# url-kaist/Quatro

Hardware: NVIDIA H100
Metric: registrations/sec (64-ring pair) (higher is better)
Workload: dtype f32 (front end, match, graph filter) / f64 (graph boundary, GNC, COTE)

## Files before the change

include/quatro_b200.h:

```cpp
#ifndef QUATRO_B200_H_
#define QUATRO_B200_H_

#include <stdint.h>

#ifdef __cplusplus
extern "C" {
#endif

#define QB200_VERSION 100

typedef enum qb200_status {
  QB200_OK = 0,
  QB200_DEGENERATE_CLIQUE = 1,
  QB200_DEGENERATE_INPUT = 2,
  QB200_CAPACITY_EXCEEDED = 3,
  QB200_ERR_BAD_ARG = -1,
  QB200_ERR_NO_DEVICE = -2,
  QB200_ERR_CUDA = -3,
  QB200_ERR_UNSUPPORTED = -4,
  QB200_ERR_VOXEL_OVERFLOW = -5
} qb200_status;

enum { QB200_FLAG_CLIQUE_TRUNCATED = 1  };
#define QB200_DEFAULT_CLIQUE_NODE_LIMIT 262144

enum { QB200_PMC_EXACT = 0, QB200_PMC_HEU = 1, QB200_KCORE_HEU = 2, QB200_INLIER_NONE = 3 };
enum { QB200_COTE_MEDIAN = 0, QB200_COTE_WEIGHTED_MEAN = 1 };
typedef enum qb200_mem_kind { QB200_MEM_HOST = 0, QB200_MEM_DEVICE = 1 } qb200_mem_kind;

typedef struct qb200_params {
  float voxel_size;
  float normal_radius;
  float fpfh_radius;
  float grid_cell;
  float tuple_scale;
  int32_t use_crosscheck;
  int32_t use_tuple_test;
  int32_t tuple_trials_per_corr;
  int32_t skip_flagged;
  int32_t reserved0;
  uint64_t seed;
  double noise_bound;
  double cbar2;
  double rot_noise_bound;
  double cote_noise_bound;
  double rotation_gnc_factor;
  double rotation_cost_threshold;
  double kcore_heuristic_threshold;
  int32_t rotation_max_iterations;
  int32_t inlier_selection_mode;
  int32_t cote_mode;
  int32_t using_rot_inliers_when_estimating_cote;
  int32_t use_pre_estimated_RyRx;
  int32_t max_clique_node_limit;
  double RyRx[9];
} qb200_params;

#define QB200_MAX_VOXEL_POINTS 262144

typedef struct qb200_config {
  int32_t device;
  int32_t max_batch_slots;
  int32_t max_raw_points;
  int32_t max_voxel_points;
  int32_t max_corr;
  int32_t reserved[3];
} qb200_config;

typedef struct qb200_result {
  int32_t valid;
  int32_t status;
  int32_t n_src_vox, n_tgt_vox;
  int32_t n_mutual;
  int32_t n_corr;
  int32_t max_core;
  int32_t clique_size;
  int32_t gnc_iters;
  int32_t n_rot_inliers;
  int32_t n_final_inliers;
  int32_t flags;
  int64_t n_edges;
  double cost;
  double T[16];
} qb200_result;

typedef struct qb200_pair {
  const float* src;
  const float* tgt;
  int32_t n_src, n_tgt;
} qb200_pair;

typedef struct qb200_handle qb200_handle;

void qb200_default_params(qb200_params* p);
void qb200_default_config(qb200_config* c);
int qb200_version(void);

int qb200_create(const qb200_config* cfg, qb200_handle** out);
void qb200_destroy(qb200_handle* h);
int qb200_set_stream(qb200_handle* h, void* cuda_stream);
const char* qb200_last_error(const qb200_handle* h);
int64_t qb200_launch_count(const qb200_handle* h);


int qb200_voxelize(qb200_handle* h, const float* pts4, int32_t n, float leaf, int32_t skip_flagged,
                   float* out4, int32_t cap, int32_t* n_out);

#define QB200_PW_MAX_ZONES 4
#define QB200_PW_MAX_THRESHOLDS 8
typedef struct qb200_patchwork_params {
  double sensor_height;
  double th_seeds;
  double th_dist;
  double max_range;
  double min_range;
  double uprightness_thr;
  double adaptive_seed_selection_margin;
  double global_elevation_threshold;
  double min_ranges_each_zone[QB200_PW_MAX_ZONES];
  double elevation_thresholds[QB200_PW_MAX_THRESHOLDS];
  double flatness_thresholds[QB200_PW_MAX_THRESHOLDS];
  int32_t num_iter;
  int32_t num_lpr;
  int32_t num_min_pts;
  int32_t using_global_elevation;
  int32_t num_zones;
  int32_t num_thresholds;
  int32_t num_sectors_each_zone[QB200_PW_MAX_ZONES];
  int32_t num_rings_each_zone[QB200_PW_MAX_ZONES];
} qb200_patchwork_params;
void qb200_default_patchwork_params(qb200_patchwork_params* p);

int qb200_patchwork(qb200_handle* h, const float* pts4, int32_t n, const qb200_patchwork_params* p,
                    float* ground4, int32_t* n_ground, float* nonground4, int32_t* n_nonground);

enum { QB200_NEIGHBORS_4 = 0, QB200_NEIGHBORS_8 = 1, QB200_NEIGHBORS_4_CROSS = 2 };
typedef struct qb200_segment_params {
  int32_t n_scan;
  int32_t horizon_scan;
  float ang_res_x;
  float ang_res_y;
  float ang_bottom;
  float segment_theta;
  int32_t neighbor_mode;
  int32_t min_pts_for_subclustering;
  int32_t segment_valid_point_num;
  int32_t segment_valid_line_num;
} qb200_segment_params;
void qb200_default_segment_params(qb200_segment_params* p);

int qb200_segment_cloud(qb200_handle* h, const float* pts4, int32_t n, const qb200_segment_params* p,
                        float* valid4, int32_t* n_valid, float* outlier4, int32_t* n_outlier);

int qb200_compute_fpfh(qb200_handle* h, const float* pts4, int32_t n, float normal_radius,
                       float fpfh_radius, float grid_cell, float* normals4, float* desc33);

int qb200_match(qb200_handle* h, const float* src4, int32_t n_src, const float* src_desc33,
                const float* tgt4, int32_t n_tgt, const float* tgt_desc33, const qb200_params* p,
                int32_t* corr, int32_t cap, int32_t* n_corr, int32_t* n_mutual);

int qb200_build_graph(qb200_handle* h, const float* a4, const float* b4, int32_t L,
                      double noise_bound, double cbar2, uint32_t* adj, int32_t words_per_row,
                      int32_t* degree, int64_t* n_edges);

int qb200_max_clique(qb200_handle* h, const uint32_t* adj, int32_t L, int32_t words_per_row,
                     int32_t mode, double kcore_heuristic_threshold, int32_t* clique, int32_t* n_clique,
                     int32_t* kcore, int32_t* kcore_order, int32_t* max_core);
int qb200_max_clique_ex(qb200_handle* h, const uint32_t* adj, int32_t L, int32_t words_per_row,
                        int32_t mode, double kcore_heuristic_threshold, int64_t node_limit, int32_t* clique, int32_t* n_clique,
                        int32_t* kcore, int32_t* kcore_order, int32_t* max_core, int32_t* flags);

int qb200_solve_pose(qb200_handle* h, const float* a4, const float* b4, int32_t L,
                     const int32_t* clique, int32_t n_clique, const qb200_params* p,
                     qb200_result* res, uint8_t* rot_inlier_mask, uint8_t* trans_inlier_mask);

int qb200_solve_correspondences(qb200_handle* h, const float* a4, const float* b4, int32_t L,
                                const qb200_params* p, qb200_result* res);

int qb200_match_and_pack(qb200_handle* h, const float* src4, int32_t n_src, const float* tgt4,
                         int32_t n_tgt, const qb200_params* p, int32_t* corr, float* src_matched4,
                         float* tgt_matched4, int32_t cap, int32_t* n_corr);

typedef struct qb200_corr_set {
  const float* a;
  const float* b;
  int32_t L;
  int32_t reserved;
} qb200_corr_set;
int qb200_solve_batch(qb200_handle* h, const qb200_corr_set* sets, int32_t n_sets, const qb200_params* p,
                      qb200_mem_kind kind, qb200_result* results);

int qb200_register_batch_enqueue(qb200_handle* h, const qb200_pair* pairs, int32_t n_pairs, const qb200_params* p, qb200_mem_kind kind,
                                 qb200_result* results);
int qb200_register_batch_flush(qb200_handle* h);

int qb200_register_pair(qb200_handle* h, const float* src4, int32_t n_src, const float* tgt4,
                        int32_t n_tgt, const qb200_params* p, qb200_result* res);

int qb200_register_batch(qb200_handle* h, const qb200_pair* pairs, int32_t n_pairs,
                         const qb200_params* p, qb200_mem_kind kind, qb200_result* results);

typedef struct qb200_slot_pair { int32_t src_slot, tgt_slot; } qb200_slot_pair;
int qb200_cache_reserve(qb200_handle* h, int32_t n_slots);
int qb200_cache_scans(qb200_handle* h, const float* const* scans4, const int32_t* n_points, const int32_t* slot_ids, int32_t n_scans,
                      const qb200_params* p, qb200_mem_kind kind);
int qb200_register_cached(qb200_handle* h, const qb200_slot_pair* pairs, int32_t n_pairs, const qb200_params* p, qb200_result* results);
int qb200_cache_copy(qb200_handle* h, int32_t from_slot, int32_t to_slot);
int qb200_cache_read(qb200_handle* h, int32_t slot, float* vox4, float* normals4, float* desc33, int32_t cap, int32_t* n);

#define QB200_UNIQUE_ID_BYTES 128
int qb200_comm_init_all(qb200_handle** handles, int32_t n_dev);
int qb200_register_batch_sharded(qb200_handle** handles, int32_t n_dev, const qb200_pair* pairs, int32_t n_pairs,
                                 const qb200_params* p, qb200_mem_kind kind, qb200_result* results);
int qb200_comm_unique_id(void* id128);
int qb200_comm_init_rank(qb200_handle* h, int32_t world, int32_t rank, const void* id128);
int qb200_register_batch_rank(qb200_handle* h, const qb200_pair* local_pairs, int32_t n_local, const qb200_params* p,
                              qb200_mem_kind kind, qb200_result* all_results, int32_t defer);
int qb200_comm_wait(qb200_handle* h);
int qb200_bind_numa(qb200_handle* h);

int qb200_get_last_clique(qb200_handle* h, int32_t* idx, int32_t cap, int32_t* n);
int qb200_get_last_final_inliers(qb200_handle* h, int32_t* idx, int32_t cap, int32_t* n);
int qb200_get_last_correspondences(qb200_handle* h, int32_t* corr, float* src_matched4,
                                   float* tgt_matched4, int32_t cap, int32_t* n);

int qb200_get_last_features(qb200_handle* h, int32_t which, float* normals4, float* desc33, int32_t cap, int32_t* n);

int qb200_get_stage_ms(qb200_handle* h, float* ms, int32_t n);

int qb200_get_kernel_ms(qb200_handle* h, float* ms, int32_t* launches, int32_t n);

int qb200_debug_tc_distances(qb200_handle* h, const float* a33, int32_t na, const float* b33, int32_t nb, float* out);


int qb200_debug_match_stats(qb200_handle* h, uint64_t* out4, int32_t reset);
int qb200_debug_tc_profile(qb200_handle* h, uint64_t* out24, int32_t reset);

int qb200_debug_match_verify(qb200_handle* h, uint64_t* out2, int32_t reset);

#ifdef __cplusplus
}
#endif
#endif
```

quatro_b200/capi.py:

```python
from __future__ import annotations

import ctypes as C
from typing import Optional, Sequence

import numpy as np

from . import _build

PMC_EXACT, PMC_HEU, KCORE_HEU, INLIER_NONE = 0, 1, 2, 3
FLAG_CLIQUE_TRUNCATED = 1
COTE_MEDIAN, COTE_WEIGHTED_MEAN = 0, 1
MEM_HOST, MEM_DEVICE = 0, 1

STATUS_NAMES = {0: "OK", 1: "DEGENERATE_CLIQUE", 2: "DEGENERATE_INPUT", 3: "CAPACITY_EXCEEDED", -1: "ERR_BAD_ARG",
                -2: "ERR_NO_DEVICE", -3: "ERR_CUDA", -4: "ERR_UNSUPPORTED", -5: "ERR_VOXEL_OVERFLOW"}


class Params(C.Structure):
    _fields_ = [
        ("voxel_size", C.c_float), ("normal_radius", C.c_float), ("fpfh_radius", C.c_float), ("grid_cell", C.c_float),
        ("tuple_scale", C.c_float), ("use_crosscheck", C.c_int32), ("use_tuple_test", C.c_int32),
        ("tuple_trials_per_corr", C.c_int32), ("skip_flagged", C.c_int32), ("reserved0", C.c_int32),
        ("seed", C.c_uint64),
        ("noise_bound", C.c_double), ("cbar2", C.c_double), ("rot_noise_bound", C.c_double),
        ("cote_noise_bound", C.c_double), ("rotation_gnc_factor", C.c_double),
        ("rotation_cost_threshold", C.c_double), ("kcore_heuristic_threshold", C.c_double),
        ("rotation_max_iterations", C.c_int32), ("inlier_selection_mode", C.c_int32), ("cote_mode", C.c_int32),
        ("using_rot_inliers_when_estimating_cote", C.c_int32), ("use_pre_estimated_RyRx", C.c_int32),
        ("max_clique_node_limit", C.c_int32), ("RyRx", C.c_double * 9),
    ]


class Config(C.Structure):
    _fields_ = [("device", C.c_int32), ("max_batch_slots", C.c_int32), ("max_raw_points", C.c_int32),
                ("max_voxel_points", C.c_int32), ("max_corr", C.c_int32), ("reserved", C.c_int32 * 3)]


class Result(C.Structure):
    _fields_ = [
        ("valid", C.c_int32), ("status", C.c_int32), ("n_src_vox", C.c_int32), ("n_tgt_vox", C.c_int32),
        ("n_mutual", C.c_int32), ("n_corr", C.c_int32), ("max_core", C.c_int32), ("clique_size", C.c_int32),
        ("gnc_iters", C.c_int32), ("n_rot_inliers", C.c_int32), ("n_final_inliers", C.c_int32),
        ("flags", C.c_int32), ("n_edges", C.c_int64), ("cost", C.c_double), ("T", C.c_double * 16),
    ]

    def matrix(self) -> np.ndarray:
        return np.array(self.T[:], dtype=np.float64).reshape(4, 4).T.copy()

    def as_dict(self) -> dict:
        d = {k: getattr(self, k) for k, _ in self._fields_ if k != "T"}
        d["T"] = self.matrix()
        return d


class PatchworkParams(C.Structure):
    _fields_ = [
        ("sensor_height", C.c_double), ("th_seeds", C.c_double), ("th_dist", C.c_double), ("max_range", C.c_double),
        ("min_range", C.c_double), ("uprightness_thr", C.c_double), ("adaptive_seed_selection_margin", C.c_double),
        ("global_elevation_threshold", C.c_double), ("min_ranges_each_zone", C.c_double * 4),
        ("elevation_thresholds", C.c_double * 8), ("flatness_thresholds", C.c_double * 8),
        ("num_iter", C.c_int32), ("num_lpr", C.c_int32), ("num_min_pts", C.c_int32), ("using_global_elevation", C.c_int32),
        ("num_zones", C.c_int32), ("num_thresholds", C.c_int32), ("num_sectors_each_zone", C.c_int32 * 4),
        ("num_rings_each_zone", C.c_int32 * 4),
    ]


class SegmentParams(C.Structure):
    _fields_ = [("n_scan", C.c_int32), ("horizon_scan", C.c_int32), ("ang_res_x", C.c_float), ("ang_res_y", C.c_float),
                ("ang_bottom", C.c_float), ("segment_theta", C.c_float), ("neighbor_mode", C.c_int32),
                ("min_pts_for_subclustering", C.c_int32), ("segment_valid_point_num", C.c_int32), ("segment_valid_line_num", C.c_int32)]


class Pair(C.Structure):
    _fields_ = [("src", C.c_void_p), ("tgt", C.c_void_p), ("n_src", C.c_int32), ("n_tgt", C.c_int32)]


class CorrSet(C.Structure):
    _fields_ = [("a", C.c_void_p), ("b", C.c_void_p), ("L", C.c_int32), ("reserved", C.c_int32)]


RESULT_DTYPE = np.dtype([
    ("valid", "<i4"), ("status", "<i4"), ("n_src_vox", "<i4"), ("n_tgt_vox", "<i4"), ("n_mutual", "<i4"),
    ("n_corr", "<i4"), ("max_core", "<i4"), ("clique_size", "<i4"), ("gnc_iters", "<i4"), ("n_rot_inliers", "<i4"),
    ("n_final_inliers", "<i4"), ("flags", "<i4"), ("n_edges", "<i8"), ("cost", "<f8"), ("T", "<f8", (16,)),
])
assert RESULT_DTYPE.itemsize == C.sizeof(Result)


class QuatroB200Error(RuntimeError):
    def __init__(self, code: int, where: str, detail: str = ""):
        self.code = code
        super().__init__(f"{where}: {STATUS_NAMES.get(code, code)} {detail}")


_LIB: Optional[C.CDLL] = None


def _f32(a, cols=None) -> np.ndarray:
    a = np.ascontiguousarray(a, dtype=np.float32)
    if cols is not None:
        assert a.ndim == 2 and a.shape[1] == cols, (a.shape, cols)
    return a


def _ptr(a: Optional[np.ndarray]):
    return None if a is None else a.ctypes.data_as(C.c_void_p)


def load_library(build: bool = True) -> C.CDLL:
    global _LIB
    if _LIB is not None:
        return _LIB
    path = _build.build_cuda() if build else _build.CUDA_LIB
    lib = C.CDLL(str(path))
    vp, i32, i64, f32, f64 = C.c_void_p, C.c_int32, C.c_int64, C.c_float, C.c_double
    P = C.POINTER
    sig = {
        "qb200_default_params": (None, [P(Params)]),
        "qb200_default_config": (None, [P(Config)]),
        "qb200_version": (i32, []),
        "qb200_create": (i32, [P(Config), P(vp)]),
        "qb200_destroy": (None, [vp]),
        "qb200_set_stream": (i32, [vp, vp]),
        "qb200_last_error": (C.c_char_p, [vp]),
        "qb200_launch_count": (i64, [vp]),
        "qb200_voxelize": (i32, [vp, vp, i32, f32, i32, vp, i32, P(i32)]),
        "qb200_default_patchwork_params": (None, [P(PatchworkParams)]),
        "qb200_default_segment_params": (None, [P(SegmentParams)]),
        "qb200_segment_cloud": (i32, [vp, vp, i32, P(SegmentParams), vp, P(i32), vp, P(i32)]),
        "qb200_patchwork": (i32, [vp, vp, i32, P(PatchworkParams), vp, P(i32), vp, P(i32)]),
        "qb200_compute_fpfh": (i32, [vp, vp, i32, f32, f32, f32, vp, vp]),
        "qb200_match": (i32, [vp, vp, i32, vp, vp, i32, vp, P(Params), vp, i32, P(i32), P(i32)]),
        "qb200_build_graph": (i32, [vp, vp, vp, i32, f64, f64, vp, i32, vp, P(i64)]),
        "qb200_max_clique": (i32, [vp, vp, i32, i32, i32, f64, vp, P(i32), vp, vp, P(i32)]),
        "qb200_max_clique_ex": (i32, [vp, vp, i32, i32, i32, f64, i64, vp, P(i32), vp, vp, P(i32), P(i32)]),
        "qb200_solve_pose": (i32, [vp, vp, vp, i32, vp, i32, P(Params), P(Result), vp, vp]),
        "qb200_solve_correspondences": (i32, [vp, vp, vp, i32, P(Params), P(Result)]),
        "qb200_match_and_pack": (i32, [vp, vp, i32, vp, i32, P(Params), vp, vp, vp, i32, P(i32)]),
        "qb200_register_pair": (i32, [vp, vp, i32, vp, i32, P(Params), P(Result)]),
        "qb200_register_batch": (i32, [vp, P(Pair), i32, P(Params), i32, vp]),
        "qb200_get_last_clique": (i32, [vp, vp, i32, P(i32)]),
        "qb200_get_last_final_inliers": (i32, [vp, vp, i32, P(i32)]),
        "qb200_get_last_correspondences": (i32, [vp, vp, vp, vp, i32, P(i32)]),
        "qb200_get_stage_ms": (i32, [vp, vp, i32]),
        "qb200_get_kernel_ms": (i32, [vp, vp, vp, i32]),
        "qb200_debug_tc_distances": (i32, [vp, vp, i32, vp, i32, vp]),
        "qb200_debug_match_stats": (i32, [vp, vp, i32]),
        "qb200_register_batch_enqueue": (i32, [vp, vp, i32, vp, i32, vp]),
        "qb200_register_batch_flush": (i32, [vp]),
        "qb200_debug_tc_profile": (i32, [vp, vp, i32]),
        "qb200_solve_batch": (i32, [vp, vp, i32, vp, i32, vp]),
        "qb200_comm_init_all": (i32, [P(vp), i32]),
        "qb200_register_batch_sharded": (i32, [P(vp), i32, P(Pair), i32, P(Params), i32, vp]),
        "qb200_comm_unique_id": (i32, [vp]),
        "qb200_comm_init_rank": (i32, [vp, i32, i32, vp]),
        "qb200_register_batch_rank": (i32, [vp, P(Pair), i32, P(Params), i32, vp, i32]),
        "qb200_comm_wait": (i32, [vp]),
        "qb200_bind_numa": (i32, [vp]),
        "qb200_debug_match_verify": (i32, [vp, vp, i32]),
        "qb200_get_last_features": (i32, [vp, i32, vp, vp, i32, P(i32)]),
        "qb200_cache_reserve": (i32, [vp, i32]),
        "qb200_cache_scans": (i32, [vp, P(vp), P(i32), P(i32), i32, P(Params), i32]),
        "qb200_register_cached": (i32, [vp, vp, i32, P(Params), vp]),
        "qb200_cache_copy": (i32, [vp, i32, i32]),
        "qb200_cache_read": (i32, [vp, i32, vp, vp, vp, i32, P(i32)]),
    }
    for name, (res, args) in sig.items():
        fn = getattr(lib, name)
        fn.restype = res
        fn.argtypes = args
    _LIB = lib
    return lib


EXPORTED_SYMBOLS = [
    "qb200_default_params", "qb200_default_config", "qb200_version", "qb200_create", "qb200_destroy",
    "qb200_set_stream", "qb200_last_error", "qb200_launch_count", "qb200_voxelize", "qb200_compute_fpfh",
    "qb200_default_patchwork_params", "qb200_patchwork", "qb200_default_segment_params", "qb200_segment_cloud", "qb200_match", "qb200_build_graph", "qb200_max_clique", "qb200_max_clique_ex", "qb200_solve_pose", "qb200_solve_correspondences",
    "qb200_match_and_pack", "qb200_register_pair", "qb200_register_batch", "qb200_get_last_clique",
    "qb200_get_last_final_inliers", "qb200_get_last_correspondences", "qb200_get_stage_ms", "qb200_get_kernel_ms",
    "qb200_debug_tc_distances",
    "qb200_debug_match_stats",
    "qb200_register_batch_enqueue",
    "qb200_register_batch_flush",
    "qb200_debug_tc_profile",
    "qb200_solve_batch",
    "qb200_comm_init_all", "qb200_register_batch_sharded", "qb200_comm_unique_id", "qb200_comm_init_rank",
    "qb200_register_batch_rank", "qb200_comm_wait", "qb200_bind_numa",
    "qb200_debug_match_verify", "qb200_get_last_features", "qb200_cache_reserve", "qb200_cache_scans", "qb200_register_cached", "qb200_cache_copy", "qb200_cache_read",
]


def default_params() -> Params:
    p = Params()
    p.voxel_size, p.normal_radius, p.fpfh_radius, p.grid_cell = 0.3, 0.5, 0.75, 0.0
    p.tuple_scale, p.use_crosscheck, p.use_tuple_test, p.tuple_trials_per_corr = 0.95, 1, 1, 100
    p.skip_flagged, p.seed = 1, 0x5EED
    p.noise_bound, p.cbar2, p.rot_noise_bound, p.cote_noise_bound = 0.3, 1.0, 0.0, 0.3
    p.rotation_gnc_factor, p.rotation_cost_threshold, p.kcore_heuristic_threshold = 1.4, 0.00011, 0.5
    p.rotation_max_iterations, p.inlier_selection_mode, p.cote_mode = 50, PMC_HEU, COTE_MEDIAN
    p.using_rot_inliers_when_estimating_cote, p.use_pre_estimated_RyRx = 0, 0
    for i in range(9):
        p.RyRx[i] = 1.0 if i in (0, 4, 8) else 0.0
    return p


def comm_init_all(handles: Sequence["Handle"]):
    arr = (C.c_void_p * len(handles))(*[h.h for h in handles])
    st = load_library().qb200_comm_init_all(arr, len(handles))
    if st != 0:
        raise QuatroB200Error(st, "qb200_comm_init_all")


def register_batch_sharded(handles: Sequence["Handle"], pairs: Sequence, params: "Params", kind: int = 0) -> np.ndarray:
    n = len(pairs)
    arr = (Pair * n)()
    keep = []
    for i, pr in enumerate(pairs):
        if kind == MEM_HOST:
            s, t = _f32(pr[0], 4), _f32(pr[1], 4)
            keep.append((s, t))
            arr[i].src, arr[i].n_src, arr[i].tgt, arr[i].n_tgt = s.ctypes.data, len(s), t.ctypes.data, len(t)
        else:
            arr[i].src, arr[i].n_src, arr[i].tgt, arr[i].n_tgt = pr[0], pr[1], pr[2], pr[3]
    out = np.zeros(n, RESULT_DTYPE)
    hs = (C.c_void_p * len(handles))(*[h.h for h in handles])
    st = load_library().qb200_register_batch_sharded(hs, len(handles), arr, n, C.byref(params), kind, _ptr(out))
    if st != 0:
        raise QuatroB200Error(st, "qb200_register_batch_sharded " + handles[0].last_error())
    return out


def default_patchwork_params() -> PatchworkParams:
    p = PatchworkParams()
    load_library().qb200_default_patchwork_params(C.byref(p))
    return p


def default_segment_params() -> SegmentParams:
    p = SegmentParams()
    load_library().qb200_default_segment_params(C.byref(p))
    return p


def default_config() -> Config:
    c = Config()
    c.device, c.max_batch_slots, c.max_raw_points, c.max_voxel_points, c.max_corr = 0, 64, 131072, 16384, 4096
    return c


class Handle:

    def __init__(self, config: Optional[Config] = None, **kw):
        self.lib = load_library()
        cfg = config or default_config()
        for k, v in kw.items():
            setattr(cfg, k, v)
        self.cfg = cfg
        h = C.c_void_p()
        st = self.lib.qb200_create(C.byref(cfg), C.byref(h))
        if st != 0:
            raise QuatroB200Error(st, "qb200_create")
        self.h = h

    def close(self):
        if getattr(self, "h", None):
            self.lib.qb200_destroy(self.h)
            self.h = None

    def __del__(self):
        try:
            self.close()
        except Exception:
            pass

    def __enter__(self):
        return self

    def __exit__(self, *a):
        self.close()

    def _check(self, st: int, where: str):
        if st < 0:
            msg = self.lib.qb200_last_error(self.h)
            raise QuatroB200Error(st, where, (msg or b"").decode())
        return st

    def set_stream(self, stream_ptr: int):
        self._check(self.lib.qb200_set_stream(self.h, C.c_void_p(stream_ptr)), "qb200_set_stream")

    def launch_count(self) -> int:
        return int(self.lib.qb200_launch_count(self.h))

    def voxelize(self, pts4, leaf: float, skip_flagged: int = 1, cap: Optional[int] = None):
        pts4 = _f32(pts4, 4)
        cap = cap or max(1, len(pts4))
        out = np.zeros((cap, 4), np.float32)
        n = C.c_int32(0)
        st = self.lib.qb200_voxelize(self.h, _ptr(pts4), len(pts4), leaf, skip_flagged, _ptr(out), cap, C.byref(n))
        if st != -5:
            self._check(st, "qb200_voxelize")
        return out[: min(n.value, cap)].copy(), st

    def compute_fpfh(self, pts4, normal_radius: float, fpfh_radius: float, grid_cell: float):
        pts4 = _f32(pts4, 4)
        n = len(pts4)
        normals = np.zeros((n, 4), np.float32)
        desc = np.zeros((n, 33), np.float32)
        self._check(self.lib.qb200_compute_fpfh(self.h, _ptr(pts4), n, normal_radius, fpfh_radius, grid_cell, _ptr(normals), _ptr(desc)),
                    "qb200_compute_fpfh")
        return normals, desc

    def match(self, src4, sdesc, tgt4, tdesc, params: Params, cap: Optional[int] = None):
        src4, tgt4, sdesc, tdesc = _f32(src4, 4), _f32(tgt4, 4), _f32(sdesc, 33), _f32(tdesc, 33)
        cap = cap or max(1, min(len(src4), len(tgt4)))
        corr = np.zeros((cap, 2), np.int32)
        n, nm = C.c_int32(0), C.c_int32(0)
        st = self._check(self.lib.qb200_match(self.h, _ptr(src4), len(src4), _ptr(sdesc), _ptr(tgt4), len(tgt4), _ptr(tdesc),
                                              C.byref(params), _ptr(corr), cap, C.byref(n), C.byref(nm)), "qb200_match")
        return corr[: min(n.value, cap)].copy(), nm.value, st

    def build_graph(self, a4, b4, noise_bound: float, cbar2: float, words_per_row: Optional[int] = None):
        a4, b4 = _f32(a4, 4), _f32(b4, 4)
        L = len(a4)
        wpr = words_per_row or (L + 31) // 32
        adj = np.zeros((L, wpr), np.uint32)
        deg = np.zeros(L, np.int32)
        ne = C.c_int64(0)
        self._check(self.lib.qb200_build_graph(self.h, _ptr(a4), _ptr(b4), L, noise_bound, cbar2, _ptr(adj), wpr, _ptr(deg), C.byref(ne)),
                    "qb200_build_graph")
        return adj, deg, ne.value

    def patchwork(self, pts, pp: "PatchworkParams"):
        pts = _f32(pts, 4)
        n = len(pts)
        g, ng = np.zeros((max(n, 1), 4), np.float32), np.zeros((max(n, 1), 4), np.float32)
        a, b = C.c_int32(0), C.c_int32(0)
        st = self._check(self.lib.qb200_patchwork(self.h, _ptr(pts), n, C.byref(pp), _ptr(g), C.byref(a), _ptr(ng), C.byref(b)), "qb200_patchwork")
        return g[: a.value].copy(), ng[: b.value].copy(), st

    def segment_cloud(self, pts, sp: "SegmentParams"):
        pts = _f32(pts, 4)
        npix = sp.n_scan * sp.horizon_scan
        v, o = np.zeros((npix, 4), np.float32), np.zeros((npix, 4), np.float32)
        a, b = C.c_int32(0), C.c_int32(0)
        self._check(self.lib.qb200_segment_cloud(self.h, _ptr(pts), len(pts), C.byref(sp), _ptr(v), C.byref(a), _ptr(o), C.byref(b)),
                    "qb200_segment_cloud")
        return v[: a.value].copy(), o[: b.value].copy()

    def max_clique(self, adj, mode: int = PMC_HEU, kcore_thr: float = 0.5):
        adj = np.ascontiguousarray(adj, np.uint32)
        L, wpr = adj.shape
        clique = np.zeros(max(L, 1), np.int32)
        kcore = np.zeros(max(L, 1), np.int32)
        order = np.zeros(max(L, 1), np.int32)
        n, mc = C.c_int32(0), C.c_int32(0)
        self._check(self.lib.qb200_max_clique(self.h, _ptr(adj), L, wpr, mode, kcore_thr, _ptr(clique), C.byref(n), _ptr(kcore),
                                              _ptr(order), C.byref(mc)), "qb200_max_clique")
        return clique[: n.value].copy(), kcore[:L].copy(), order[:L].copy(), mc.value

    def max_clique_ex(self, adj, mode: int = PMC_EXACT, kcore_thr: float = 0.5, node_limit: int = 0):
        adj = np.ascontiguousarray(adj, np.uint32)
        L, wpr = adj.shape
        clique, kcore, order = (np.zeros(max(L, 1), np.int32) for _ in range(3))
        n, mc, fl = C.c_int32(0), C.c_int32(0), C.c_int32(0)
        self._check(self.lib.qb200_max_clique_ex(self.h, _ptr(adj), L, wpr, mode, kcore_thr, node_limit, _ptr(clique), C.byref(n),
                                                 _ptr(kcore), _ptr(order), C.byref(mc), C.byref(fl)), "qb200_max_clique_ex")
        return clique[: n.value].copy(), kcore[:L].copy(), order[:L].copy(), mc.value, fl.value

    def solve_pose(self, a4, b4, clique, params: Params):
        a4, b4 = _f32(a4, 4), _f32(b4, 4)
        clique = np.ascontiguousarray(clique, np.int32)
        res = Result()
        rm = np.zeros(max(len(clique), 1), np.uint8)
        tm = np.zeros(max(len(clique), 1), np.uint8)
        st = self._check(self.lib.qb200_solve_pose(self.h, _ptr(a4), _ptr(b4), len(a4), _ptr(clique), len(clique), C.byref(params),
                                                   C.byref(res), _ptr(rm), _ptr(tm)), "qb200_solve_pose")
        return res, rm[: len(clique)], tm[: len(clique)], st

    def solve_correspondences(self, a4, b4, params: Params):
        a4, b4 = _f32(a4, 4), _f32(b4, 4)
        res = Result()
        st = self._check(self.lib.qb200_solve_correspondences(self.h, _ptr(a4), _ptr(b4), len(a4), C.byref(params), C.byref(res)),
                         "qb200_solve_correspondences")
        return res, st

    def match_and_pack(self, src4, tgt4, params: Params, cap: Optional[int] = None):
        src4, tgt4 = _f32(src4, 4), _f32(tgt4, 4)
        cap = cap or max(1, min(len(src4), len(tgt4)))
        corr = np.zeros((cap, 2), np.int32)
        sm = np.zeros((cap, 4), np.float32)
        tm = np.zeros((cap, 4), np.float32)
        n = C.c_int32(0)
        st = self._check(self.lib.qb200_match_and_pack(self.h, _ptr(src4), len(src4), _ptr(tgt4), len(tgt4), C.byref(params), _ptr(corr),
                                                       _ptr(sm), _ptr(tm), cap, C.byref(n)), "qb200_match_and_pack")
        m = min(n.value, cap)
        return corr[:m].copy(), sm[:m].copy(), tm[:m].copy(), st

    def register_pair(self, src4, tgt4, params: Params):
        src4, tgt4 = _f32(src4, 4), _f32(tgt4, 4)
        res = Result()
        st = self._check(self.lib.qb200_register_pair(self.h, _ptr(src4), len(src4), _ptr(tgt4), len(tgt4), C.byref(params), C.byref(res)),
                         "qb200_register_pair")
        return res, st

    def register_batch(self, pairs: Sequence, params: Params, kind: int = MEM_HOST) -> np.ndarray:
        n = len(pairs)
        arr = (Pair * n)()
        keep = []
        for i, pr in enumerate(pairs):
            if kind == MEM_HOST:
                s, t = _f32(pr[0], 4), _f32(pr[1], 4)
                keep.append((s, t))
                arr[i].src, arr[i].n_src, arr[i].tgt, arr[i].n_tgt = s.ctypes.data, len(s), t.ctypes.data, len(t)
            else:
                arr[i].src, arr[i].n_src, arr[i].tgt, arr[i].n_tgt = pr[0], pr[1], pr[2], pr[3]
        out = np.zeros(n, RESULT_DTYPE)
        self._check(self.lib.qb200_register_batch(self.h, arr, n, C.byref(params), kind, _ptr(out)), "qb200_register_batch")
        return out

    def solve_batch(self, sets: Sequence, params: Params, kind: int = MEM_HOST) -> np.ndarray:
        n = len(sets)
        arr = (CorrSet * n)()
        keep = []
        for i, st in enumerate(sets):
            if kind == MEM_HOST:
                a, b = _f32(st[0], 4), _f32(st[1], 4)
                assert len(a) == len(b)
                keep.append((a, b))
                arr[i].a, arr[i].b, arr[i].L = a.ctypes.data, b.ctypes.data, len(a)
            else:
                arr[i].a, arr[i].b, arr[i].L = st[0], st[1], st[2]
        out = np.zeros(n, RESULT_DTYPE)
        self._check(self.lib.qb200_solve_batch(self.h, arr, n, C.byref(params), kind, _ptr(out)), "qb200_solve_batch")
        return out

    def last_features(self, which: int, cap: Optional[int] = None):
        cap = cap or self.cfg.max_voxel_points
        nrm, desc = np.zeros((cap, 4), np.float32), np.zeros((cap, 33), np.float32)
        n = C.c_int32(0)
        self._check(self.lib.qb200_get_last_features(self.h, which, _ptr(nrm), _ptr(desc), cap, C.byref(n)), "qb200_get_last_features")
        m = min(n.value, cap)
        return nrm[:m].copy(), desc[:m].copy()

    def cache_reserve(self, n_slots: int):
        self._check(self.lib.qb200_cache_reserve(self.h, n_slots), "qb200_cache_reserve")

    def cache_scans(self, scans: Sequence, slot_ids: Sequence[int], params: Params, kind: int = MEM_HOST):
        n = len(scans)
        keep = [_f32(sc, 4) for sc in scans] if kind == MEM_HOST else None
        ptrs = (C.c_void_p * n)(*([a.ctypes.data for a in keep] if kind == MEM_HOST else [sc[0] for sc in scans]))
        cnts = (C.c_int32 * n)(*([len(a) for a in keep] if kind == MEM_HOST else [sc[1] for sc in scans]))
        ids = (C.c_int32 * n)(*[int(x) for x in slot_ids])
        self._check(self.lib.qb200_cache_scans(self.h, ptrs, cnts, ids, n, C.byref(params), kind), "qb200_cache_scans")

    def register_cached(self, slot_pairs, params: Params) -> np.ndarray:
        sp = np.ascontiguousarray(np.asarray(slot_pairs, np.int32).reshape(-1, 2))
        out = np.zeros(len(sp), RESULT_DTYPE)
        self._check(self.lib.qb200_register_cached(self.h, _ptr(sp), len(sp), C.byref(params), _ptr(out)), "qb200_register_cached")
        return out

    def cache_copy(self, from_slot: int, to_slot: int):
        self._check(self.lib.qb200_cache_copy(self.h, from_slot, to_slot), "qb200_cache_copy")

    def cache_read(self, slot: int, cap: Optional[int] = None):
        cap = cap or self.cfg.max_voxel_points
        vox, nrm, desc = np.zeros((cap, 4), np.float32), np.zeros((cap, 4), np.float32), np.zeros((cap, 33), np.float32)
        n = C.c_int32(0)
        self._check(self.lib.qb200_cache_read(self.h, slot, _ptr(vox), _ptr(nrm), _ptr(desc), cap, C.byref(n)), "qb200_cache_read")
        m = min(n.value, cap)
        return vox[:m].copy(), nrm[:m].copy(), desc[:m].copy()

    @staticmethod
    def comm_unique_id() -> bytes:
        buf = C.create_string_buffer(128)
        st = load_library().qb200_comm_unique_id(buf)
        if st != 0:
            raise QuatroB200Error(st, "qb200_comm_unique_id")
        return buf.raw

    def comm_init_rank(self, world: int, rank: int, unique_id: bytes):
        buf = C.create_string_buffer(unique_id, 128)
        self._check(self.lib.qb200_comm_init_rank(self.h, world, rank, buf), "qb200_comm_init_rank")
        self.world, self.rank = world, rank

    def register_batch_rank_raw(self, pair_array, n_local: int, params: Params, kind: int, out_all: np.ndarray, defer: bool = False):
        return self._check(self.lib.qb200_register_batch_rank(self.h, pair_array, n_local, C.byref(params), kind, _ptr(out_all), int(defer)),
                           "qb200_register_batch_rank")

    def bind_numa(self) -> int:
        return int(self.lib.qb200_bind_numa(self.h))

    def comm_wait(self):
        return self._check(self.lib.qb200_comm_wait(self.h), "qb200_comm_wait")

    def register_batch_raw(self, pair_array, n: int, params: Params, kind: int, out: np.ndarray):
        return self._check(self.lib.qb200_register_batch(self.h, pair_array, n, C.byref(params), kind, _ptr(out)), "qb200_register_batch")

    def register_batch_enqueue_raw(self, pair_array, n: int, params: Params, kind: int, out: np.ndarray):
        return self._check(self.lib.qb200_register_batch_enqueue(self.h, pair_array, n, C.byref(params), kind, _ptr(out)), "qb200_register_batch_enqueue")

    def register_batch_flush(self):
        return self._check(self.lib.qb200_register_batch_flush(self.h), "qb200_register_batch_flush")

    def last_clique(self, cap: int = 1 << 16):
        idx = np.zeros(cap, np.int32)
        n = C.c_int32(0)
        self._check(self.lib.qb200_get_last_clique(self.h, _ptr(idx), cap, C.byref(n)), "qb200_get_last_clique")
        return idx[: n.value].copy()

    def last_final_inliers(self, cap: int = 1 << 16):
        idx = np.zeros(cap, np.int32)
        n = C.c_int32(0)
        self._check(self.lib.qb200_get_last_final_inliers(self.h, _ptr(idx), cap, C.byref(n)), "qb200_get_last_final_inliers")
        return idx[: n.value].copy()

    def last_correspondences(self, cap: int = 1 << 16):
        corr = np.zeros((cap, 2), np.int32)
        sm = np.zeros((cap, 4), np.float32)
        tm = np.zeros((cap, 4), np.float32)
        n = C.c_int32(0)
        self._check(self.lib.qb200_get_last_correspondences(self.h, _ptr(corr), _ptr(sm), _ptr(tm), cap, C.byref(n)),
                    "qb200_get_last_correspondences")
        return corr[: n.value].copy(), sm[: n.value].copy(), tm[: n.value].copy()

    def debug_match_stats(self, reset: bool = True) -> dict:
        out = np.zeros(4, np.uint64)
        self._check(self.lib.qb200_debug_match_stats(self.h, _ptr(out), int(reset)), "qb200_debug_match_stats")
        return {"exact_evals": int(out[0]), "tiles": int(out[1]), "warmups": int(out[2]), "aborted_stripes": int(out[3])}

    def debug_tc_profile(self, reset: bool = True) -> np.ndarray:
        out = np.zeros(24, np.uint64)
        self._check(self.lib.qb200_debug_tc_profile(self.h, _ptr(out), int(reset)), "qb200_debug_tc_profile")
        return out

    def debug_match_verify(self, reset: bool = True) -> dict:
        out = np.zeros(2, np.uint64)
        self._check(self.lib.qb200_debug_match_verify(self.h, _ptr(out), int(reset)), "qb200_debug_match_verify")
        return {"compared": int(out[0]), "mismatches": int(out[1])}

    def debug_tc_distances(self, a33, b33) -> np.ndarray:
        a33, b33 = _f32(a33, 33), _f32(b33, 33)
        out = np.zeros((128, 128), np.float32)
        self._check(self.lib.qb200_debug_tc_distances(self.h, _ptr(a33), len(a33), _ptr(b33), len(b33), _ptr(out)), "qb200_debug_tc_distances")
        return out[: len(a33), : len(b33)].copy()

    def kernel_ms(self):
        ms = np.zeros(2, np.float32)
        calls = np.zeros(2, np.int32)
        self.lib.qb200_get_kernel_ms(self.h, _ptr(ms), _ptr(calls), 2)
        return ms, calls

    def stage_ms(self) -> np.ndarray:
        ms = np.zeros(8, np.float32)
        self.lib.qb200_get_stage_ms(self.h, _ptr(ms), 8)
        return ms
```

quatro_b200/csrc/api.cu:

```cuda
#include <math.h>
#include <new>
#include <stdio.h>
#include <stdlib.h>
#include <string.h>
#include <map>
#include <mutex>
#include <utility>
#include <vector>

#include "handle.cuh"

using namespace qb;

namespace qb {
int launch_degree(qb200_handle* h, int n_pairs);

int ensure_dyn_smem(qb200_handle* h, const void* kernel, size_t bytes) {
  static std::mutex mu;
  static std::map<std::pair<const void*, int>, size_t> current;
  std::lock_guard<std::mutex> lock(mu);
  size_t& cur = current[std::make_pair(kernel, h->device)];
  if (bytes > cur) {
    QB_CUDA_TRY(h, cudaFuncSetAttribute(kernel, cudaFuncAttributeMaxDynamicSharedMemorySize, (int)bytes));
    cur = bytes;
  }
  return QB200_OK;
}
}

namespace {

__global__ void wave_init_kernel(int* ctr_block, int n_ints, int* bbox, int n_clouds) {
  const int i = blockIdx.x * blockDim.x + threadIdx.x;
  if (i < n_ints) ctr_block[i] = 0;
  if (i < n_clouds * 6) bbox[i] = (i % 6) < 3 ? INT_MAX : INT_MIN;
}

__global__ void cache_copy_kernel(int to_cache, const int* __restrict__ slot_of_cloud, int V, float4* __restrict__ w_vox, float4* __restrict__ w_nrm,
                                  float* __restrict__ w_desc, int* __restrict__ w_n, int* __restrict__ w_status, float4* __restrict__ c_vox,
                                  float4* __restrict__ c_nrm, float* __restrict__ c_desc, int* __restrict__ c_n, int* __restrict__ c_status) {
  const int cloud = blockIdx.z, slot = slot_of_cloud[cloud], row = blockIdx.y;
  const int q = blockIdx.x * blockDim.x + threadIdx.x;
  if (slot < 0) return;
  const int n = to_cache ? w_n[cloud] : c_n[slot];
  if (row == 42) {
    if (q == 0) {
      if (to_cache) { c_n[slot] = w_n[cloud]; c_status[slot] = w_status[cloud]; }
      else { w_n[cloud] = c_n[slot]; w_status[cloud] = c_status[slot]; }
    }
    return;
  }
  if (q >= n || q >= V) return;
  if (row < kDescK) {
    float* w = w_desc + ((size_t)cloud * kDescK + row) * V + q;
    float* c = c_desc + ((size_t)slot * kDescK + row) * V + q;
    if (to_cache) *c = *w; else *w = *c;
  } else if (row == 40) {
    if (to_cache) c_vox[(size_t)slot * V + q] = w_vox[(size_t)cloud * V + q]; else w_vox[(size_t)cloud * V + q] = c_vox[(size_t)slot * V + q];
  } else {
    if (to_cache) c_nrm[(size_t)slot * V + q] = w_nrm[(size_t)cloud * V + q]; else w_nrm[(size_t)cloud * V + q] = c_nrm[(size_t)slot * V + q];
  }
}

template <class T>
cudaError_t dalloc(T** p, size_t count) {
  return cudaMalloc(reinterpret_cast<void**>(p), count * sizeof(T));
}

#define QB_ALLOC(h, ptr, count)                                                    \
  do {                                                                             \
    cudaError_t _e = dalloc(&(ptr), (size_t)(count));                              \
    if (_e != cudaSuccess) {                                                       \
      (h)->fail(__FILE__, __LINE__, cudaGetErrorString(_e));                       \
      return QB200_ERR_CUDA;                                                       \
    }                                                                              \
  } while (0)

int alloc_all(qb200_handle* h) {
  const size_t S = h->S, R = h->R, V = h->V, Lc = h->Lc, W = h->W, C = 2 * S;
  QB_CUDA_TRY(h, cudaMalloc((void**)&h->d_cloud_ptr, C * sizeof(float4*)));
  QB_ALLOC(h, h->d_cloud_n, C);
  QB_ALLOC(h, h->d_raw_off, C + 1);
  QB_CUDA_TRY(h, cudaMallocHost((void**)&h->h_cloud_ptr, C * sizeof(float4*)));
  QB_CUDA_TRY(h, cudaMallocHost((void**)&h->h_cloud_n, C * sizeof(int)));
  QB_CUDA_TRY(h, cudaMallocHost((void**)&h->h_raw_off, (C + 1) * sizeof(int)));
  QB_ALLOC(h, h->raw_stage, C * R);
  QB_CUDA_TRY(h, cudaEventCreate(&h->ev_fork));
  QB_CUDA_TRY(h, cudaStreamCreateWithFlags(&h->copy_stream, cudaStreamNonBlocking));
  QB_CUDA_TRY(h, cudaEventCreateWithFlags(&h->ev_copied, cudaEventDisableTiming));
  const size_t n_sort = C * (R > V ? R : V) + 64;
  const size_t n_hist = C * 256 * ((R + kVsTile - 1) / kVsTile);
  QB_ALLOC(h, h->key_a, n_sort);
  QB_ALLOC(h, h->key_b, n_sort);
  QB_ALLOC(h, h->val_a, n_sort > n_hist ? n_sort : n_hist);
  QB_ALLOC(h, h->val_b, n_sort);
  QB_ALLOC(h, h->aos_scratch, 2 * V * kDescDim);
  h->cub_bytes = sort_temp_bytes((int)(C * V));
  QB_CUDA_TRY(h, cudaMalloc(&h->cub_temp, h->cub_bytes));
  QB_ALLOC(h, h->vox_start, C * (V + 1));
  QB_ALLOC(h, h->vox_pts, C * V);
  QB_ALLOC(h, h->cell_key, C * V);
  QB_ALLOC(h, h->cell_start, C * (V + 1));
  QB_ALLOC(h, h->normals, C * V);
  QB_ALLOC(h, h->spfh, C * V * kDescPad);
  QB_ALLOC(h, h->nbr_list, C * kNbrGlobalCap * V);
  QB_ALLOC(h, h->nbr_cnt, C * V);
  QB_ALLOC(h, h->desc_t, C * kDescK * V);
  QB_CUDA_TRY(h, cudaMemset(h->desc_t, 0, C * kDescK * V * sizeof(float)));
  QB_ALLOC(h, h->desc_tiles, C * kDescK * V * 3);
  QB_CUDA_TRY(h, cudaMemset(h->desc_tiles, 0, C * kDescK * V * 3 * sizeof(float)));
  QB_ALLOC(h, h->desc_norm, C * V);
  QB_ALLOC(h, h->tc_fallback, S);
  QB_ALLOC(h, h->tc_stats, 32);
  QB_CUDA_TRY(h, cudaMemset(h->tc_stats, 0, 32 * sizeof(unsigned long long)));
  QB_ALLOC(h, h->rowbest, S * V);
  QB_ALLOC(h, h->colpart, 2 * S * V + S * (V >> 7) * 2 + 2);
  QB_ALLOC(h, h->colbest, S * V);
  QB_ALLOC(h, h->mut_i, S * V);
  QB_ALLOC(h, h->mut_j, S * V);
  QB_ALLOC(h, h->mark, S * V);
  QB_ALLOC(h, h->partner, S * V);
  QB_ALLOC(h, h->mean, C * 4);
  QB_ALLOC(h, h->corr_src, S * Lc);
  QB_ALLOC(h, h->corr_tgt, S * Lc);
  QB_ALLOC(h, h->ma, S * Lc);
  QB_ALLOC(h, h->mb, S * Lc);
  QB_ALLOC(h, h->adj, S * Lc * W);
  QB_ALLOC(h, h->adjp, S * Lc * W);
  QB_ALLOC(h, h->deg, S * Lc);
  QB_ALLOC(h, h->kcore, S * (Lc + 2));
  QB_ALLOC(h, h->korder, S * (Lc + 2));
  QB_ALLOC(h, h->rank_of, S * (Lc + 2));
  QB_ALLOC(h, h->by_rank, S * (Lc + 2));
  QB_ALLOC(h, h->kbin, S * (Lc + 2));
  QB_ALLOC(h, h->clique, S * Lc);
  QB_ALLOC(h, h->final_inl, S * Lc);
  QB_ALLOC(h, h->rot_mask, S * Lc);
  QB_ALLOC(h, h->trans_mask, S * Lc);
  QB_ALLOC(h, h->d_results, S);
  QB_CUDA_TRY(h, cudaMemset(h->d_results, 0, S * sizeof(qb200_result)));
  QB_CUDA_TRY(h, cudaMallocHost((void**)&h->h_results, S * sizeof(qb200_result)));
  const size_t n_ints = C * 5 + C * 6 + S * 7 + 2 * S + 2;
  QB_ALLOC(h, h->ctr_block, n_ints);
  h->ctr_ints = n_ints;
  int* p = h->ctr_block;
  h->ctr.n_edges = reinterpret_cast<long long*>(p); p += 2 * S;
  h->ctr.n_valid = p; p += C;
  h->ctr.n_vox = p; p += C;
  h->ctr.n_lat = p; p += C;
  h->ctr.n_cells = p; p += C;
  h->ctr.cloud_status = p; p += C;
  h->ctr.bbox = p; p += C * 6;
  h->ctr.n_mutual = p; p += S;
  h->ctr.n_corr = p; p += S;
  h->ctr.swapped = p; p += S;
  h->ctr.n_clique = p; p += S;
  h->ctr.max_core = p; p += S;
  h->ctr.n_final = p; p += S;
  h->ctr.flags = p; p += S;
  for (int i = 0; i < 9; ++i) QB_CUDA_TRY(h, cudaEventCreate(&h->ev[i]));
  for (int i = 0; i < 4; ++i) QB_CUDA_TRY(h, cudaEventCreate(&h->kev[i]));
  return QB200_OK;
}

int wave_reset(qb200_handle* h, int n_clouds) {
  const int n = (int)h->ctr_ints;
  wave_init_kernel<<<(n + 255) / 256, 256, 0, h->stream>>>(h->ctr_block, n, h->ctr.bbox, n_clouds);
  h->launches++;
  QB_CUDA_TRY(h, cudaGetLastError());
  return QB200_OK;
}

int set_counter(qb200_handle* h, int* dptr, int value) {
  QB_CUDA_TRY(h, cudaMemcpyAsync(dptr, &value, sizeof(int), cudaMemcpyHostToDevice, h->stream));
  QB_CUDA_TRY(h, cudaStreamSynchronize(h->stream));
  return QB200_OK;
}

int get_counter(qb200_handle* h, const int* dptr, int* value) {
  QB_CUDA_TRY(h, cudaMemcpyAsync(value, dptr, sizeof(int), cudaMemcpyDeviceToHost, h->stream));
  QB_CUDA_TRY(h, cudaStreamSynchronize(h->stream));
  return QB200_OK;
}

bool params_ok(const qb200_params* p) {
  if (!p) return false;
  if (!(p->voxel_size > 0) || !(p->normal_radius > 0) || !(p->fpfh_radius > 0)) return false;
  if (p->normal_radius > p->fpfh_radius) return false;
  if (!(p->noise_bound > 0) || !(p->cbar2 > 0) || !(p->cote_noise_bound > 0)) return false;
  if (p->cote_mode != QB200_COTE_MEDIAN && p->cote_mode != QB200_COTE_WEIGHTED_MEAN) return false;
  if (p->inlier_selection_mode < 0 || p->inlier_selection_mode > 3 || p->max_clique_node_limit < 0) return false;
  if (p->rotation_max_iterations < 0 || p->tuple_trials_per_corr < 0) return false;
  return true;
}

float lattice_cell(const qb200_params& p) { return p.grid_cell > 0 ? p.grid_cell : p.fpfh_radius * 1.001953125f; }

int run_solver(qb200_handle* h, int n_pairs, const qb200_params& p, int have_frontend) {
  int rc;
  if (p.inlier_selection_mode == QB200_INLIER_NONE) {
    if ((rc = launch_iota_clique(h, n_pairs))) return rc;
  } else {
    if ((rc = launch_graph(h, n_pairs, p.noise_bound, p.cbar2))) return rc;
    if (h->ev[5]) cudaEventRecord(h->ev[5], h->stream);
    if ((rc = launch_clique(h, n_pairs, p.inlier_selection_mode, p.kcore_heuristic_threshold, p.max_clique_node_limit))) return rc;
  }
  if (h->ev[6]) cudaEventRecord(h->ev[6], h->stream);
  if ((rc = launch_fill_counters(h, n_pairs, have_frontend))) return rc;
  if ((rc = launch_pose(h, n_pairs, p))) return rc;
  if ((rc = launch_finalize_status(h, n_pairs))) return rc;
  return QB200_OK;
}

int upload_matched(qb200_handle* h, const float* a4, const float* b4, int L) {
  if (L > h->Lc) {
    h->fail(__FILE__, __LINE__, "L exceeds max_corr");
    return QB200_ERR_BAD_ARG;
  }
  int rc = wave_reset(h, 2);
  if (rc) return rc;
  if (L > 0) {
    QB_CUDA_TRY(h, cudaMemcpyAsync(h->ma, a4, (size_t)L * sizeof(float4), cudaMemcpyHostToDevice, h->stream));
    QB_CUDA_TRY(h, cudaMemcpyAsync(h->mb, b4, (size_t)L * sizeof(float4), cudaMemcpyHostToDevice, h->stream));
  }
  return set_counter(h, h->ctr.n_corr, L);
}

int upload_cloud_as_voxels(qb200_handle* h, int cloud, const float* pts4, int n) {
  if (n > h->V) {
    h->fail(__FILE__, __LINE__, "cloud exceeds max_voxel_points");
    return QB200_ERR_BAD_ARG;
  }
  if (n > 0) QB_CUDA_TRY(h, cudaMemcpyAsync(h->vox_pts + (size_t)cloud * h->V, pts4, (size_t)n * sizeof(float4), cudaMemcpyHostToDevice, h->stream));
  return set_counter(h, h->ctr.n_vox + cloud, n);
}

int fetch_result(qb200_handle* h, qb200_result* res) {
  QB_CUDA_TRY(h, cudaMemcpyAsync(h->h_results, h->d_results, sizeof(qb200_result), cudaMemcpyDeviceToHost, h->stream));
  QB_CUDA_TRY(h, cudaStreamSynchronize(h->stream));
  *res = h->h_results[0];
  h->last_n_corr = res->n_corr;
  h->last_n_clique = res->clique_size;
  h->last_n_final = res->n_final_inliers;
  return res->status;
}

}

#define QB_IDLE(h)                                        \
  do {                                                    \
    if ((h) && (h)->lanes_active) {                       \
      const int rc_idle_ = batch_flush(h);                \
      if (rc_idle_) return rc_idle_;                      \
    }                                                     \
  } while (0)

extern "C" {
static int batch_flush(qb200_handle* h);
static void cache_free(qb200_handle* h);
}
static void cache_free_public(qb200_handle* h) { cache_free(h); }

extern "C" {

int qb200_version(void) { return QB200_VERSION; }

void qb200_default_params(qb200_params* p) {
  memset(p, 0, sizeof(*p));
  p->voxel_size = 0.3f; p->normal_radius = 0.5f; p->fpfh_radius = 0.75f; p->grid_cell = 0.0f;
  p->tuple_scale = 0.95f; p->use_crosscheck = 1; p->use_tuple_test = 1; p->tuple_trials_per_corr = 100;
  p->skip_flagged = 1; p->seed = 0x5EED;
  p->noise_bound = 0.3; p->cbar2 = 1.0; p->rot_noise_bound = 0.0; p->cote_noise_bound = 0.3;
  p->rotation_gnc_factor = 1.4; p->rotation_cost_threshold = 0.00011; p->kcore_heuristic_threshold = 0.5;
  p->rotation_max_iterations = 50; p->inlier_selection_mode = QB200_PMC_HEU; p->cote_mode = QB200_COTE_MEDIAN;
  p->using_rot_inliers_when_estimating_cote = 0; p->use_pre_estimated_RyRx = 0;
  p->RyRx[0] = p->RyRx[4] = p->RyRx[8] = 1.0;
}

void qb200_default_config(qb200_config* c) {
  memset(c, 0, sizeof(*c));
  c->device = 0; c->max_batch_slots = 64; c->max_raw_points = 131072; c->max_voxel_points = 16384; c->max_corr = 4096;
}

int qb200_create(const qb200_config* cfg_in, qb200_handle** out) {
  if (!out) return QB200_ERR_BAD_ARG;
  *out = nullptr;
  qb200_config cfg;
  if (cfg_in) cfg = *cfg_in; else qb200_default_config(&cfg);
  if (cfg.max_batch_slots < 1 || cfg.max_batch_slots > 2048 || cfg.max_raw_points < 1 || cfg.max_voxel_points < kMatchTile ||
      cfg.max_voxel_points % kMatchTile != 0 || cfg.max_voxel_points > QB200_MAX_VOXEL_POINTS || cfg.max_corr < 32 || cfg.max_corr % 32 != 0 ||
      cfg.max_corr > 8192 || (long long)cfg.max_batch_slots * 2 * cfg.max_raw_points > 2000000000LL ||
      (long long)cfg.max_batch_slots * 2 * cfg.max_voxel_points > 2000000000LL)
    return QB200_ERR_BAD_ARG;
  int ndev = 0;
  if (cudaGetDeviceCount(&ndev) != cudaSuccess || ndev <= 0 || cfg.device < 0 || cfg.device >= ndev) return QB200_ERR_NO_DEVICE;
  if (cudaSetDevice(cfg.device) != cudaSuccess) return QB200_ERR_NO_DEVICE;
  qb200_handle* h = new (std::nothrow) qb200_handle();
  if (!h) return QB200_ERR_CUDA;
  memset(h, 0, sizeof(*h));
  h->cfg = cfg; h->device = cfg.device;
  h->S = cfg.max_batch_slots; h->R = cfg.max_raw_points; h->V = cfg.max_voxel_points; h->Lc = cfg.max_corr;
  h->W = h->Lc / 32; h->NS = h->V / kMatchTile;
  if (cudaDeviceGetAttribute(&h->n_sm, cudaDevAttrMultiProcessorCount, cfg.device) != cudaSuccess || h->n_sm <= 0) { delete h; return QB200_ERR_NO_DEVICE; }
  const char* fe = getenv("QB200_MATCH_EXACT");
  h->force_exact_match = (fe && fe[0] == '1') ? 1 : 0;
  const char* ln = getenv("QB200_LANES");
  h->max_lanes = (ln && ln[0] >= '1' && ln[0] <= '8') ? ln[0] - '0' : 4;
  if (cudaStreamCreateWithFlags(&h->own_stream, cudaStreamNonBlocking) != cudaSuccess) { delete h; return QB200_ERR_CUDA; }
  h->stream = h->own_stream;
  const int rc = alloc_all(h);
  if (rc != QB200_OK) {
    fprintf(stderr, "qb200_create: %s\n", h->err);
    qb200_destroy(h);
    return rc;
  }
  cudaStreamSynchronize(h->stream);
  *out = h;
  return QB200_OK;
}

void qb200_destroy(qb200_handle* h) {
  if (!h) return;
  cudaSetDevice(h->device);
  cudaDeviceSynchronize();
  comm_release(h);
  cache_free_public(h);
  void* dev_ptrs[] = {(void*)h->d_cloud_ptr, h->d_cloud_n, h->d_raw_off, h->raw_stage, h->key_a, h->key_b, h->val_a, h->val_b, h->cub_temp,
                      h->vox_start, h->vox_pts, h->cell_key, h->cell_start, h->normals, h->spfh, h->nbr_list, h->nbr_cnt, h->desc_t, h->rowbest, h->colpart, h->colbest,
                      h->desc_tiles, h->desc_norm, h->tc_fallback, h->tc_stats, h->aos_scratch,
                      h->mut_i, h->mut_j, h->mark, h->partner, h->mean, h->corr_src, h->corr_tgt, h->ma, h->mb, h->adj, h->adjp, h->deg,
                      h->kcore, h->korder, h->rank_of, h->by_rank, h->kbin, h->clique, h->ex_stack, h->ex_pool, h->ex_lvl, h->ex_cur, h->pw_ints, h->pw_out, h->ip_buf, h->final_inl, h->rot_mask, h->trans_mask, h->d_results,
                      h->ctr_block};
  for (void* p : dev_ptrs)
    if (p) cudaFree(p);
  if (h->h_cloud_ptr) cudaFreeHost((void*)h->h_cloud_ptr);
  if (h->h_cloud_n) cudaFreeHost(h->h_cloud_n);
  if (h->h_raw_off) cudaFreeHost(h->h_raw_off);
  if (h->h_results) cudaFreeHost(h->h_results);
  for (int i = 0; i < 9; ++i)
    if (h->ev[i]) cudaEventDestroy(h->ev[i]);
  for (int i = 0; i < 4; ++i)
    if (h->kev[i]) cudaEventDestroy(h->kev[i]);
  if (h->ev_fork) cudaEventDestroy(h->ev_fork);
  if (h->ev_copied) cudaEventDestroy(h->ev_copied);
  if (h->copy_stream) cudaStreamDestroy(h->copy_stream);
  for (int i = 0; i < 7; ++i)
    if (h->lane[i]) qb200_destroy(h->lane[i]);
  if (h->own_stream) cudaStreamDestroy(h->own_stream);
  delete h;
}

int qb200_set_stream(qb200_handle* h, void* cuda_stream) {
  if (!h) return QB200_ERR_BAD_ARG;
  h->stream = cuda_stream ? (cudaStream_t)cuda_stream : h->own_stream;
  return QB200_OK;
}

const char* qb200_last_error(const qb200_handle* h) { return h ? h->err : "null handle"; }
int64_t qb200_launch_count(const qb200_handle* h) {
  if (!h) return 0;
  int64_t n = h->launches;
  for (int i = 0; i < 7; ++i)
    if (h->lane[i]) n += h->lane[i]->launches;
  return n;
}

int qb200_voxelize(qb200_handle* h, const float* pts4, int32_t n, float leaf, int32_t skip_flagged, float* out4, int32_t cap,
                   int32_t* n_out) {
  QB_IDLE(h);
  if (!h || !n_out || n < 0 || (n > 0 && !pts4) || !(leaf > 0) || cap < 0 || (cap > 0 && !out4)) return QB200_ERR_BAD_ARG;
  *n_out = 0;
  if (n > h->R) { h->fail(__FILE__, __LINE__, "n exceeds max_raw_points"); return QB200_ERR_BAD_ARG; }
  cudaSetDevice(h->device);
  if (n == 0) return QB200_OK;
  int rc = wave_reset(h, 1);
  if (rc) return rc;
  QB_CUDA_TRY(h, cudaMemcpyAsync(h->raw_stage, pts4, (size_t)n * sizeof(float4), cudaMemcpyHostToDevice, h->stream));
  h->h_cloud_ptr[0] = h->raw_stage; h->h_cloud_n[0] = n; h->h_raw_off[0] = 0; h->h_raw_off[1] = n;
  QB_CUDA_TRY(h, cudaMemcpyAsync(h->d_cloud_ptr, h->h_cloud_ptr, sizeof(float4*), cudaMemcpyHostToDevice, h->stream));
  QB_CUDA_TRY(h, cudaMemcpyAsync(h->d_cloud_n, h->h_cloud_n, sizeof(int), cudaMemcpyHostToDevice, h->stream));
  QB_CUDA_TRY(h, cudaMemcpyAsync(h->d_raw_off, h->h_raw_off, 2 * sizeof(int), cudaMemcpyHostToDevice, h->stream));
  if ((rc = launch_voxel(h, 1, leaf, skip_flagged))) return rc;
  int nv = 0, st = 0;
  if ((rc = get_counter(h, h->ctr.n_vox, &nv))) return rc;
  if ((rc = get_counter(h, h->ctr.cloud_status, &st))) return rc;
  if (st == QB200_ERR_VOXEL_OVERFLOW) {
    int m = 0;
    for (int i = 0; i < n; ++i) {
      const float* p = pts4 + 4 * (size_t)i;
      if (!(isfinite(p[0]) && isfinite(p[1]) && isfinite(p[2])) || (skip_flagged && p[3] < 0.0f)) continue;
      if (m < cap) memcpy(out4 + 4 * (size_t)m, p, 4 * sizeof(float));
      ++m;
    }
    *n_out = m;
    return m > cap ? QB200_CAPACITY_EXCEEDED : QB200_ERR_VOXEL_OVERFLOW;
  }
  *n_out = nv;
  const int m = nv < cap ? nv : cap;
  if (m > 0) {
    QB_CUDA_TRY(h, cudaMemcpyAsync(out4, h->vox_pts, (size_t)m * sizeof(float4), cudaMemcpyDeviceToHost, h->stream));
    QB_CUDA_TRY(h, cudaStreamSynchronize(h->stream));
  }
  if (st == QB200_CAPACITY_EXCEEDED || nv > cap) return QB200_CAPACITY_EXCEEDED;
  return QB200_OK;
}

int qb200_patchwork(qb200_handle* h, const float* pts4, int32_t n, const qb200_patchwork_params* p, float* ground4, int32_t* n_ground,
                    float* nonground4, int32_t* n_nonground) {
  QB_IDLE(h);
  if (!h || !p || !n_ground || !n_nonground || n < 0 || (n > 0 && !pts4)) return QB200_ERR_BAD_ARG;
  *n_ground = *n_nonground = 0;
  if (n > h->R) { h->fail(__FILE__, __LINE__, "n exceeds max_raw_points"); return QB200_ERR_BAD_ARG; }
  cudaSetDevice(h->device);
  if (n > 0) QB_CUDA_TRY(h, cudaMemcpyAsync(h->raw_stage, pts4, (size_t)n * sizeof(float4), cudaMemcpyHostToDevice, h->stream));
  int ng = 0, nn = 0, st = 0;
  const int rc = launch_patchwork(h, h->raw_stage, n, *p, &ng, &nn, &st);
  if (rc) return rc;
  *n_ground = ng;
  *n_nonground = nn;
  if (ground4 && ng > 0) QB_CUDA_TRY(h, cudaMemcpyAsync(ground4, h->pw_out, (size_t)ng * sizeof(float4), cudaMemcpyDeviceToHost, h->stream));
  if (nonground4 && nn > 0)
    QB_CUDA_TRY(h, cudaMemcpyAsync(nonground4, h->pw_out + h->R, (size_t)nn * sizeof(float4), cudaMemcpyDeviceToHost, h->stream));
  QB_CUDA_TRY(h, cudaStreamSynchronize(h->stream));
  return st;
}

int qb200_segment_cloud(qb200_handle* h, const float* pts4, int32_t n, const qb200_segment_params* p, float* valid4, int32_t* n_valid,
                        float* outlier4, int32_t* n_outlier) {
  QB_IDLE(h);
  if (!h || !p || !n_valid || !n_outlier || n < 0 || (n > 0 && !pts4)) return QB200_ERR_BAD_ARG;
  *n_valid = *n_outlier = 0;
  if (n > h->R) { h->fail(__FILE__, __LINE__, "n exceeds max_raw_points"); return QB200_ERR_BAD_ARG; }
  cudaSetDevice(h->device);
  if (n > 0) QB_CUDA_TRY(h, cudaMemcpyAsync(h->raw_stage, pts4, (size_t)n * sizeof(float4), cudaMemcpyHostToDevice, h->stream));
  int nv = 0, no = 0;
  const float4 *dv = nullptr, *dout = nullptr;
  const int rc = launch_segment_cloud(h, h->raw_stage, n, *p, &nv, &no, &dv, &dout);
  if (rc) return rc;
  *n_valid = nv;
  *n_outlier = no;
  if (valid4 && nv > 0) QB_CUDA_TRY(h, cudaMemcpyAsync(valid4, dv, (size_t)nv * sizeof(float4), cudaMemcpyDeviceToHost, h->stream));
  if (outlier4 && no > 0) QB_CUDA_TRY(h, cudaMemcpyAsync(outlier4, dout, (size_t)no * sizeof(float4), cudaMemcpyDeviceToHost, h->stream));
  QB_CUDA_TRY(h, cudaStreamSynchronize(h->stream));
  return QB200_OK;
}

int qb200_compute_fpfh(qb200_handle* h, const float* pts4, int32_t n, float normal_radius, float fpfh_radius, float grid_cell,
                       float* normals4, float* desc33) {
  QB_IDLE(h);
  if (!h || n < 0 || (n > 0 && !pts4) || !(normal_radius > 0) || !(fpfh_radius > 0) || !(grid_cell > 0)) return QB200_ERR_BAD_ARG;
  if (normal_radius > fpfh_radius) return QB200_ERR_BAD_ARG;
  cudaSetDevice(h->device);
  if (n == 0) return QB200_OK;
  int rc = wave_reset(h, 1);
  if (rc) return rc;
  if ((rc = upload_cloud_as_voxels(h, 0, pts4, n))) return rc;
  if ((rc = launch_fpfh(h, 1, normal_radius, fpfh_radius, grid_cell))) return rc;
  if (normals4) QB_CUDA_TRY(h, cudaMemcpyAsync(normals4, h->normals, (size_t)n * sizeof(float4), cudaMemcpyDeviceToHost, h->stream));
  if (desc33) {
    float* scratch = h->aos_scratch;
    if ((rc = launch_desc_to_aos(h, 0, n, scratch))) return rc;
    QB_CUDA_TRY(h, cudaMemcpyAsync(desc33, scratch, (size_t)n * kDescDim * sizeof(float), cudaMemcpyDeviceToHost, h->stream));
  }
  QB_CUDA_TRY(h, cudaStreamSynchronize(h->stream));
  return QB200_OK;
}

static int download_corr(qb200_handle* h, int32_t* corr, float* sm4, float* tm4, int cap, int32_t* n_corr, int32_t* n_mutual) {
  int nc = 0, nm = 0, st = 0, rc;
  if ((rc = get_counter(h, h->ctr.n_corr, &nc))) return rc;
  if ((rc = get_counter(h, h->ctr.n_mutual, &nm))) return rc;
  if ((rc = get_counter(h, h->ctr.cloud_status, &st))) return rc;
  *n_corr = nc;
  if (n_mutual) *n_mutual = nm;
  h->last_n_corr = nc;
  const int m = nc < cap ? nc : cap;
  if (m > 0) {
    std::vector<int> s(m), t(m);
    QB_CUDA_TRY(h, cudaMemcpyAsync(s.data(), h->corr_src, (size_t)m * sizeof(int), cudaMemcpyDeviceToHost, h->stream));
    QB_CUDA_TRY(h, cudaMemcpyAsync(t.data(), h->corr_tgt, (size_t)m * sizeof(int), cudaMemcpyDeviceToHost, h->stream));
    if (sm4) QB_CUDA_TRY(h, cudaMemcpyAsync(sm4, h->ma, (size_t)m * sizeof(float4), cudaMemcpyDeviceToHost, h->stream));
    if (tm4) QB_CUDA_TRY(h, cudaMemcpyAsync(tm4, h->mb, (size_t)m * sizeof(float4), cudaMemcpyDeviceToHost, h->stream));
    QB_CUDA_TRY(h, cudaStreamSynchronize(h->stream));
    if (corr)
      for (int i = 0; i < m; ++i) { corr[2 * i] = s[i]; corr[2 * i + 1] = t[i]; }
  }
  if (st == QB200_CAPACITY_EXCEEDED || nc > cap) return QB200_CAPACITY_EXCEEDED;
  return QB200_OK;
}

int qb200_match(qb200_handle* h, const float* src4, int32_t n_src, const float* src_desc33, const float* tgt4, int32_t n_tgt,
                const float* tgt_desc33, const qb200_params* p, int32_t* corr, int32_t cap, int32_t* n_corr, int32_t* n_mutual) {
  QB_IDLE(h);
  if (!h || !p || !n_corr || n_src < 0 || n_tgt < 0 || cap < 0) return QB200_ERR_BAD_ARG;
  if ((n_src > 0 && (!src4 || !src_desc33)) || (n_tgt > 0 && (!tgt4 || !tgt_desc33))) return QB200_ERR_BAD_ARG;
  if (!p->use_crosscheck) return QB200_ERR_UNSUPPORTED;
  *n_corr = 0;
  if (n_mutual) *n_mutual = 0;
  if (n_src > h->V || n_tgt > h->V) { h->fail(__FILE__, __LINE__, "cloud exceeds max_voxel_points"); return QB200_ERR_BAD_ARG; }
  cudaSetDevice(h->device);
  if (n_src == 0 || n_tgt == 0) return QB200_OK;
  int rc = wave_reset(h, 2);
  if (rc) return rc;
  if ((rc = upload_cloud_as_voxels(h, 0, src4, n_src))) return rc;
  if ((rc = upload_cloud_as_voxels(h, 1, tgt4, n_tgt))) return rc;
  float* scratch = h->aos_scratch;
  QB_CUDA_TRY(h, cudaMemcpyAsync(scratch, src_desc33, (size_t)n_src * kDescDim * sizeof(float), cudaMemcpyHostToDevice, h->stream));
  if ((rc = launch_desc_from_aos(h, 0, n_src, scratch))) return rc;
  float* scratch2 = scratch + (size_t)h->V * kDescDim;
  QB_CUDA_TRY(h, cudaMemcpyAsync(scratch2, tgt_desc33, (size_t)n_tgt * kDescDim * sizeof(float), cudaMemcpyHostToDevice, h->stream));
  if ((rc = launch_desc_from_aos(h, 1, n_tgt, scratch2))) return rc;
  if ((rc = launch_match(h, 1, *p))) return rc;
  return download_corr(h, corr, nullptr, nullptr, cap, n_corr, n_mutual);
}

int qb200_match_and_pack(qb200_handle* h, const float* src4, int32_t n_src, const float* tgt4, int32_t n_tgt, const qb200_params* p,
                         int32_t* corr, float* src_matched4, float* tgt_matched4, int32_t cap, int32_t* n_corr) {
  QB_IDLE(h);
  if (!h || !n_corr || !params_ok(p) || n_src < 0 || n_tgt < 0 || cap < 0) return QB200_ERR_BAD_ARG;
  if (!p->use_crosscheck) return QB200_ERR_UNSUPPORTED;
  *n_corr = 0;
  if (n_src > h->V || n_tgt > h->V) { h->fail(__FILE__, __LINE__, "cloud exceeds max_voxel_points"); return QB200_ERR_BAD_ARG; }
  cudaSetDevice(h->device);
  if (n_src == 0 || n_tgt == 0) return QB200_OK;
  int rc = wave_reset(h, 2);
  if (rc) return rc;
  if ((rc = upload_cloud_as_voxels(h, 0, src4, n_src))) return rc;
  if ((rc = upload_cloud_as_voxels(h, 1, tgt4, n_tgt))) return rc;
  if ((rc = launch_fpfh(h, 2, p->normal_radius, p->fpfh_radius, lattice_cell(*p)))) return rc;
  if ((rc = launch_match(h, 1, *p))) return rc;
  return download_corr(h, corr, src_matched4, tgt_matched4, cap, n_corr, nullptr);
}

int qb200_build_graph(qb200_handle* h, const float* a4, const float* b4, int32_t L, double noise_bound, double cbar2, uint32_t* adj,
                      int32_t words_per_row, int32_t* degree, int64_t* n_edges) {
  QB_IDLE(h);
  if (!h || L < 0 || (L > 0 && (!a4 || !b4 || !adj)) || words_per_row < (L + 31) / 32 || !(noise_bound > 0) || !(cbar2 > 0))
    return QB200_ERR_BAD_ARG;
  cudaSetDevice(h->device);
  if (n_edges) *n_edges = 0;
  if (L == 0) return QB200_OK;
  int rc = upload_matched(h, a4, b4, L);
  if (rc) return rc;
  if ((rc = launch_graph(h, 1, noise_bound, cbar2))) return rc;
  const int nb = (L + 31) / 32;
  memset(adj, 0, (size_t)L * words_per_row * sizeof(uint32_t));
  QB_CUDA_TRY(h, cudaMemcpy2DAsync(adj, (size_t)words_per_row * 4, h->adj, (size_t)h->W * 4, (size_t)nb * 4, L, cudaMemcpyDeviceToHost, h->stream));
  if (degree) QB_CUDA_TRY(h, cudaMemcpyAsync(degree, h->deg, (size_t)L * sizeof(int), cudaMemcpyDeviceToHost, h->stream));
  long long e2 = 0;
  QB_CUDA_TRY(h, cudaMemcpyAsync(&e2, h->ctr.n_edges, sizeof(long long), cudaMemcpyDeviceToHost, h->stream));
  QB_CUDA_TRY(h, cudaStreamSynchronize(h->stream));
  if (n_edges) *n_edges = e2 / 2;
  return QB200_OK;
}

int qb200_max_clique_ex(qb200_handle* h, const uint32_t* adj, int32_t L, int32_t words_per_row, int32_t mode, double kcore_thr,
                        int64_t node_limit, int32_t* clique, int32_t* n_clique, int32_t* kcore, int32_t* kcore_order, int32_t* max_core,
                        int32_t* flags) {
  QB_IDLE(h);
  if (!h || !n_clique || L < 0 || (L > 0 && (!adj || !clique)) || words_per_row < (L + 31) / 32) return QB200_ERR_BAD_ARG;
  if (mode != QB200_PMC_EXACT && mode != QB200_PMC_HEU && mode != QB200_KCORE_HEU) return QB200_ERR_BAD_ARG;
  if (node_limit < 0) return QB200_ERR_BAD_ARG;
  if (flags) *flags = 0;
  *n_clique = 0;
  if (max_core) *max_core = 0;
  if (L > h->Lc) { h->fail(__FILE__, __LINE__, "L exceeds max_corr"); return QB200_ERR_BAD_ARG; }
  cudaSetDevice(h->device);
  if (L == 0) return QB200_OK;
  int rc = wave_reset(h, 2);
  if (rc) return rc;
  const int nb = (L + 31) / 32;
  QB_CUDA_TRY(h, cudaMemsetAsync(h->adj, 0, (size_t)L * h->W * 4, h->stream));
  QB_CUDA_TRY(h, cudaMemcpy2DAsync(h->adj, (size_t)h->W * 4, adj, (size_t)words_per_row * 4, (size_t)nb * 4, L, cudaMemcpyHostToDevice, h->stream));
  if ((rc = set_counter(h, h->ctr.n_corr, L))) return rc;
  if ((rc = launch_degree(h, 1))) return rc;
  if ((rc = launch_clique(h, 1, mode, kcore_thr, node_limit))) return rc;
  int nc = 0, mc = 0, fl = 0;
  if ((rc = get_counter(h, h->ctr.n_clique, &nc))) return rc;
  if ((rc = get_counter(h, h->ctr.max_core, &mc))) return rc;
  if ((rc = get_counter(h, h->ctr.flags, &fl))) return rc;
  if (flags) *flags = fl;
  *n_clique = nc;
  if (max_core) *max_core = mc;
  if (nc > 0) QB_CUDA_TRY(h, cudaMemcpyAsync(clique, h->clique, (size_t)nc * sizeof(int), cudaMemcpyDeviceToHost, h->stream));
  if (kcore) QB_CUDA_TRY(h, cudaMemcpyAsync(kcore, h->kcore, (size_t)L * sizeof(int), cudaMemcpyDeviceToHost, h->stream));
  if (kcore_order) QB_CUDA_TRY(h, cudaMemcpyAsync(kcore_order, h->korder, (size_t)L * sizeof(int), cudaMemcpyDeviceToHost, h->stream));
  QB_CUDA_TRY(h, cudaStreamSynchronize(h->stream));
  h->last_n_clique = nc;
  return QB200_OK;
}

int qb200_max_clique(qb200_handle* h, const uint32_t* adj, int32_t L, int32_t words_per_row, int32_t mode, double kcore_thr,
                     int32_t* clique, int32_t* n_clique, int32_t* kcore, int32_t* kcore_order, int32_t* max_core) {
  return qb200_max_clique_ex(h, adj, L, words_per_row, mode, kcore_thr, 0, clique, n_clique, kcore, kcore_order, max_core, nullptr);
}

int qb200_solve_pose(qb200_handle* h, const float* a4, const float* b4, int32_t L, const int32_t* clique, int32_t n_clique,
                     const qb200_params* p, qb200_result* res, uint8_t* rot_inlier_mask, uint8_t* trans_inlier_mask) {
  QB_IDLE(h);
  if (!h || !res || !params_ok(p) || L < 0 || (L > 0 && (!a4 || !b4)) || n_clique < 0 || n_clique > L || (n_clique > 0 && !clique))
    return QB200_ERR_BAD_ARG;
  cudaSetDevice(h->device);
  int rc = upload_matched(h, a4, b4, L);
  if (rc) return rc;
  if (n_clique > 0) QB_CUDA_TRY(h, cudaMemcpyAsync(h->clique, clique, (size_t)n_clique * sizeof(int), cudaMemcpyHostToDevice, h->stream));
  if ((rc = set_counter(h, h->ctr.n_clique, n_clique))) return rc;
  if ((rc = launch_fill_counters(h, 1, 0))) return rc;
  if ((rc = launch_pose(h, 1, *p))) return rc;
  rc = fetch_result(h, res);
  if (rc < 0) return rc;
  if (res->valid) {
    const int nc = res->clique_size;
    if (rot_inlier_mask) QB_CUDA_TRY(h, cudaMemcpyAsync(rot_inlier_mask, h->rot_mask, (size_t)nc, cudaMemcpyDeviceToHost, h->stream));
    if (trans_inlier_mask) QB_CUDA_TRY(h, cudaMemcpyAsync(trans_inlier_mask, h->trans_mask, (size_t)nc, cudaMemcpyDeviceToHost, h->stream));
    QB_CUDA_TRY(h, cudaStreamSynchronize(h->stream));
  }
  return rc;
}

int qb200_solve_correspondences(qb200_handle* h, const float* a4, const float* b4, int32_t L, const qb200_params* p, qb200_result* res) {
  if (!h || !res || !params_ok(p) || L < 0 || (L > 0 && (!a4 || !b4))) return QB200_ERR_BAD_ARG;
  cudaSetDevice(h->device);
  int rc = upload_matched(h, a4, b4, L);
  if (rc) return rc;
  if ((rc = run_solver(h, 1, *p, 0))) return rc;
  return fetch_result(h, res);
}

int qb200_solve_batch(qb200_handle* h, const qb200_corr_set* sets, int32_t n_sets, const qb200_params* p, qb200_mem_kind kind,
                      qb200_result* results) {
  QB_IDLE(h);
  if (!h || n_sets < 0 || (n_sets > 0 && (!sets || !results)) || !params_ok(p)) return QB200_ERR_BAD_ARG;
  for (int i = 0; i < n_sets; ++i)
    if (sets[i].L < 0 || sets[i].L > h->Lc || (sets[i].L > 0 && (!sets[i].a || !sets[i].b))) {
      h->fail(__FILE__, __LINE__, "correspondence set is null or exceeds max_corr");
      return QB200_ERR_BAD_ARG;
    }
  cudaSetDevice(h->device);
  for (int i = 0; i < 8; ++i) h->stage_ms[i] = 0.f;
  for (int i = 0; i < 2; ++i) { h->kernel_ms[i] = 0.f; h->kernel_calls[i] = 0; h->kev_armed[i] = 0; }
  const cudaMemcpyKind ck = kind == QB200_MEM_HOST ? cudaMemcpyHostToDevice : cudaMemcpyDeviceToDevice;
  for (int w0 = 0; w0 < n_sets; w0 += h->S) {
    const int np = n_sets - w0 < h->S ? n_sets - w0 : h->S;
    int rc = wave_reset(h, 2 * np);
    if (rc) return rc;
    for (int s = 0; s < np; ++s) {
      const qb200_corr_set& cs = sets[w0 + s];
      h->h_cloud_n[s] = cs.L;
      if (cs.L > 0) {
        QB_CUDA_TRY(h, cudaMemcpyAsync(h->ma + (size_t)s * h->Lc, cs.a, (size_t)cs.L * sizeof(float4), ck, h->stream));
        QB_CUDA_TRY(h, cudaMemcpyAsync(h->mb + (size_t)s * h->Lc, cs.b, (size_t)cs.L * sizeof(float4), ck, h->stream));
      }
    }
    QB_CUDA_TRY(h, cudaMemcpyAsync(h->ctr.n_corr, h->h_cloud_n, (size_t)np * sizeof(int), cudaMemcpyHostToDevice, h->stream));
    cudaEventRecord(h->ev[4], h->stream);
    cudaEventRecord(h->ev[5], h->stream);
    if ((rc = run_solver(h, np, *p, 0))) return rc;
    cudaEventRecord(h->ev[7], h->stream);
    QB_CUDA_TRY(h, cudaMemcpyAsync(h->h_results, h->d_results, (size_t)np * sizeof(qb200_result), cudaMemcpyDeviceToHost, h->stream));
    QB_CUDA_TRY(h, cudaStreamSynchronize(h->stream));
    memcpy(results + w0, h->h_results, (size_t)np * sizeof(qb200_result));
    for (int i = 4; i < 7; ++i) {
      float ms = 0.f;
      if (cudaEventElapsedTime(&ms, h->ev[i], h->ev[i + 1]) == cudaSuccess) h->stage_ms[i] += ms;
    }
    if (h->kev_armed[1]) {
      float ms = 0.f;
      if (cudaEventElapsedTime(&ms, h->kev[2], h->kev[3]) == cudaSuccess) { h->kernel_ms[1] += ms; h->kernel_calls[1] += 1; }
      h->kev_armed[1] = 0;
    }
  }
  if (n_sets == 1) {
    h->last_n_corr = results[0].n_corr;
    h->last_n_clique = results[0].clique_size;
    h->last_n_final = results[0].n_final_inliers;
  }
  return QB200_OK;
}

static int wave_submit(qb200_handle* L, const qb200_pair* pairs, int w0, int np, qb200_mem_kind kind, const qb200_params* p, float cell,
                       cudaStream_t cs) {
  const int ncl = 2 * np;
  int rc;
  cudaEventRecord(L->ev[0], L->stream);
  const cudaStream_t cps = cs ? cs : L->stream;
  int total = 0;
  const float* run_src = nullptr;
  int run_dst = 0, run_n = 0;
  auto flush_run = [&]() -> int {
    if (run_n > 0)
      QB_CUDA_TRY(L, cudaMemcpyAsync(L->raw_stage + run_dst, run_src, (size_t)run_n * sizeof(float4), cudaMemcpyHostToDevice, cps));
    run_n = 0;
    return QB200_OK;
  };
  for (int s = 0; s < np; ++s) {
    const qb200_pair& pr = pairs[w0 + s];
    const float* ptr[2] = {pr.src, pr.tgt};
    const int cnt[2] = {pr.n_src, pr.n_tgt};
    for (int k = 0; k < 2; ++k) {
      const int cloud = 2 * s + k;
      L->h_raw_off[cloud] = total;
      L->h_cloud_n[cloud] = cnt[k];
      if (kind == QB200_MEM_HOST) {
        L->h_cloud_ptr[cloud] = L->raw_stage + total;
        if (cnt[k] > 0) {
          if (run_n > 0 && ptr[k] == run_src + (size_t)run_n * 4 && run_n < (1 << 26)) {
            run_n += cnt[k];
          } else {
            if ((rc = flush_run())) return rc;
            run_src = ptr[k]; run_dst = total; run_n = cnt[k];
          }
        }
      } else {
        L->h_cloud_ptr[cloud] = reinterpret_cast<const float4*>(ptr[k]);
      }
      total += cnt[k];
    }
  }
  if ((rc = flush_run())) return rc;
  L->h_raw_off[ncl] = total;
  QB_CUDA_TRY(L, cudaMemcpyAsync(L->d_cloud_ptr, L->h_cloud_ptr, (size_t)ncl * sizeof(float4*), cudaMemcpyHostToDevice, cps));
  QB_CUDA_TRY(L, cudaMemcpyAsync(L->d_cloud_n, L->h_cloud_n, (size_t)ncl * sizeof(int), cudaMemcpyHostToDevice, cps));
  QB_CUDA_TRY(L, cudaMemcpyAsync(L->d_raw_off, L->h_raw_off, (size_t)(ncl + 1) * sizeof(int), cudaMemcpyHostToDevice, cps));
  if ((rc = wave_reset(L, ncl))) return rc;
  if (cs) {
    QB_CUDA_TRY(L, cudaEventRecord(L->ev_copied, cs));
    QB_CUDA_TRY(L, cudaStreamWaitEvent(L->stream, L->ev_copied, 0));
  }
  cudaEventRecord(L->ev[1], L->stream);
  if ((rc = launch_voxel(L, ncl, p->voxel_size, p->skip_flagged))) return rc;
  cudaEventRecord(L->ev[2], L->stream);
  if ((rc = launch_fpfh(L, ncl, p->normal_radius, p->fpfh_radius, cell))) return rc;
  cudaEventRecord(L->ev[3], L->stream);
  if ((rc = launch_match(L, np, *p))) return rc;
  cudaEventRecord(L->ev[4], L->stream);
  cudaEventRecord(L->ev[5], L->stream);
  if ((rc = run_solver(L, np, *p, 1))) return rc;
  cudaEventRecord(L->ev[7], L->stream);
  QB_CUDA_TRY(L, cudaMemcpyAsync(L->h_results, L->d_results, (size_t)np * sizeof(qb200_result), cudaMemcpyDeviceToHost, L->stream));
  cudaEventRecord(L->ev[8], L->stream);
  L->pend_w0 = w0;
  L->pend_np = np;
  return QB200_OK;
}

static int wave_collect(qb200_handle* h, qb200_handle* L) {
  if (L->pend_np == 0) return QB200_OK;
  const int np = L->pend_np;
  L->pend_np = 0;
  if (cudaStreamSynchronize(L->stream) != cudaSuccess) {
    h->fail(__FILE__, __LINE__, cudaGetErrorString(cudaGetLastError()));
    return QB200_ERR_CUDA;
  }
  memcpy(L->pend_dst + L->pend_w0, L->h_results, (size_t)np * sizeof(qb200_result));
  static const int timeline = (getenv("QB200_TIMELINE") && getenv("QB200_TIMELINE")[0] == '1') ? 1 : 0;
  if (timeline) {
    fprintf(stderr, "[qb200 timeline] wave w0=%d np=%d:", L->pend_w0, np);
    for (int i = 0; i < 9; ++i) {
      float ms = -1.f;
      cudaEventElapsedTime(&ms, h->ev_fork, L->ev[i]);
      fprintf(stderr, " %.2f", ms);
    }
    fprintf(stderr, "\n");
  }
  for (int i = 0; i < 8; ++i) {
    float ms = 0.f;
    if (cudaEventElapsedTime(&ms, L->ev[i], L->ev[i + 1]) == cudaSuccess) h->stage_ms[i] += ms;
  }
  for (int k = 0; k < 2; ++k) {
    float ms = 0.f;
    if (L->kev_armed[k] && cudaEventElapsedTime(&ms, L->kev[2 * k], L->kev[2 * k + 1]) == cudaSuccess) {
      h->kernel_ms[k] += ms;
      h->kernel_calls[k] += 1;
    }
    L->kev_armed[k] = 0;
  }
  return QB200_OK;
}

static int batch_flush(qb200_handle* h) {
  int rc = QB200_OK;
  const int n = h->lanes_active > 0 ? h->lanes_active : 1;
  for (int i = 0; i < n; ++i) {
    const int l = (h->lane_cursor + i) % n;
    qb200_handle* L = l == 0 ? h : h->lane[l - 1];
    if (!L) continue;
    const int rc2 = wave_collect(h, L);
    if (rc == QB200_OK) rc = rc2;
  }
  h->lanes_active = 0;
  h->lane_cursor = 0;
  return rc;
}

static int collect_batch_impl(qb200_handle* h, const qb200_result* dst) {
  int rc = QB200_OK;
  const int n = h->lanes_active > 0 ? h->lanes_active : 1;
  for (int i = 0; i < n; ++i) {
    const int l = (h->lane_cursor + i) % n;
    qb200_handle* L = l == 0 ? h : h->lane[l - 1];
    if (!L || L->pend_np == 0 || L->pend_dst != dst) continue;
    const int rc2 = wave_collect(h, L);
    if (rc == QB200_OK) rc = rc2;
  }
  return rc;
}

int qb200_register_batch_flush(qb200_handle* h) {
  if (!h) return QB200_ERR_BAD_ARG;
  cudaSetDevice(h->device);
  return batch_flush(h);
}

int qb200_register_batch(qb200_handle* h, const qb200_pair* pairs, int32_t n_pairs, const qb200_params* p, qb200_mem_kind kind,
                         qb200_result* results) {
  int rc = qb200_register_batch_enqueue(h, pairs, n_pairs, p, kind, results);
  const int rc2 = h ? batch_flush(h) : QB200_OK;
  if (rc == QB200_OK) rc = rc2;
  if (rc != QB200_OK) return rc;
  if (n_pairs == 1) {
    h->last_n_corr = results[0].n_corr;
    h->last_n_clique = results[0].clique_size;
    h->last_n_final = results[0].n_final_inliers;
  }
  return QB200_OK;
}

int qb200_register_batch_enqueue(qb200_handle* h, const qb200_pair* pairs, int32_t n_pairs, const qb200_params* p, qb200_mem_kind kind,
                                 qb200_result* results) {
  if (!h || n_pairs < 0 || (n_pairs > 0 && (!pairs || !results)) || !params_ok(p)) return QB200_ERR_BAD_ARG;
  if (!p->use_crosscheck) return QB200_ERR_UNSUPPORTED;
  for (int i = 0; i < n_pairs; ++i) {
    if (pairs[i].n_src < 0 || pairs[i].n_tgt < 0 || pairs[i].n_src > h->R || pairs[i].n_tgt > h->R ||
        (pairs[i].n_src > 0 && !pairs[i].src) || (pairs[i].n_tgt > 0 && !pairs[i].tgt)) {
      h->fail(__FILE__, __LINE__, "pair has a null cloud or exceeds max_raw_points");
      return QB200_ERR_BAD_ARG;
    }
  }
  cudaSetDevice(h->device);
  const bool pipelined = h->lanes_active > 0;
  if (!pipelined) {
    for (int i = 0; i < 8; ++i) h->stage_ms[i] = 0.f;
    for (int i = 0; i < 2; ++i) { h->kernel_ms[i] = 0.f; h->kernel_calls[i] = 0; h->kev_armed[i] = 0; }
  }
  qb200_params p_resolved = *p;
  if (!(p_resolved.rot_noise_bound > 0)) {
    if (h->rot_noise_bound_latched <= 0) h->rot_noise_bound_latched = 2.0 * p->noise_bound;
    p_resolved.rot_noise_bound = h->rot_noise_bound_latched;
  }
  p = &p_resolved;
  const float cell = lattice_cell(*p);
  int wave_n[64], n_waves = 0;
  {
    int left = n_pairs;
    if (kind == QB200_MEM_HOST && n_pairs > h->S && h->S >= 8 && h->max_lanes > 1) {
      wave_n[n_waves++] = h->S / 4;
      wave_n[n_waves++] = h->S - h->S / 4;
      left -= h->S;
    }
    while (left > 0 && n_waves < 63) {
      wave_n[n_waves] = left < h->S ? left : h->S;
      left -= wave_n[n_waves++];
    }
    if (left > 0) n_waves = 0;
  }
  const bool planned = n_waves > 0;
  if (!planned) n_waves = (n_pairs + h->S - 1) / h->S;
  int n_lanes = n_waves < h->max_lanes ? (n_waves < 1 ? 1 : n_waves) : h->max_lanes;
  if (pipelined && h->lanes_active != n_lanes) {
    const int rc0 = batch_flush(h);
    if (rc0) return rc0;
  }
  const bool fresh = h->lanes_active == 0;
  qb200_handle* lanes[8] = {h, h, h, h, h, h, h, h};
  for (int l = 1; l < n_lanes; ++l) {
    if (!h->lane[l - 1]) {
      const int rc = qb200_create(&h->cfg, &h->lane[l - 1]);
      if (rc != QB200_OK) {
        h->fail(__FILE__, __LINE__, "cannot allocate another lane");
        return rc;
      }
      h->lane[l - 1]->max_lanes = 1;
    }
    lanes[l] = h->lane[l - 1];
    if (fresh) {
      if (l == 1) QB_CUDA_TRY(h, cudaEventRecord(h->ev_fork, h->stream));
      QB_CUDA_TRY(h, cudaStreamWaitEvent(lanes[l]->stream, h->ev_fork, 0));
    }
  }
  cudaStream_t copy_stream = nullptr;
  if (kind == QB200_MEM_HOST && n_lanes > 1) {
    copy_stream = h->copy_stream;
    if (fresh) QB_CUDA_TRY(h, cudaStreamWaitEvent(copy_stream, h->ev_fork, 0));
  }
  h->lanes_active = n_lanes;
  int rc = QB200_OK, wave = 0;
  for (int w0 = 0; w0 < n_pairs && rc == QB200_OK; ++wave) {
    qb200_handle* L = lanes[h->lane_cursor];
    int np = planned ? wave_n[wave] : h->S;
    if (np > n_pairs - w0) np = n_pairs - w0;
    if ((rc = wave_collect(h, L))) break;
    L->pend_dst = results;
    rc = wave_submit(L, pairs, w0, np, kind, p, cell, copy_stream);
    if (rc != QB200_OK && L != h) h->fail(__FILE__, __LINE__, L->err);
    h->lane_cursor = (h->lane_cursor + 1) % n_lanes;
    w0 += np;
  }
  return rc;
}

int qb200_register_pair(qb200_handle* h, const float* src4, int32_t n_src, const float* tgt4, int32_t n_tgt, const qb200_params* p,
                        qb200_result* res) {
  if (!res) return QB200_ERR_BAD_ARG;
  qb200_pair pr;
  pr.src = src4; pr.tgt = tgt4; pr.n_src = n_src; pr.n_tgt = n_tgt;
  const int rc = qb200_register_batch(h, &pr, 1, p, QB200_MEM_HOST, res);
  if (rc != QB200_OK) return rc;
  return res->status;
}

static int copy_ints(qb200_handle* h, const int* dsrc, int n_have, int32_t* dst, int32_t cap, int32_t* n) {
  if (!h || !n || cap < 0) return QB200_ERR_BAD_ARG;
  *n = n_have;
  const int m = n_have < cap ? n_have : cap;
  cudaSetDevice(h->device);
  if (m > 0 && dst) {
    QB_CUDA_TRY(h, cudaMemcpyAsync(dst, dsrc, (size_t)m * sizeof(int), cudaMemcpyDeviceToHost, h->stream));
    QB_CUDA_TRY(h, cudaStreamSynchronize(h->stream));
  }
  return n_have > cap ? QB200_CAPACITY_EXCEEDED : QB200_OK;
}
int qb200_get_last_clique(qb200_handle* h, int32_t* idx, int32_t cap, int32_t* n) {
  return h ? copy_ints(h, h->clique, h->last_n_clique, idx, cap, n) : QB200_ERR_BAD_ARG;
}
int qb200_get_last_final_inliers(qb200_handle* h, int32_t* idx, int32_t cap, int32_t* n) {
  return h ? copy_ints(h, h->final_inl, h->last_n_final, idx, cap, n) : QB200_ERR_BAD_ARG;
}
int qb200_get_last_correspondences(qb200_handle* h, int32_t* corr, float* src_matched4, float* tgt_matched4, int32_t cap, int32_t* n) {
  if (!h || !n || cap < 0) return QB200_ERR_BAD_ARG;
  cudaSetDevice(h->device);
  const int nc = h->last_n_corr;
  *n = nc;
  const int m = nc < cap ? nc : cap;
  if (m > 0) {
    std::vector<int> s(m), t(m);
    QB_CUDA_TRY(h, cudaMemcpyAsync(s.data(), h->corr_src, (size_t)m * sizeof(int), cudaMemcpyDeviceToHost, h->stream));
    QB_CUDA_TRY(h, cudaMemcpyAsync(t.data(), h->corr_tgt, (size_t)m * sizeof(int), cudaMemcpyDeviceToHost, h->stream));
    if (src_matched4) QB_CUDA_TRY(h, cudaMemcpyAsync(src_matched4, h->ma, (size_t)m * sizeof(float4), cudaMemcpyDeviceToHost, h->stream));
    if (tgt_matched4) QB_CUDA_TRY(h, cudaMemcpyAsync(tgt_matched4, h->mb, (size_t)m * sizeof(float4), cudaMemcpyDeviceToHost, h->stream));
    QB_CUDA_TRY(h, cudaStreamSynchronize(h->stream));
    if (corr)
      for (int i = 0; i < m; ++i) { corr[2 * i] = s[i]; corr[2 * i + 1] = t[i]; }
  }
  return nc > cap ? QB200_CAPACITY_EXCEEDED : QB200_OK;
}

int qb200_get_last_features(qb200_handle* h, int32_t which, float* normals4, float* desc33, int32_t cap, int32_t* n_out) {
  if (!h || !n_out || which < 0 || which > 1 || cap < 0) return QB200_ERR_BAD_ARG;
  cudaSetDevice(h->device);
  int n = 0, rc;
  if ((rc = get_counter(h, h->ctr.n_vox + which, &n))) return rc;
  *n_out = n;
  const int m = n < cap ? n : cap;
  if (m > 0) {
    if (normals4) QB_CUDA_TRY(h, cudaMemcpyAsync(normals4, h->normals + (size_t)which * h->V, (size_t)m * sizeof(float4), cudaMemcpyDeviceToHost, h->stream));
    if (desc33) {
      if ((rc = launch_desc_to_aos(h, which, m, h->aos_scratch))) return rc;
      QB_CUDA_TRY(h, cudaMemcpyAsync(desc33, h->aos_scratch, (size_t)m * kDescDim * sizeof(float), cudaMemcpyDeviceToHost, h->stream));
    }
    QB_CUDA_TRY(h, cudaStreamSynchronize(h->stream));
  }
  return n > cap ? QB200_CAPACITY_EXCEEDED : QB200_OK;
}

int qb200_get_stage_ms(qb200_handle* h, float* ms, int32_t n) {
  if (!h || !ms || n < 0) return QB200_ERR_BAD_ARG;
  for (int i = 0; i < n && i < 8; ++i) ms[i] = h->stage_ms[i];
  return QB200_OK;
}

int qb200_debug_match_verify(qb200_handle* h, uint64_t* out2, int32_t reset) {
  if (!h || !out2) return QB200_ERR_BAD_ARG;
  cudaSetDevice(h->device);
  QB_CUDA_TRY(h, cudaStreamSynchronize(h->stream));
  QB_CUDA_TRY(h, cudaMemcpy(out2, h->tc_stats + 4, 2 * sizeof(unsigned long long), cudaMemcpyDeviceToHost));
  if (reset) QB_CUDA_TRY(h, cudaMemset(h->tc_stats + 4, 0, 2 * sizeof(unsigned long long)));
  for (int l = 0; l < 7; ++l) {
    if (!h->lane[l]) continue;
    uint64_t o2[2];
    const int rc = qb200_debug_match_verify(h->lane[l], o2, reset);
    if (rc) return rc;
    out2[0] += o2[0]; out2[1] += o2[1];
  }
  return QB200_OK;
}

int qb200_debug_tc_profile(qb200_handle* h, uint64_t* out24, int32_t reset) {
  if (!h || !out24) return QB200_ERR_BAD_ARG;
  cudaSetDevice(h->device);
  QB_CUDA_TRY(h, cudaStreamSynchronize(h->stream));
  QB_CUDA_TRY(h, cudaMemcpy(out24, h->tc_stats + 8, 24 * sizeof(unsigned long long), cudaMemcpyDeviceToHost));
  if (reset) QB_CUDA_TRY(h, cudaMemset(h->tc_stats + 8, 0, 24 * sizeof(unsigned long long)));
  for (int l = 0; l < 7; ++l) {
    if (!h->lane[l]) continue;
    uint64_t o[24];
    const int rc = qb200_debug_tc_profile(h->lane[l], o, reset);
    if (rc) return rc;
    for (int i = 0; i < 24; ++i) out24[i] += o[i];
  }
  return QB200_OK;
}

int qb200_debug_match_stats(qb200_handle* h, uint64_t* out4, int32_t reset) {
  if (!h || !out4) return QB200_ERR_BAD_ARG;
  cudaSetDevice(h->device);
  QB_CUDA_TRY(h, cudaStreamSynchronize(h->stream));
  QB_CUDA_TRY(h, cudaMemcpy(out4, h->tc_stats, 4 * sizeof(unsigned long long), cudaMemcpyDeviceToHost));
  if (reset) QB_CUDA_TRY(h, cudaMemset(h->tc_stats, 0, 4 * sizeof(unsigned long long)));
  for (int l = 0; l < 7; ++l) {
    if (!h->lane[l]) continue;
    uint64_t o2[4];
    const int rc = qb200_debug_match_stats(h->lane[l], o2, reset);
    if (rc) return rc;
    for (int i = 0; i < 4; ++i) out4[i] += o2[i];
  }
  return QB200_OK;
}

int qb200_debug_tc_distances(qb200_handle* h, const float* a33, int32_t na, const float* b33, int32_t nb, float* out) {
  QB_IDLE(h);
  if (!h || !a33 || !b33 || !out || na < 1 || nb < 1 || na > 128 || nb > 128) return QB200_ERR_BAD_ARG;
  cudaSetDevice(h->device);
  int rc = wave_reset(h, 2);
  if (rc) return rc;
  if ((rc = set_counter(h, h->ctr.n_vox + 0, na))) return rc;
  if ((rc = set_counter(h, h->ctr.n_vox + 1, nb))) return rc;
  float* scratch = h->aos_scratch;
  QB_CUDA_TRY(h, cudaMemcpyAsync(scratch, a33, (size_t)na * kDescDim * sizeof(float), cudaMemcpyHostToDevice, h->stream));
  if ((rc = launch_desc_from_aos(h, 0, na, scratch))) return rc;
  float* scratch2 = scratch + (size_t)128 * kDescDim;
  QB_CUDA_TRY(h, cudaMemcpyAsync(scratch2, b33, (size_t)nb * kDescDim * sizeof(float), cudaMemcpyHostToDevice, h->stream));
  if ((rc = launch_desc_from_aos(h, 1, nb, scratch2))) return rc;
  float* d_out = h->spfh;
  QB_CUDA_TRY(h, cudaMemsetAsync(d_out, 0, 128 * 128 * sizeof(float), h->stream));
  if ((rc = launch_tc_debug_tile(h, d_out))) return rc;
  QB_CUDA_TRY(h, cudaMemcpyAsync(out, d_out, 128 * 128 * sizeof(float), cudaMemcpyDeviceToHost, h->stream));
  QB_CUDA_TRY(h, cudaStreamSynchronize(h->stream));
  return QB200_OK;
}

static void cache_free(qb200_handle* h) {
  if (h->c_vox) cudaFree(h->c_vox);
  if (h->c_nrm) cudaFree(h->c_nrm);
  if (h->c_desc) cudaFree(h->c_desc);
  if (h->c_n) cudaFree(h->c_n);
  if (h->c_status) cudaFree(h->c_status);
  if (h->d_slot_of_cloud) cudaFree(h->d_slot_of_cloud);
  if (h->h_slot_of_cloud) cudaFreeHost(h->h_slot_of_cloud);
  delete[] h->c_sig;
  h->c_vox = h->c_nrm = nullptr; h->c_desc = nullptr; h->c_n = h->c_status = h->d_slot_of_cloud = h->h_slot_of_cloud = nullptr;
  h->c_sig = nullptr;
  h->c_slots = 0;
}

int qb200_cache_reserve(qb200_handle* h, int32_t n_slots) {
  if (!h || n_slots < 0 || n_slots > (1 << 20)) return QB200_ERR_BAD_ARG;
  cudaSetDevice(h->device);
  QB_CUDA_TRY(h, cudaStreamSynchronize(h->stream));
  cache_free(h);
  if (n_slots == 0) return QB200_OK;
  const size_t V = h->V, N = (size_t)n_slots;
  QB_ALLOC(h, h->c_vox, N * V);
  QB_ALLOC(h, h->c_nrm, N * V);
  QB_ALLOC(h, h->c_desc, N * kDescK * V);
  QB_ALLOC(h, h->c_n, N);
  QB_ALLOC(h, h->c_status, N);
  QB_ALLOC(h, h->d_slot_of_cloud, 2 * (size_t)h->S);
  QB_CUDA_TRY(h, cudaMallocHost((void**)&h->h_slot_of_cloud, 2 * (size_t)h->S * sizeof(int)));
  QB_CUDA_TRY(h, cudaMemset(h->c_n, 0, N * sizeof(int)));
  QB_CUDA_TRY(h, cudaMemset(h->c_status, 0, N * sizeof(int)));
  QB_CUDA_TRY(h, cudaMemset(h->c_desc, 0, N * kDescK * V * sizeof(float)));
  h->c_sig = new (std::nothrow) float[4 * N]();
  if (!h->c_sig) return QB200_ERR_CUDA;
  h->c_slots = n_slots;
  return QB200_OK;
}

static int cache_copy(qb200_handle* h, int to_cache, int n_clouds) {
  QB_CUDA_TRY(h, cudaMemcpyAsync(h->d_slot_of_cloud, h->h_slot_of_cloud, (size_t)n_clouds * sizeof(int), cudaMemcpyHostToDevice, h->stream));
  const dim3 g((h->V + 255) / 256, 43, n_clouds);
  cache_copy_kernel<<<g, 256, 0, h->stream>>>(to_cache, h->d_slot_of_cloud, h->V, h->vox_pts, h->normals, h->desc_t, h->ctr.n_vox, h->ctr.cloud_status,
                                              h->c_vox, h->c_nrm, h->c_desc, h->c_n, h->c_status);
  h->launches++;
  QB_CUDA_TRY(h, cudaGetLastError());
  return QB200_OK;
}

int qb200_cache_scans(qb200_handle* h, const float* const* scans4, const int32_t* n_points, const int32_t* slot_ids, int32_t n_scans,
                      const qb200_params* p, qb200_mem_kind kind) {
  QB_IDLE(h);
  if (!h || n_scans < 0 || (n_scans > 0 && (!scans4 || !n_points || !slot_ids)) || !params_ok(p)) return QB200_ERR_BAD_ARG;
  for (int i = 0; i < n_scans; ++i)
    if (slot_ids[i] < 0 || slot_ids[i] >= h->c_slots || n_points[i] < 0 || n_points[i] > h->R || (n_points[i] > 0 && !scans4[i])) {
      h->fail(__FILE__, __LINE__, "scan is null, exceeds max_raw_points or names a slot outside qb200_cache_reserve()");
      return QB200_ERR_BAD_ARG;
    }
  cudaSetDevice(h->device);
  const float cell = lattice_cell(*p);
  const int C = 2 * h->S;
  for (int c0 = 0; c0 < n_scans; c0 += C) {
    const int nc = n_scans - c0 < C ? n_scans - c0 : C;
    int total = 0, rc;
    for (int c = 0; c < nc; ++c) {
      const int n = n_points[c0 + c];
      h->h_raw_off[c] = total;
      h->h_cloud_n[c] = n;
      h->h_slot_of_cloud[c] = slot_ids[c0 + c];
      if (kind == QB200_MEM_HOST) {
        h->h_cloud_ptr[c] = h->raw_stage + total;
        if (n > 0) QB_CUDA_TRY(h, cudaMemcpyAsync(h->raw_stage + total, scans4[c0 + c], (size_t)n * sizeof(float4), cudaMemcpyHostToDevice, h->stream));
      } else {
        h->h_cloud_ptr[c] = reinterpret_cast<const float4*>(scans4[c0 + c]);
      }
      total += n;
      float* sig = h->c_sig + 4 * (size_t)slot_ids[c0 + c];
      sig[0] = p->voxel_size; sig[1] = p->normal_radius; sig[2] = p->fpfh_radius; sig[3] = cell;
    }
    h->h_raw_off[nc] = total;
    QB_CUDA_TRY(h, cudaMemcpyAsync(h->d_cloud_ptr, h->h_cloud_ptr, (size_t)nc * sizeof(float4*), cudaMemcpyHostToDevice, h->stream));
    QB_CUDA_TRY(h, cudaMemcpyAsync(h->d_cloud_n, h->h_cloud_n, (size_t)nc * sizeof(int), cudaMemcpyHostToDevice, h->stream));
    QB_CUDA_TRY(h, cudaMemcpyAsync(h->d_raw_off, h->h_raw_off, (size_t)(nc + 1) * sizeof(int), cudaMemcpyHostToDevice, h->stream));
    if ((rc = wave_reset(h, nc))) return rc;
    if ((rc = launch_voxel(h, nc, p->voxel_size, p->skip_flagged))) return rc;
    if ((rc = launch_fpfh(h, nc, p->normal_radius, p->fpfh_radius, cell))) return rc;
    if ((rc = cache_copy(h, 1, nc))) return rc;
    QB_CUDA_TRY(h, cudaStreamSynchronize(h->stream));
  }
  return QB200_OK;
}

int qb200_register_cached(qb200_handle* h, const qb200_slot_pair* pairs, int32_t n_pairs, const qb200_params* p, qb200_result* results) {
  QB_IDLE(h);
  if (!h || n_pairs < 0 || (n_pairs > 0 && (!pairs || !results)) || !params_ok(p)) return QB200_ERR_BAD_ARG;
  if (!p->use_crosscheck) return QB200_ERR_UNSUPPORTED;
  const float cell = lattice_cell(*p);
  for (int i = 0; i < n_pairs; ++i) {
    const int sl[2] = {pairs[i].src_slot, pairs[i].tgt_slot};
    for (int k = 0; k < 2; ++k) {
      if (sl[k] < 0 || sl[k] >= h->c_slots) { h->fail(__FILE__, __LINE__, "slot outside qb200_cache_reserve()"); return QB200_ERR_BAD_ARG; }
      const float* sig = h->c_sig + 4 * (size_t)sl[k];
      if (sig[0] != p->voxel_size || sig[1] != p->normal_radius || sig[2] != p->fpfh_radius || sig[3] != cell) {
        h->fail(__FILE__, __LINE__, "cached scan was computed with other front-end parameters (or the slot is empty)");
        return QB200_ERR_BAD_ARG;
      }
    }
  }
  cudaSetDevice(h->device);
  qb200_params pr = *p;
  if (!(pr.rot_noise_bound > 0)) {
    if (h->rot_noise_bound_latched <= 0) h->rot_noise_bound_latched = 2.0 * p->noise_bound;
    pr.rot_noise_bound = h->rot_noise_bound_latched;
  }
  for (int i = 0; i < 8; ++i) h->stage_ms[i] = 0.f;
  for (int w0 = 0; w0 < n_pairs; w0 += h->S) {
    const int np = n_pairs - w0 < h->S ? n_pairs - w0 : h->S;
    int rc;
    for (int s = 0; s < np; ++s) {
      h->h_slot_of_cloud[2 * s] = pairs[w0 + s].src_slot;
      h->h_slot_of_cloud[2 * s + 1] = pairs[w0 + s].tgt_slot;
    }
    if ((rc = wave_reset(h, 2 * np))) return rc;
    cudaEventRecord(h->ev[2], h->stream);
    if ((rc = cache_copy(h, 0, 2 * np))) return rc;
    cudaEventRecord(h->ev[3], h->stream);
    if ((rc = launch_match(h, np, pr))) return rc;
    cudaEventRecord(h->ev[4], h->stream);
    cudaEventRecord(h->ev[5], h->stream);
    if ((rc = run_solver(h, np, pr, 1))) return rc;
    cudaEventRecord(h->ev[7], h->stream);
    QB_CUDA_TRY(h, cudaMemcpyAsync(h->h_results, h->d_results, (size_t)np * sizeof(qb200_result), cudaMemcpyDeviceToHost, h->stream));
    QB_CUDA_TRY(h, cudaStreamSynchronize(h->stream));
    memcpy(results + w0, h->h_results, (size_t)np * sizeof(qb200_result));
    for (int i = 2; i < 7; ++i) {
      float ms = 0.f;
      if (cudaEventElapsedTime(&ms, h->ev[i], h->ev[i + 1]) == cudaSuccess) h->stage_ms[i] += ms;
    }
  }
  if (n_pairs == 1) {
    h->last_n_corr = results[0].n_corr;
    h->last_n_clique = results[0].clique_size;
    h->last_n_final = results[0].n_final_inliers;
  }
  return QB200_OK;
}

int qb200_cache_copy(qb200_handle* h, int32_t from_slot, int32_t to_slot) {
  if (!h || from_slot < 0 || to_slot < 0 || from_slot >= h->c_slots || to_slot >= h->c_slots) return QB200_ERR_BAD_ARG;
  if (from_slot == to_slot) return QB200_OK;
  cudaSetDevice(h->device);
  const size_t V = h->V;
  QB_CUDA_TRY(h, cudaMemcpyAsync(h->c_vox + to_slot * V, h->c_vox + from_slot * V, V * sizeof(float4), cudaMemcpyDeviceToDevice, h->stream));
  QB_CUDA_TRY(h, cudaMemcpyAsync(h->c_nrm + to_slot * V, h->c_nrm + from_slot * V, V * sizeof(float4), cudaMemcpyDeviceToDevice, h->stream));
  QB_CUDA_TRY(h, cudaMemcpyAsync(h->c_desc + to_slot * kDescK * V, h->c_desc + from_slot * kDescK * V, kDescK * V * sizeof(float), cudaMemcpyDeviceToDevice, h->stream));
  QB_CUDA_TRY(h, cudaMemcpyAsync(h->c_n + to_slot, h->c_n + from_slot, sizeof(int), cudaMemcpyDeviceToDevice, h->stream));
  QB_CUDA_TRY(h, cudaMemcpyAsync(h->c_status + to_slot, h->c_status + from_slot, sizeof(int), cudaMemcpyDeviceToDevice, h->stream));
  memcpy(h->c_sig + 4 * (size_t)to_slot, h->c_sig + 4 * (size_t)from_slot, 4 * sizeof(float));
  QB_CUDA_TRY(h, cudaStreamSynchronize(h->stream));
  return QB200_OK;
}

int qb200_cache_read(qb200_handle* h, int32_t slot, float* vox4, float* normals4, float* desc33, int32_t cap, int32_t* n_out) {
  if (!h || !n_out || slot < 0 || slot >= h->c_slots || cap < 0) return QB200_ERR_BAD_ARG;
  cudaSetDevice(h->device);
  int n = 0, rc;
  if ((rc = get_counter(h, h->c_n + slot, &n))) return rc;
  *n_out = n;
  const int m = n < cap ? n : cap;
  const size_t V = h->V;
  if (m > 0) {
    if (vox4) QB_CUDA_TRY(h, cudaMemcpyAsync(vox4, h->c_vox + slot * V, (size_t)m * sizeof(float4), cudaMemcpyDeviceToHost, h->stream));
    if (normals4) QB_CUDA_TRY(h, cudaMemcpyAsync(normals4, h->c_nrm + slot * V, (size_t)m * sizeof(float4), cudaMemcpyDeviceToHost, h->stream));
    if (desc33) {
      desc_to_aos_rows(h, h->c_desc + slot * kDescK * V, m, h->aos_scratch);
      QB_CUDA_TRY(h, cudaMemcpyAsync(desc33, h->aos_scratch, (size_t)m * kDescDim * sizeof(float), cudaMemcpyDeviceToHost, h->stream));
    }
    QB_CUDA_TRY(h, cudaStreamSynchronize(h->stream));
  }
  return n > cap ? QB200_CAPACITY_EXCEEDED : QB200_OK;
}

int qb200_get_kernel_ms(qb200_handle* h, float* ms, int32_t* launches, int32_t n) {
  if (!h || !ms || n < 0) return QB200_ERR_BAD_ARG;
  for (int i = 0; i < n && i < 2; ++i) {
    ms[i] = h->kernel_ms[i];
    if (launches) launches[i] = h->kernel_calls[i];
  }
  return QB200_OK;
}

}

namespace qb {
int collect_batch(qb200_handle* h, const qb200_result* dst) {
  cudaSetDevice(h->device);
  return collect_batch_impl(h, dst);
}
}
```

quatro_b200/csrc/handle.cuh:

```cuda
#pragma once
#include <string.h>

#include "common.cuh"

struct qb200_handle {
  qb200_config cfg;
  int S, R, V, Lc, W;
  int NS;
  int device;
  int n_sm;
  cudaStream_t own_stream, stream;
  char err[512];
  int64_t launches;

  const float4** d_cloud_ptr;
  int* d_cloud_n;
  int* d_raw_off;
  const float4** h_cloud_ptr; int* h_cloud_n; int* h_raw_off;
  float4* raw_stage;
  qb200_handle* lane[7];
  int max_lanes;
  unsigned func_attr_set;
  int pend_w0, pend_np;
  qb200_result* pend_dst;
  int lanes_active, lane_cursor;
  cudaEvent_t ev_fork;
  cudaStream_t copy_stream;
  cudaEvent_t ev_copied;

  uint64_t *key_a, *key_b;
  uint32_t *val_a, *val_b;
  void* cub_temp; size_t cub_bytes;
  float* aos_scratch;

  int* vox_start;
  float4* vox_pts;
  uint64_t* cell_key;
  int* cell_start;
  float4* normals;
  float* spfh;
  uint32_t* nbr_list;
  int* nbr_cnt;
  float* desc_t;
  float* desc_tiles;
  float* desc_norm;
  int* tc_fallback;
  unsigned long long* tc_stats;
  int force_exact_match;
  unsigned long long* rowbest;
  unsigned long long* colpart;
  unsigned long long* colbest;
  int *mut_i, *mut_j;
  unsigned char* mark;
  int* partner;
  float* mean;
  int *corr_src, *corr_tgt;
  float4 *ma, *mb;
  uint32_t *adj, *adjp;
  int* deg;
  int *kcore, *korder, *rank_of, *by_rank, *kbin;
  int* clique;
  uint32_t *ex_stack, *ex_pool;
  int* ex_lvl;
  unsigned short* ex_cur;
  int* final_inl;
  unsigned char *rot_mask, *trans_mask;
  int* pw_ints;
  float4* pw_out;
  void* ip_buf; int ip_npix;
  qb200_result* d_results;
  qb200_result* h_results;
  qb::WaveCounters ctr;
  int* ctr_block; size_t ctr_ints;

  int c_slots;
  float4 *c_vox, *c_nrm;
  float* c_desc;
  int *c_n, *c_status;
  int *d_slot_of_cloud, *h_slot_of_cloud;
  float* c_sig;

  void* comm;
  int comm_world, comm_rank, comm_cap;
  cudaStream_t comm_stream;
  cudaEvent_t comm_done;
  qb200_result *d_send, *d_recv, *h_send, *h_recv;
  int pend_gather_n;
  qb200_result* pend_gather_dst;
  int pipe_n, pipe_buf;
  qb200_result* pipe_dst;

  double rot_noise_bound_latched;
  int last_n_corr, last_n_clique, last_n_final;

  cudaEvent_t ev[9];
  float stage_ms[8];
  cudaEvent_t kev[4];
  float kernel_ms[2];
  int kernel_calls[2];
  int kev_armed[2];

  void fail(const char* file, int line, const char* msg) {
    snprintf(err, sizeof(err), "%s:%d: %s", file, line, msg);
  }
};

namespace qb {

int launch_voxel(qb200_handle* h, int n_clouds, float leaf, int skip_flagged);
int launch_fpfh(qb200_handle* h, int n_clouds, float normal_radius, float fpfh_radius, float cell);
int launch_match(qb200_handle* h, int n_pairs, const qb200_params& p);
int launch_graph(qb200_handle* h, int n_pairs, double noise_bound, double cbar2);
int launch_clique(qb200_handle* h, int n_pairs, int mode, double kcore_thr, long long node_limit);
int launch_pose(qb200_handle* h, int n_pairs, const qb200_params& p);
int launch_fill_counters(qb200_handle* h, int n_pairs, int have_frontend);
int launch_finalize_status(qb200_handle* h, int n_pairs);
int launch_iota_clique(qb200_handle* h, int n_pairs);
int launch_segment_cloud(qb200_handle* h, const float4* pts, int n, const qb200_segment_params& sp, int* n_valid, int* n_outlier,
                         const float4** valid_dev, const float4** outlier_dev);
int launch_patchwork(qb200_handle* h, const float4* pts, int n, const qb200_patchwork_params& pp, int* n_ground, int* n_nonground, int* status);
int launch_match_nn(qb200_handle* h, int n_pairs);
int launch_match_exact(qb200_handle* h, int n_pairs, const int* only);
int launch_tc_debug_tile(qb200_handle* h, float* d_out);
int launch_desc_to_aos(qb200_handle* h, int cloud, int n, float* d_out33);
int launch_desc_from_aos(qb200_handle* h, int cloud, int n, const float* d_in33);
int desc_to_aos_rows(qb200_handle* h, const float* desc_rows, int n, float* d_out33);
size_t sort_temp_bytes(int max_items);
void comm_release(qb200_handle* h);
int collect_batch(qb200_handle* h, const qb200_result* dst);
int ensure_dyn_smem(qb200_handle* h, const void* kernel, size_t bytes);
int sort_pairs(qb200_handle* h, int n_items, int end_bit);
int launch_voxel_sort(qb200_handle* h, int n_clouds, float inv_leaf, int skip_flagged, int idx_bits);
int launch_cloud_sort(qb200_handle* h, int n_clouds, const int* n_items, int f1, int f2);

}
```

quatro_b200/csrc/tc_match.cu:

```cuda
#include "handle.cuh"
#include <cstdlib>

namespace qb {

constexpr int kTcM = 128, kTcN = 128;
constexpr int kTcKB = kDescK / 8;
constexpr int kTcTileBytes = kDescK * 128 * 4;
constexpr int kTileFloats = kDescK * 128;
constexpr int kTcImages = 3;
constexpr int kTcEpiWarps = 16;
constexpr int kTcThreads = (kTcEpiWarps + 2) * 32;
constexpr int kTcDone = 4;
constexpr int kTcStages = 4;
constexpr float kTcC = 1.2e-4f;
constexpr int kSpinLimit = 400000;

__device__ __forceinline__ uint32_t smem_u32(const void* p) { return (uint32_t)__cvta_generic_to_shared(p); }

__device__ __forceinline__ uint64_t tc_smem_desc(uint32_t addr) {
  return (uint64_t)((addr & 0x3FFFF) >> 4) | ((uint64_t)(2048 >> 4) << 16) | ((uint64_t)(128 >> 4) << 32);
}

__device__ __forceinline__ void wgmma_tf32_64x64x8(float (&d)[32], uint64_t adesc, uint64_t bdesc, int accumulate) {
  asm volatile(
      "{\n\t"
      ".reg .pred p;\n\t"
      "setp.ne.b32 p, %34, 0;\n\t"
      "wgmma.mma_async.sync.aligned.m64n64k8.f32.tf32.tf32 "
      "{%0, %1, %2, %3, %4, %5, %6, %7, %8, %9, %10, %11, %12, %13, %14, %15, "
      "%16, %17, %18, %19, %20, %21, %22, %23, %24, %25, %26, %27, %28, %29, %30, %31}, %32, %33, p, 1, 1;\n\t"
      "}\n"
      : "+f"(d[0]), "+f"(d[1]), "+f"(d[2]), "+f"(d[3]), "+f"(d[4]), "+f"(d[5]), "+f"(d[6]), "+f"(d[7]), "+f"(d[8]), "+f"(d[9]),
        "+f"(d[10]), "+f"(d[11]), "+f"(d[12]), "+f"(d[13]), "+f"(d[14]), "+f"(d[15]), "+f"(d[16]), "+f"(d[17]), "+f"(d[18]),
        "+f"(d[19]), "+f"(d[20]), "+f"(d[21]), "+f"(d[22]), "+f"(d[23]), "+f"(d[24]), "+f"(d[25]), "+f"(d[26]), "+f"(d[27]),
        "+f"(d[28]), "+f"(d[29]), "+f"(d[30]), "+f"(d[31])
      : "l"(adesc), "l"(bdesc), "r"(accumulate)
      : "memory");
}

__device__ __forceinline__ bool wg_all(bool v, int g) {
  uint32_t r;
  asm volatile(
      "{\n\t.reg .pred p, q;\n\t"
      "setp.ne.u32 p, %1, 0;\n\t"
      "bar.red.and.pred q, %2, 128, p;\n\t"
      "selp.u32 %0, 1, 0, q;\n\t}\n"
      : "=r"(r)
      : "r"((uint32_t)v), "r"(1 + g)
      : "memory");
  return r != 0;
}

__device__ __forceinline__ float tc_mu(int d) { return (d == 5 || d == 16 || d == 27) ? 100.0f : 0.0f; }

__global__ void __launch_bounds__(256) norm_key_kernel(const float* __restrict__ desc_t, const int* __restrict__ n_vox, int V,
                                                       uint64_t* __restrict__ keys, uint32_t* __restrict__ vals) {
  const int cloud = blockIdx.y;
  const int q = blockIdx.x * blockDim.x + threadIdx.x;
  if (q >= V) return;
  uint32_t bits = 0xFFFFFFFFu;
  if (q < n_vox[cloud]) {
    const size_t base = (size_t)cloud * kDescK * V + q;
    float acc = 0.0f;
#pragma unroll
    for (int d = 0; d < kDescDim; ++d) {
      const float xc = desc_t[base + (size_t)d * V] - tc_mu(d);
      acc = __fmaf_rn(xc, xc, acc);
    }
    bits = acc == acc ? __float_as_uint(acc) : 0xFFFFFFFEu;
  }
  keys[(size_t)cloud * V + q] = ((uint64_t)cloud << 32) | bits;
  vals[(size_t)cloud * V + q] = (uint32_t)q;
}

__global__ void __launch_bounds__(256) split_desc_kernel(const float* __restrict__ desc_t, const int* __restrict__ n_vox, int V,
                                                         const uint32_t* __restrict__ perm, float* __restrict__ tiles,
                                                         float* __restrict__ norm) {
  const int cloud = blockIdx.y;
  const int q = blockIdx.x * blockDim.x + threadIdx.x;
  const int n = n_vox[cloud];
  const int NB = V >> 7;
  if (q >= ((n + 127) & ~127)) return;
  const size_t base = (size_t)cloud * kDescK * V + (q < n ? perm[(size_t)cloud * V + q] : 0u);
  const int blk = q >> 7, p = q & 127;
  float4* __restrict__ img = reinterpret_cast<float4*>(tiles + (size_t)(cloud * NB + blk) * kTcImages * kTileFloats) + p;
  const bool is_col = (cloud & 1) != 0;
  const float kLow = 1.0f - 0.5f * kTcC;
  float acc = 0.0f;
#pragma unroll
  for (int kc = 0; kc < kDescK / 4; ++kc) {
    float xv[4], hv[4], lv[4];
#pragma unroll
    for (int e = 0; e < 4; ++e) {
      const int d = 4 * kc + e;
      const bool live = d < kDescDim && q < n;
      const float x = live ? desc_t[base + (size_t)d * V] : 0.0f;
      const float xc = live ? x - tc_mu(d) : 0.0f;
      xv[e] = x;
      acc = __fmaf_rn(xc, xc, acc);
      float xs = is_col ? -2.0f * xc : xc;
      if (q < n && d == kDescDim) xs = is_col ? 1.0f : kLow * acc;
      if (q < n && d == kDescDim + 1) xs = is_col ? kLow * acc : 1.0f;
      hv[e] = __uint_as_float(__float_as_uint(xs) & 0xFFFFE000u);
      lv[e] = __uint_as_float(__float_as_uint(xs - hv[e]) & 0xFFFFE000u);
    }
    img[0 * (kTileFloats / 4) + kc * 128] = make_float4(hv[0], hv[1], hv[2], hv[3]);
    img[1 * (kTileFloats / 4) + kc * 128] = make_float4(lv[0], lv[1], lv[2], lv[3]);
    if (kc < kDescK / 4 - 1) img[2 * (kTileFloats / 4) + kc * 128] = make_float4(xv[0], xv[1], xv[2], xv[3]);
  }
  img[2 * (kTileFloats / 4) + (kDescK / 4 - 1) * 128] = make_float4(q < n ? kLow * acc : INFINITY, 0.0f, 0.0f, 0.0f);
  if (q < n) norm[(size_t)cloud * V + q] = acc;
}

__global__ void __launch_bounds__(1024) dedup_kernel(const float* __restrict__ desc_t, const int* __restrict__ n_vox, int V,
                                                     const uint64_t* __restrict__ sorted_keys, const uint32_t* __restrict__ perm, int enable,
                                                     uint32_t* __restrict__ uperm, uint32_t* __restrict__ class_of, int* __restrict__ n_unique) {
  __shared__ int scan_smem[33];
  const int cloud = blockIdx.x;
  const int n = n_vox[cloud];
  const float* __restrict__ D = desc_t + (size_t)cloud * kDescK * V;
  const uint32_t* __restrict__ pm = perm + (size_t)cloud * V;
  const uint64_t* __restrict__ sk = sorted_keys + (size_t)cloud * V;
  int base = 0;
  for (int start = 0; start < n; start += blockDim.x) {
    const int r = start + threadIdx.x;
    int flag = 0;
    if (r < n) {
      flag = 1;
      if (enable && r > 0 && sk[r] == sk[r - 1]) {
        const uint32_t a = pm[r], b = pm[r - 1];
        bool same = true;
#pragma unroll
        for (int g = 0; g < 3; ++g) {
          if (!same) break;
          unsigned diff = 0;
#pragma unroll
          for (int j = 0; j < 11; ++j) {
            const int d = 11 * g + j;
            diff |= __float_as_uint(D[(size_t)d * V + a]) ^ __float_as_uint(D[(size_t)d * V + b]);
          }
          same = diff == 0;
        }
        flag = same ? 0 : 1;
      }
    }
    int total;
    const int ex = block_excl_scan(flag, scan_smem, &total);
    if (r < n) {
      const int u = base + ex + flag - 1;
      class_of[(size_t)cloud * V + r] = (uint32_t)u;
      if (flag) uperm[(size_t)cloud * V + u] = pm[r];
    }
    base += total;
  }
  if (threadIdx.x == 0) n_unique[cloud] = base;
}

__global__ void __launch_bounds__(256) broadcast_best_kernel(const unsigned long long* __restrict__ rowbest_u,
                                                             const unsigned long long* __restrict__ colbest_u, const int* __restrict__ n_vox,
                                                             int V, const uint32_t* __restrict__ perm, const uint32_t* __restrict__ class_of,
                                                             unsigned long long* __restrict__ rowbest, unsigned long long* __restrict__ colbest) {
  const int cloud = blockIdx.y, pair = cloud >> 1;
  const int r = blockIdx.x * blockDim.x + threadIdx.x;
  if (r >= n_vox[cloud]) return;
  const uint32_t u = class_of[(size_t)cloud * V + r], q = perm[(size_t)cloud * V + r];
  if (cloud & 1) colbest[(size_t)pair * V + q] = colbest_u[(size_t)pair * V + u];
  else rowbest[(size_t)pair * V + q] = rowbest_u[(size_t)pair * V + u];
}

__device__ __forceinline__ void mbar_init(uint32_t bar, int count) {
  asm volatile("mbarrier.init.shared::cta.b64 [%0], %1;\n" ::"r"(bar), "r"(count) : "memory");
}
__device__ __forceinline__ void mbar_expect_tx(uint32_t bar, uint32_t bytes) {
  asm volatile("mbarrier.arrive.expect_tx.shared::cta.b64 _, [%0], %1;\n" ::"r"(bar), "r"(bytes) : "memory");
}
__device__ __forceinline__ void bulk_g2s(uint32_t dst, const void* src, uint32_t bytes, uint32_t bar) {
  asm volatile("cp.async.bulk.shared::cluster.global.mbarrier::complete_tx::bytes [%0], [%1], %2, [%3];\n" ::"r"(dst), "l"(src), "r"(bytes),
               "r"(bar)
               : "memory");
}
__device__ __forceinline__ bool mbar_wait(uint32_t bar, uint32_t parity) {
  for (int spin = 0; spin < kSpinLimit; ++spin) {
    uint32_t ok;
    asm volatile(
        "{\n\t.reg .pred p;\n\t"
        "mbarrier.try_wait.parity.shared::cta.b64 p, [%1], %2;\n\t"
        "selp.u32 %0, 1, 0, p;\n\t}\n"
        : "=r"(ok)
        : "r"(bar), "r"(parity)
        : "memory");
    if (ok) return true;
  }
  return false;
}

__device__ __forceinline__ unsigned long long tc_pack(float d, int idx) {
  return ((unsigned long long)__float_as_uint(d) << 32) | (unsigned)idx;
}

__device__ __forceinline__ void mbar_arrive(uint32_t bar) {
  asm volatile("mbarrier.arrive.shared::cta.b64 _, [%0];\n" ::"r"(bar) : "memory");
}
__device__ __forceinline__ unsigned tc_fkey(float f) {
  unsigned key = __float_as_uint(f);
  key = (key & 0x80000000u) ? ~key : (key | 0x80000000u);
  return f == f ? key : 0xFFFFFFFFu;
}
__device__ __forceinline__ float tc_fkey_inv(unsigned key) { return __uint_as_float((key & 0x80000000u) ? (key & 0x7FFFFFFFu) : ~key); }

template <bool kDbg, bool kProf = false>
__global__ void __launch_bounds__(kTcThreads, 1)
tc_nn_kernel(const float* __restrict__ tiles, const float* __restrict__ norm, const int* __restrict__ n_vox, int V,
             const uint32_t* __restrict__ perm, unsigned long long* __restrict__ rowbest, unsigned long long* __restrict__ colbest_r,
             unsigned* __restrict__ tile_cmax, int* __restrict__ fallback, unsigned long long* __restrict__ stats,
             float* __restrict__ dbg_tile) {
  extern __shared__ __align__(128) unsigned char smem[];
  __shared__ uint64_t s_fullx[kTcStages], s_sfree[kTcStages], s_fullhl[2], s_mma[kTcDone], s_afull;
  __shared__ unsigned long long s_rbest[kTcM];
  __shared__ __align__(16) float s_wcj[kTcEpiWarps][64];
  __shared__ unsigned short s_queue[kTcEpiWarps][32];
  __shared__ int s_seq[8];
  __shared__ float s_tlb[128];
  __shared__ int s_dead, s_abort, s_evals, s_warm, s_npos;
  __shared__ int s_ndec;

  const int pair = blockIdx.y, stripe = blockIdx.x;
  const int cloudA = 2 * pair, cloudB = 2 * pair + 1;
  const int nA = n_vox[cloudA], nB = n_vox[cloudB];
  const int r0 = stripe * kTcM;
  if (r0 >= nA || nB <= 0) return;

  const int warp = threadIdx.x >> 5, lane = threadIdx.x & 31;
  const int NB = V >> 7;
  auto tick = [&]() -> long long { return kProf ? clock64() : 0ll; };
  auto prof = [&](int slot, long long cyc) { if (kProf && lane == 0) atomicAdd(stats + slot, (unsigned long long)cyc); };
  const long long t_begin = tick();
  constexpr uint32_t kABytes = kTcImages * kTcTileBytes;
  constexpr uint32_t kHLBytes = 2 * kTcTileBytes;
  constexpr uint32_t kXBytes = kTcTileBytes;
  const uint32_t sA = smem_u32(smem), sHL0 = sA + kABytes, sX0 = sHL0 + 2 * kHLBytes;
  const float* __restrict__ tA = tiles + (size_t)cloudA * NB * kTcImages * kTileFloats;
  const float* __restrict__ tB = tiles + (size_t)cloudB * NB * kTcImages * kTileFloats;
  const float* __restrict__ nrmA = norm + (size_t)cloudA * V;
  const float* __restrict__ nrmB = norm + (size_t)cloudB * V;
  const uint32_t* __restrict__ permA = perm + (size_t)cloudA * V;
  const uint32_t* __restrict__ permB = perm + (size_t)cloudB * V;
  unsigned long long* __restrict__ cbg = colbest_r + (size_t)pair * V;
  const uint32_t bar_fullx0 = smem_u32(&s_fullx[0]), bar_sfree0 = smem_u32(&s_sfree[0]), bar_fullhl0 = smem_u32(&s_fullhl[0]),
                 bar_mma0 = smem_u32(&s_mma[0]), bar_a = smem_u32(&s_afull);
  const int n_tiles = (nB + kTcN - 1) / kTcN;

  if (threadIdx.x == 0) {
    for (int i = 0; i < kTcStages; ++i) { mbar_init(bar_fullx0 + 8 * i, 1); mbar_init(bar_sfree0 + 8 * i, kTcEpiWarps); }
    for (int i = 0; i < 2; ++i) mbar_init(bar_fullhl0 + 8 * i, 1);
    for (int i = 0; i < kTcDone; ++i) mbar_init(bar_mma0 + 8 * i, kTcEpiWarps);
    mbar_init(bar_a, 1);
    s_dead = 0; s_abort = 0; s_evals = 0; s_warm = 0; s_npos = 0; s_ndec = 0;
    asm volatile("fence.mbarrier_init.release.cluster;\n" ::: "memory");
  }
  if (threadIdx.x < kTcM) s_rbest[threadIdx.x] = ~0ull;
  __syncthreads();
  const long long t_setup = tick();
  if (kProf && threadIdx.x == 0) { atomicAdd(stats + 8, 1ull); atomicAdd(stats + 10, (unsigned long long)(t_setup - t_begin)); }
  volatile int* v_dead = &s_dead;
  volatile int* v_abort = &s_abort;
  volatile int* v_seq = s_seq;
  volatile int* v_ndec = &s_ndec;
  auto wait_decided = [&](int n) -> bool {
    for (int spin = 0; spin < kSpinLimit; ++spin) {
      if (*v_ndec > n) { __threadfence_block(); return true; }
      __nanosleep(32);
    }
    return false;
  };
  volatile unsigned long long* v_rbest = s_rbest;

  if (warp == kTcEpiWarps) {
    auto issue_hl = [&](int n) {
      const int t = v_seq[n & 7];
      if (lane != 0) return;
      const uint32_t bar = bar_fullhl0 + 8 * (n & 1);
      if (t < 0) { mbar_arrive(bar); return; }
      mbar_expect_tx(bar, kHLBytes);
      bulk_g2s(sHL0 + (n & 1) * kHLBytes, tB + (size_t)t * kTcImages * kTileFloats, kHLBytes, bar);
    };
    if (lane == 0) {
      mbar_expect_tx(bar_a, kABytes);
      bulk_g2s(sA, tA + (size_t)stripe * kTcImages * kTileFloats, kABytes, bar_a);
    }
    bool ok = wait_decided(0);
    if (ok) { issue_hl(0); ok = wait_decided(1); }
    if (ok) issue_hl(1);
    long long p_wm = 0, p_wd = 0;
    bool ended = !ok || v_seq[0] < 0 || v_seq[1] < 0;
    for (int k = 0; ok && !ended; ++k) {
      const long long t0 = tick();
      ok = mbar_wait(bar_mma0 + 8 * (k & (kTcDone - 1)), (uint32_t)((k >> 2) & 1));
      const long long t1 = tick();
      p_wm += t1 - t0;
      if (ok) ok = wait_decided(k + 2);
      p_wd += tick() - t1;
      if (!ok) break;
      issue_hl(k + 2);
      ended = v_seq[(k + 2) & 7] < 0;
    }
    prof(12, p_wm); prof(28, p_wd);
    if (!ok) *v_dead = 1;
  } else if (warp == kTcEpiWarps + 1) {
    const float amin = sqrtf(nrmA[r0]), amax = sqrtf(nrmA[(r0 + kTcM < nA ? r0 + kTcM : nA) - 1]);
    auto tile_lb = [&](int t) -> float {
      const float bmin = sqrtf(nrmB[t * kTcN]), bmax = sqrtf(nrmB[(t * kTcN + kTcN < nB ? t * kTcN + kTcN : nB) - 1]);
      const float gap = fmaxf(amin - bmax, bmin - amax) - 2.0e-3f;
      if (!(amin <= amax && bmin <= bmax)) return 0.0f;
      return gap > 0.0f ? gap * gap * 0.9999f : 0.0f;
    };
    const uint4* __restrict__ tcm4 = reinterpret_cast<const uint4*>(tile_cmax) + (size_t)pair * (V >> 7);
    uint4 pq0, pq1, pq2, pq3;
    auto fetch_tcm = [&]() {
      pq0 = pq1 = pq2 = pq3 = make_uint4(0xFFFFFFFFu, 0xFFFFFFFFu, 0xFFFFFFFFu, 0xFFFFFFFFu);
      if (lane < n_tiles) pq0 = __ldcg(tcm4 + lane);
      if (lane + 32 < n_tiles) pq1 = __ldcg(tcm4 + lane + 32);
      if (lane + 64 < n_tiles) pq2 = __ldcg(tcm4 + lane + 64);
      if (lane + 96 < n_tiles) pq3 = __ldcg(tcm4 + lane + 96);
    };
    auto max4 = [](const uint4& q) -> unsigned { return max(max(q.x, q.y), max(q.z, q.w)); };
    fetch_tcm();
    int t0 = 0;
    {
      float best = INFINITY;
      for (int t = lane; t < n_tiles; t += 32) {
        const float g = tile_lb(t);
        if (t < 128) s_tlb[t] = g;
        if (g < best) { best = g; t0 = t; }
      }
      const unsigned key = __reduce_min_sync(0xffffffffu, tc_fkey(best));
      const unsigned who = __ballot_sync(0xffffffffu, tc_fkey(best) == key);
      t0 = __shfl_sync(0xffffffffu, t0, __ffs(who) - 1);
      __syncwarp();
    }
    auto tlb = [&](int t) -> float { return t < 128 ? s_tlb[t] : tile_lb(t); };
    int lo = t0 - 1, hi = t0 + 1;
    bool first = true, done = false;
    auto next_tile = [&]() -> int {
      if (first) { first = false; return t0; }
      unsigned rmax = 0;
#pragma unroll
      for (int i = 0; i < kTcM / 32; ++i) {
        const int row = lane + 32 * i;
        if (r0 + row < nA) {
          const unsigned long long rb = v_rbest[row];
          rmax = max(rmax, rb == ~0ull ? 0x7F800000u : (unsigned)(rb >> 32));
        }
      }
      const float rmaxf = __uint_as_float(__reduce_max_sync(0xffffffffu, rmax));
      const unsigned tc0 = max4(pq0), tc1 = max4(pq1), tc2 = max4(pq2), tc3 = max4(pq3);
      if (*v_abort || *v_dead) return -1;
      const bool is_left = lane < 16;
      while (true) {
        if (lo < 0 && hi >= n_tiles) return -1;
        const int t = is_left ? lo - lane : hi + (lane - 16);
        const bool valid = is_left ? t >= 0 : t < n_tiles;
        const float lb = valid ? tlb(t) : INFINITY;
        unsigned cm = 0xFFFFFFFFu;
        {
          const int src = t & 31, sl = (t >> 5) & 3;
          const unsigned a0 = __shfl_sync(0xffffffffu, tc0, src), a1 = __shfl_sync(0xffffffffu, tc1, src);
          const unsigned a2 = __shfl_sync(0xffffffffu, tc2, src), a3 = __shfl_sync(0xffffffffu, tc3, src);
          if (valid && t < 128) cm = sl == 0 ? a0 : sl == 1 ? a1 : sl == 2 ? a2 : a3;
          else if (valid) cm = max4(__ldcg(tcm4 + t));
        }
        const bool visit = valid && (lb <= 0.0f || !(lb > rmaxf) || !(lb > __uint_as_float(cm)));
        const unsigned vb = __ballot_sync(0xffffffffu, visit);
        const int fl = (vb & 0xFFFFu) ? __ffs(vb & 0xFFFFu) - 1 : 16;
        const int fr = (vb >> 16) ? __ffs(vb >> 16) - 1 : 16;
        if (fl == 16 && fr == 16) { lo -= 16; hi += 16; continue; }
        const float gl = __shfl_sync(0xffffffffu, lb, fl & 15), gh = __shfl_sync(0xffffffffu, lb, 16 + (fr & 15));
        const bool left = fr == 16 || (fl < 16 && gl <= gh);
        const int tv = left ? lo - fl : hi + fr;
        lo -= left ? fl + 1 : fl;
        hi += left ? fr : fr + 1;
        return tv;
      }
    };
    int n_issued = 0;
    auto decide = [&](int n) {
      int t = -1;
      if (!done) {
        t = next_tile();
        if (t < 0) done = true; else ++n_issued;
      }
      if (lane == 0) {
        v_seq[n & 7] = t;
        __threadfence_block();
        *v_ndec = n + 1;
      }
      __syncwarp();
      if (!done) fetch_tcm();
      return t;
    };
    auto issue_x = [&](int n) {
      const int t = v_seq[n & 7];
      if (lane != 0) return;
      const uint32_t bar = bar_fullx0 + 8 * (n & (kTcStages - 1));
      if (t < 0) { mbar_arrive(bar); return; }
      mbar_expect_tx(bar, kXBytes);
      bulk_g2s(sX0 + (n & (kTcStages - 1)) * kXBytes, tB + ((size_t)t * kTcImages + 2) * kTileFloats, kXBytes, bar);
    };
    for (int n = 0; n < 3; ++n) { decide(n); issue_x(n); }
    prof(11, tick() - t_setup);
    long long p_wm = 0, p_dec = 0, p_sf = 0;
    auto mbar_test = [&](uint32_t bar, uint32_t parity) -> bool {
      uint32_t ready;
      asm volatile(
          "{\n\t.reg .pred p;\n\t"
          "mbarrier.test_wait.parity.shared::cta.b64 p, [%1], %2;\n\t"
          "selp.u32 %0, 1, 0, p;\n\t}\n"
          : "=r"(ready)
          : "r"(bar), "r"(parity)
          : "memory");
      return __all_sync(0xffffffffu, ready != 0);
    };
    int nd = 3, nx = 3;
    bool ok = true, end_decided = v_seq[0] < 0 || v_seq[1] < 0 || v_seq[2] < 0;
    if (end_decided) nx = nd;
    int idle = 0;
    long long t_idle = 0;
    while (ok && !(end_decided && nx == nd)) {
      const uint32_t bar_s = bar_sfree0 + 8 * (nx & (kTcStages - 1)), par_s = (uint32_t)(((nx - 4) >> 2) & 1);
      const uint32_t bar_m = bar_mma0 + 8 * ((nd - 3) & (kTcDone - 1)), par_m = (uint32_t)(((nd - 3) >> 2) & 1);
      const bool can_x = nx < nd, can_d = !end_decided && nd < nx + 4;
      if (can_x && (nx < 4 || mbar_test(bar_s, par_s))) {
        if (kProf && idle) { (can_d ? p_wm : p_sf) += tick() - t_idle; }
        idle = 0;
        issue_x(nx);
        ++nx;
        continue;
      }
      if (can_d && mbar_test(bar_m, par_m)) {
        const long long t1 = tick();
        if (kProf && idle) { (can_x ? p_wm : p_sf) += t1 - t_idle; }
        idle = 0;
        if (decide(nd) < 0) end_decided = true;
        ++nd;
        p_dec += tick() - t1;
        continue;
      }
      if (idle == 0) t_idle = tick();
      if (++idle > kSpinLimit) { ok = false; break; }
      __nanosleep(32);
    }
    prof(29, p_wm); prof(13, p_dec); prof(14, p_sf);
    if (!ok) *v_dead = 1;
    if (lane == 0) s_npos = n_issued;
  } else {
    const int wg = warp >> 2;
    const int rbase = (wg & 1) * 64 + 16 * (warp & 3);
    const int cb = (wg >> 1) * 64;
    const int cl = 2 * (lane & 3);
    const float kLow = 1.0f - 0.5f * kTcC;
    const float kW = kTcC / kLow;
    bool row_ok[2];
    float nam[2], Ri_ub[2];
    unsigned oa[2];
#pragma unroll
    for (int h = 0; h < 2; ++h) {
      const int gi = r0 + rbase + (lane >> 2) + 8 * h;
      row_ok[h] = gi < nA;
      nam[h] = row_ok[h] ? kLow * nrmA[gi] : INFINITY;
      oa[h] = row_ok[h] ? permA[gi] : 0u;
      Ri_ub[h] = row_ok[h] ? INFINITY : -INFINITY;
    }
    const uint32_t row_bits = (row_ok[0] ? 0x33333333u : 0u) | (row_ok[1] ? 0xCCCCCCCCu : 0u);
    const float4* __restrict__ aex = reinterpret_cast<const float4*>(smem + 2 * kTcTileBytes);
    const uint32_t aH = sA + (uint32_t)((wg & 1) * 64 * 16), aL = aH + kTcTileBytes;
    float* wcj = s_wcj[warp];
    unsigned short* wq = s_queue[warp];
    int evals_w = 0;
    bool alive = mbar_wait(bar_a, 0);
    const long long t_loop = tick();
    prof(19, t_loop - t_setup);
    long long p_wx = 0, p_wmm = 0, p_ld = 0, p_prep = 0, p_fil = 0, p_ev = 0;
    int p_tiles = 0;
    int pf_tile = -1;
    unsigned long long pf_cb[2] = {~0ull, ~0ull};
    unsigned pf_ob[2] = {0u, 0u};
    unsigned* __restrict__ tcmw = tile_cmax + ((size_t)pair * (V >> 7)) * 4 + (cb >> 5);
    int rr_tile = -1;
    unsigned rr_val[2] = {0u, 0u};
    auto rr_flush = [&]() {
      if (rr_tile < 0) return;
#pragma unroll
      for (int s = 0; s < 2; ++s) {
        const unsigned m = __reduce_max_sync(0xffffffffu, rr_val[s]);
        if (lane == 0) atomicMin(tcmw + (size_t)rr_tile * 4 + s, m);
      }
      rr_tile = -1;
    };
    for (int k = 0;; ++k) {
      const int ts = k & (kTcDone - 1), st = k & (kTcStages - 1), hs = k & 1;
      const long long q0 = tick();
      if (alive) alive = mbar_wait(bar_fullx0 + 8 * st, (uint32_t)((k >> 2) & 1));
      const long long q1 = tick();
      p_wx += q1 - q0;
      alive = __all_sync(0xffffffffu, alive);
      const int jt = alive ? v_seq[k & 7] : -1;
      const int c0 = jt * kTcN;
      unsigned long long cb_cur[2] = {~0ull, ~0ull};
      unsigned ob[2] = {0u, 0u};
      if (jt >= 0) {
        if (pf_tile == jt) {
#pragma unroll
          for (int s = 0; s < 2; ++s) { cb_cur[s] = pf_cb[s]; ob[s] = pf_ob[s]; }
        } else {
#pragma unroll
          for (int s = 0; s < 2; ++s)
            if (c0 + cb + 32 * s + lane < nB) {
              cb_cur[s] = __ldcg(cbg + c0 + cb + 32 * s + lane);
              ob[s] = permB[c0 + cb + 32 * s + lane];
            }
        }
        pf_tile = -1;
        if (__all_sync(0xffffffffu, *v_ndec > k + 1)) {
          const int jn = v_seq[(k + 1) & 7];
          if (jn >= 0) {
            pf_tile = jn;
#pragma unroll
            for (int s = 0; s < 2; ++s) {
              pf_cb[s] = ~0ull; pf_ob[s] = 0u;
              if (jn * kTcN + cb + 32 * s + lane < nB) {
                pf_cb[s] = __ldcg(cbg + jn * kTcN + cb + 32 * s + lane);
                pf_ob[s] = permB[jn * kTcN + cb + 32 * s + lane];
              }
            }
          }
        }
      }
      const long long q2 = tick();
      if (alive && jt >= 0) alive = mbar_wait(bar_fullhl0 + 8 * hs, (uint32_t)((k >> 1) & 1));
      alive = __all_sync(0xffffffffu, alive);
      if (!wg_all(alive && jt >= 0, wg)) {
        if (!alive) *v_dead = 1;
        break;
      }
      float d[32];
#pragma unroll
      for (int i = 0; i < 32; ++i) d[i] = 0.0f;
      {
        const uint32_t bH = sHL0 + hs * kHLBytes + (uint32_t)(cb * 16), bL = bH + kTcTileBytes;
        asm volatile("wgmma.fence.sync.aligned;\n" ::: "memory");
#pragma unroll
        for (int kb = 0; kb < kTcKB; ++kb) {
          wgmma_tf32_64x64x8(d, tc_smem_desc(aH + kb * 4096), tc_smem_desc(bL + kb * 4096), kb > 0);
          wgmma_tf32_64x64x8(d, tc_smem_desc(aL + kb * 4096), tc_smem_desc(bH + kb * 4096), 1);
        }
#pragma unroll
        for (int kb = 0; kb < kTcKB; ++kb) wgmma_tf32_64x64x8(d, tc_smem_desc(aH + kb * 4096), tc_smem_desc(bH + kb * 4096), 1);
        asm volatile("wgmma.commit_group.sync.aligned;\n" ::: "memory");
        asm volatile("wgmma.wait_group.sync.aligned 0;\n" ::: "memory");
#pragma unroll
        for (int i = 0; i < 32; ++i) asm volatile("" : "+f"(d[i])::"memory");
      }
      __syncwarp();
      if (lane == 0) mbar_arrive(bar_mma0 + 8 * ts);
      const long long q3 = tick();
      p_wmm += q3 - q2;
      p_prep += q2 - q1;
      ++p_tiles;
      const bool skip = __any_sync(0xffffffffu, (*v_abort | *v_dead) != 0);
      const long long q4 = tick();
      p_ld += q4 - q3;
      if (!skip) {
        const float4* __restrict__ bex = reinterpret_cast<const float4*>(smem + kABytes + 2 * kHLBytes + st * kXBytes);
        float dbest[2];
        bool col_warm = false;
#pragma unroll
        for (int s = 0; s < 2; ++s) {
          const float nbm = bex[9 * 128 + cb + 32 * s + lane].x;
          dbest[s] = cb_cur[s] == ~0ull ? INFINITY : __uint_as_float((unsigned)(cb_cur[s] >> 32));
          wcj[32 * s + lane] = nbm == INFINITY ? -INFINITY : dbest[s];
          col_warm |= cb_cur[s] == ~0ull && nbm != INFINITY;
        }
        float Ri[2];
        bool row_warm = false;
#pragma unroll
        for (int h = 0; h < 2; ++h) {
          const unsigned long long rb = v_rbest[rbase + (lane >> 2) + 8 * h];
          Ri[h] = fminf(Ri_ub[h], rb == ~0ull ? INFINITY : __uint_as_float((unsigned)(rb >> 32)));
          row_warm |= row_ok[h] && Ri[h] == INFINITY;
        }
        __syncwarp();
        if (__any_sync(0xffffffffu, row_warm || col_warm)) {
          if (lane == 0) atomicAdd(&s_warm, 1);
          float rowub[2] = {INFINITY, INFINITY};
#pragma unroll
          for (int i = 0; i < 32; i += 4) {
#pragma unroll
            for (int e = 0; e < 2; ++e) {
              const int c = 2 * i + cl + e;
              const float nbc = bex[9 * 128 + cb + c].x;
              const float ub0 = fmaf(kW, nam[0] + nbc, d[i + e]), ub1 = fmaf(kW, nam[1] + nbc, d[i + 2 + e]);
              rowub[0] = fminf(rowub[0], ub0);
              rowub[1] = fminf(rowub[1], ub1);
              unsigned mn = min(ub0 >= 0.0f ? __float_as_uint(ub0) : 0xFFFFFFFFu, ub1 >= 0.0f ? __float_as_uint(ub1) : 0xFFFFFFFFu);
              mn = min(mn, __shfl_xor_sync(0xffffffffu, mn, 4));
              mn = min(mn, __shfl_xor_sync(0xffffffffu, mn, 8));
              mn = min(mn, __shfl_xor_sync(0xffffffffu, mn, 16));
              if (lane < 4 && mn != 0xFFFFFFFFu && nbc != INFINITY) wcj[c] = fminf(wcj[c], __uint_as_float(mn));
            }
          }
#pragma unroll
          for (int h = 0; h < 2; ++h) {
            rowub[h] = fminf(rowub[h], __shfl_xor_sync(0xffffffffu, rowub[h], 1));
            rowub[h] = fminf(rowub[h], __shfl_xor_sync(0xffffffffu, rowub[h], 2));
            if (row_ok[h]) { Ri_ub[h] = fminf(Ri_ub[h], rowub[h]); Ri[h] = fminf(Ri[h], Ri_ub[h]); }
          }
        }
        __syncwarp();
        const long long q5 = tick();
        p_prep += q5 - q4;
        const int ncol = nB - c0 - cb;
        uint32_t mask = 0, col_bits = 0;
#pragma unroll
        for (int i = 0; i < 32; i += 4) {
          const float2 x = *reinterpret_cast<const float2*>(wcj + 2 * i + cl);
#pragma unroll
          for (int e = 0; e < 4; ++e) {
            const float lbv = d[i + e];
            const float xc = (e & 1) ? x.y : x.x;
            asm("{\n\t.reg .pred p, q;\n\t"
                "setp.le.f32 p, %1, %2;\n\t"
                "setp.le.or.f32 q, %1, %3, p;\n\t"
                "@q or.b32 %0, %0, %4;\n\t}\n"
                : "+r"(mask)
                : "f"(lbv), "f"(xc), "f"(Ri[e >> 1]), "r"(1u << (i + e)));
            if (2 * i + cl + (e & 1) < ncol) col_bits |= 1u << (i + e);
            if (kDbg) {
              const int h = e >> 1, c = 2 * i + cl + (e & 1);
              if (stripe == 0 && k == 0 && row_ok[h] && c < ncol)
                dbg_tile[(size_t)oa[h] * kTcN + permB[c0 + cb + c]] = fmaf(0.5f * kW, nam[h] + bex[9 * 128 + cb + c].x, lbv);
            }
          }
        }
        mask &= col_bits & row_bits;
        int remaining = __reduce_add_sync(0xffffffffu, __popc(mask));
        const long long q6 = tick();
        p_fil += q6 - q5;
        evals_w += remaining;
        while (remaining > 0) {
          int tot;
          int p = warp_excl_scan(__popc(mask), &tot);
          while (mask && p < 32) {
            const int i = __ffs(mask) - 1;
            mask &= mask - 1;
            wq[p++] = (unsigned short)((lane << 5) | i);
          }
          __syncwarp();
          const int nb = tot < 32 ? tot : 32;
          const int q = lane < nb ? wq[lane] : 0;
          const int sl = q >> 5, i = q & 31, h = (i >> 1) & 1;
          const int rr = rbase + (sl >> 2) + 8 * h;
          const int c = 8 * (i >> 2) + 2 * (sl & 3) + (i & 1);
          const int pcol = cb + c;
          float acc = 0.0f;
#pragma unroll
          for (int kc = 0; kc < (kDescDim + 3) / 4; ++kc) {
            const float4 a = aex[kc * 128 + rr], b = bex[kc * 128 + pcol];
            float diff = a.x - b.x;
            acc = __fmaf_rn(diff, diff, acc);
            if (4 * kc + 1 < kDescDim) { diff = a.y - b.y; acc = __fmaf_rn(diff, diff, acc); }
            if (4 * kc + 2 < kDescDim) { diff = a.z - b.z; acc = __fmaf_rn(diff, diff, acc); }
            if (4 * kc + 3 < kDescDim) { diff = a.w - b.w; acc = __fmaf_rn(diff, diff, acc); }
          }
          const float db0 = __shfl_sync(0xffffffffu, dbest[0], c & 31), db1 = __shfl_sync(0xffffffffu, dbest[1], c & 31);
          const unsigned ob0 = __shfl_sync(0xffffffffu, ob[0], c & 31), ob1 = __shfl_sync(0xffffffffu, ob[1], c & 31);
          const unsigned oa0 = __shfl_sync(0xffffffffu, oa[0], sl & ~3), oa1 = __shfl_sync(0xffffffffu, oa[1], sl & ~3);
          const float dbc = c < 32 ? db0 : db1;
          const unsigned oc = c < 32 ? ob0 : ob1;
          const unsigned orow = h ? oa1 : oa0;
          if (lane < nb && acc == acc) {
            const unsigned long long pr = tc_pack(acc, (int)oc);
            if (pr < v_rbest[rr]) atomicMin(&s_rbest[rr], pr);
            if (acc <= dbc) atomicMin(cbg + c0 + pcol, tc_pack(acc, (int)orow));
          }
          __syncwarp();
          remaining = tot - nb;
        }
        if (lane == 0 && evals_w) {
          const int seen = atomicAdd(&s_evals, evals_w) + evals_w;
          if (k >= 7 && seen > (k + 1) * (kTcM * kTcN / 2)) *v_abort = 1;
        }
        evals_w = 0;
        p_ev += tick() - q6;
      }
      __syncwarp();
      if (lane == 0) mbar_arrive(bar_sfree0 + 8 * st);
      rr_flush();
      if (!skip) {
        rr_tile = jt;
#pragma unroll
        for (int s = 0; s < 2; ++s) {
          rr_val[s] = 0;
          if (c0 + cb + 32 * s + lane < nB) {
            const unsigned long long cbn = __ldcg(cbg + c0 + cb + 32 * s + lane);
            rr_val[s] = cbn == ~0ull ? 0x7F800000u : (unsigned)(cbn >> 32);
          }
        }
      }
    }
    rr_flush();
    prof(20, p_wx); prof(21, p_wmm); prof(22, p_ld); prof(23, p_prep); prof(24, p_fil); prof(25, p_ev);
    prof(26, tick() - t_loop); prof(27, p_tiles);
  }
  __syncthreads();
  const bool aborted = (s_abort | s_dead) != 0;
  if (kProf && threadIdx.x == 0) atomicAdd(stats + 9, (unsigned long long)(tick() - t_begin));
  if (threadIdx.x == 0) {
    atomicAdd(stats + 0, (unsigned long long)s_evals);
    atomicAdd(stats + 1, (unsigned long long)s_npos);
    atomicAdd(stats + 2, (unsigned long long)s_warm);
    if (aborted) {
      atomicAdd(stats + 3, 1ull);
      fallback[pair] = 1;
    }
  }
  if (!aborted && threadIdx.x < kTcM && r0 + (int)threadIdx.x < nA) rowbest[(size_t)pair * V + r0 + threadIdx.x] = s_rbest[threadIdx.x];
}

static size_t tc_smem_bytes() { return (size_t)kTcImages * kTcTileBytes + 2 * 2 * (size_t)kTcTileBytes + (size_t)kTcStages * kTcTileBytes; }

static int sort_and_dedup(qb200_handle* h, int n_clouds, int dedup) {
  const int V = h->V;
  const dim3 g((V + 255) / 256, n_clouds);
  norm_key_kernel<<<g, 256, 0, h->stream>>>(h->desc_t, h->ctr.n_vox, V, h->key_a, h->val_a);
  h->launches += 1;
  int bits = 0;
  while ((1 << bits) < n_clouds) ++bits;
  int rc = launch_cloud_sort(h, n_clouds, h->ctr.n_vox, 32, 32);
  if (rc == QB200_ERR_UNSUPPORTED) rc = sort_pairs(h, n_clouds * V, 32 + bits);
  if (rc) return rc;
  uint32_t* class_of = reinterpret_cast<uint32_t*>(h->key_a);
  int* n_unique = reinterpret_cast<int*>(class_of + (size_t)2 * h->S * V);
  dedup_kernel<<<n_clouds, 1024, 0, h->stream>>>(h->desc_t, h->ctr.n_vox, V, h->key_b, h->val_b, dedup, h->val_a, class_of, n_unique);
  h->launches += 1;
  QB_CUDA_TRY(h, cudaGetLastError());
  return QB200_OK;
}

int launch_match_nn(qb200_handle* h, int n_pairs) {
  const int V = h->V;
  const size_t smem = tc_smem_bytes();
  if (int rc = ensure_dyn_smem(h, (const void*)tc_nn_kernel<false>, smem)) return rc;
  int rc = sort_and_dedup(h, 2 * n_pairs, 1);
  if (rc) return rc;
  const uint32_t* uperm = h->val_a;
  const uint32_t* class_of = reinterpret_cast<const uint32_t*>(h->key_a);
  const int* n_unique = reinterpret_cast<const int*>(class_of + (size_t)2 * h->S * V);
  unsigned long long* colbest_u = h->colpart;
  unsigned long long* rowbest_u = h->colpart + (size_t)h->S * V;
  unsigned* tile_cmax = reinterpret_cast<unsigned*>(h->colpart + (size_t)2 * h->S * V);
  QB_CUDA_TRY(h, cudaMemsetAsync(h->rowbest, 0xFF, (size_t)n_pairs * V * 8, h->stream));
  QB_CUDA_TRY(h, cudaMemsetAsync(h->colbest, 0xFF, (size_t)n_pairs * V * 8, h->stream));
  QB_CUDA_TRY(h, cudaMemsetAsync(h->colpart, 0xFF, ((size_t)2 * h->S * V + (size_t)h->S * (V >> 7) * 2 + 2) * 8, h->stream));
  QB_CUDA_TRY(h, cudaMemsetAsync(h->tc_fallback, 0, (size_t)n_pairs * sizeof(int), h->stream));
  const dim3 gsplit((V + 255) / 256, 2 * n_pairs);
  split_desc_kernel<<<gsplit, 256, 0, h->stream>>>(h->desc_t, n_unique, V, uperm, h->desc_tiles, h->desc_norm);
  const dim3 g(h->NS, n_pairs);
  cudaEventRecord(h->kev[0], h->stream);
  static const int tc_prof = (getenv("QB200_TC_PROF") && getenv("QB200_TC_PROF")[0] == '1') ? 1 : 0;
  if (tc_prof) {
    if (int rc2 = ensure_dyn_smem(h, (const void*)tc_nn_kernel<false, true>, smem)) return rc2;
    tc_nn_kernel<false, true><<<g, kTcThreads, smem, h->stream>>>(h->desc_tiles, h->desc_norm, n_unique, V, uperm, rowbest_u, colbest_u,
                                                                  tile_cmax, h->tc_fallback, h->tc_stats, nullptr);
  } else {
    tc_nn_kernel<false><<<g, kTcThreads, smem, h->stream>>>(h->desc_tiles, h->desc_norm, n_unique, V, uperm, rowbest_u, colbest_u,
                                                            tile_cmax, h->tc_fallback, h->tc_stats, nullptr);
  }
  cudaEventRecord(h->kev[1], h->stream);
  h->kev_armed[0] = 1;
  broadcast_best_kernel<<<gsplit, 256, 0, h->stream>>>(rowbest_u, colbest_u, h->ctr.n_vox, V, h->val_b, class_of, h->rowbest, h->colbest);
  h->launches += 3;
  QB_CUDA_TRY(h, cudaGetLastError());
  return launch_match_exact(h, n_pairs, h->tc_fallback);
}

int launch_tc_debug_tile(qb200_handle* h, float* d_out) {
  const size_t smem = tc_smem_bytes();
  if (int rc0 = ensure_dyn_smem(h, (const void*)tc_nn_kernel<true>, smem)) return rc0;
  int rc = sort_and_dedup(h, 2, 0);
  if (rc) return rc;
  const uint32_t* uperm = h->val_a;
  const int* n_unique = reinterpret_cast<const int*>(reinterpret_cast<const uint32_t*>(h->key_a) + (size_t)2 * h->S * h->V);
  QB_CUDA_TRY(h, cudaMemsetAsync(h->colpart, 0xFF, ((size_t)2 * h->S * h->V + (size_t)h->S * (h->V >> 7) * 2 + 2) * 8, h->stream));
  QB_CUDA_TRY(h, cudaMemsetAsync(h->tc_fallback, 0, sizeof(int), h->stream));
  const dim3 gsplit((h->V + 255) / 256, 2);
  split_desc_kernel<<<gsplit, 256, 0, h->stream>>>(h->desc_t, n_unique, h->V, uperm, h->desc_tiles, h->desc_norm);
  const dim3 g(1, 1);
  tc_nn_kernel<true><<<g, kTcThreads, smem, h->stream>>>(h->desc_tiles, h->desc_norm, n_unique, h->V, uperm, h->colpart + (size_t)h->S * h->V,
                                                         h->colpart, reinterpret_cast<unsigned*>(h->colpart + (size_t)2 * h->S * h->V), h->tc_fallback, h->tc_stats, d_out);
  h->launches += 2;
  QB_CUDA_TRY(h, cudaGetLastError());
  return QB200_OK;
}

}
```

Before: 12120.

## Shrink TC NN tiles to 128x64 and fit two CTAs per SM

Narrows the column tile of the tensor-core nearest-neighbour kernel from 128 to 64, halves the epilogue warps, drops the H/L buffer from double to single, and cuts X stages from four to two. The shared-memory footprint shrinks so launch bounds can request two CTAs per SM, with the max-shared carveout set explicitly. The goal is to hide latency through more resident CTAs instead of deeper per-CTA pipelining. The cost is less prefetch depth per CTA and a single HL buffer that serialises loads against MMA. A footprint debug API is also added.

```diff
diff --git a/include/quatro_b200.h b/include/quatro_b200.h
--- a/include/quatro_b200.h
+++ b/include/quatro_b200.h
@@ -235,6 +235,7 @@
 
 int qb200_debug_match_stats(qb200_handle* h, uint64_t* out4, int32_t reset);
 int qb200_debug_tc_profile(qb200_handle* h, uint64_t* out24, int32_t reset);
+int qb200_debug_tc_footprint(qb200_handle* h, int32_t* out5);
 
 int qb200_debug_match_verify(qb200_handle* h, uint64_t* out2, int32_t reset);
 
diff --git a/quatro_b200/capi.py b/quatro_b200/capi.py
--- a/quatro_b200/capi.py
+++ b/quatro_b200/capi.py
@@ -149,6 +149,7 @@
         "qb200_register_batch_enqueue": (i32, [vp, vp, i32, vp, i32, vp]),
         "qb200_register_batch_flush": (i32, [vp]),
         "qb200_debug_tc_profile": (i32, [vp, vp, i32]),
+        "qb200_debug_tc_footprint": (i32, [vp, vp]),
         "qb200_solve_batch": (i32, [vp, vp, i32, vp, i32, vp]),
         "qb200_comm_init_all": (i32, [P(vp), i32]),
         "qb200_register_batch_sharded": (i32, [P(vp), i32, P(Pair), i32, P(Params), i32, vp]),
@@ -184,6 +185,7 @@
     "qb200_register_batch_enqueue",
     "qb200_register_batch_flush",
     "qb200_debug_tc_profile",
+    "qb200_debug_tc_footprint",
     "qb200_solve_batch",
     "qb200_comm_init_all", "qb200_register_batch_sharded", "qb200_comm_unique_id", "qb200_comm_init_rank",
     "qb200_register_batch_rank", "qb200_comm_wait", "qb200_bind_numa",
@@ -534,6 +536,12 @@
         self._check(self.lib.qb200_debug_tc_profile(self.h, _ptr(out), int(reset)), "qb200_debug_tc_profile")
         return out
 
+    def debug_tc_footprint(self) -> dict:
+        out = np.zeros(5, np.int32)
+        self._check(self.lib.qb200_debug_tc_footprint(self.h, _ptr(out)), "qb200_debug_tc_footprint")
+        return {"threads": int(out[0]), "dyn_smem": int(out[1]), "static_smem": int(out[2]), "regs": int(out[3]),
+                "ctas_per_sm": int(out[4])}
+
     def debug_match_verify(self, reset: bool = True) -> dict:
         out = np.zeros(2, np.uint64)
         self._check(self.lib.qb200_debug_match_verify(self.h, _ptr(out), int(reset)), "qb200_debug_match_verify")
diff --git a/quatro_b200/csrc/api.cu b/quatro_b200/csrc/api.cu
--- a/quatro_b200/csrc/api.cu
+++ b/quatro_b200/csrc/api.cu
@@ -1027,6 +1027,12 @@
   return QB200_OK;
 }
 
+int qb200_debug_tc_footprint(qb200_handle* h, int32_t* out5) {
+  if (!h || !out5) return QB200_ERR_BAD_ARG;
+  cudaSetDevice(h->device);
+  return tc_footprint(h, out5);
+}
+
 int qb200_debug_tc_distances(qb200_handle* h, const float* a33, int32_t na, const float* b33, int32_t nb, float* out) {
   QB_IDLE(h);
   if (!h || !a33 || !b33 || !out || na < 1 || nb < 1 || na > 128 || nb > 128) return QB200_ERR_BAD_ARG;
diff --git a/quatro_b200/csrc/handle.cuh b/quatro_b200/csrc/handle.cuh
--- a/quatro_b200/csrc/handle.cuh
+++ b/quatro_b200/csrc/handle.cuh
@@ -122,6 +122,7 @@
 int launch_match_nn(qb200_handle* h, int n_pairs);
 int launch_match_exact(qb200_handle* h, int n_pairs, const int* only);
 int launch_tc_debug_tile(qb200_handle* h, float* d_out);
+int tc_footprint(qb200_handle* h, int* out5);
 int launch_desc_to_aos(qb200_handle* h, int cloud, int n, float* d_out33);
 int launch_desc_from_aos(qb200_handle* h, int cloud, int n, const float* d_in33);
 int desc_to_aos_rows(qb200_handle* h, const float* desc_rows, int n, float* d_out33);
diff --git a/quatro_b200/csrc/tc_match.cu b/quatro_b200/csrc/tc_match.cu
--- a/quatro_b200/csrc/tc_match.cu
+++ b/quatro_b200/csrc/tc_match.cu
@@ -3,22 +3,24 @@
 
 namespace qb {
 
-constexpr int kTcM = 128, kTcN = 128;
+constexpr int kTcM = 128, kTcN = 64;
+constexpr int kTcBlk = 64;
 constexpr int kTcKB = kDescK / 8;
-constexpr int kTcTileBytes = kDescK * 128 * 4;
-constexpr int kTileFloats = kDescK * 128;
+constexpr int kTcTileBytes = kDescK * kTcBlk * 4;
+constexpr int kTileFloats = kDescK * kTcBlk;
 constexpr int kTcImages = 3;
-constexpr int kTcEpiWarps = 16;
+constexpr int kTcEpiWarps = 8;
 constexpr int kTcThreads = (kTcEpiWarps + 2) * 32;
 constexpr int kTcDone = 4;
-constexpr int kTcStages = 4;
+constexpr int kTcStages = 2;
+constexpr int kTcSmemTiles = 256;
 constexpr float kTcC = 1.2e-4f;
 constexpr int kSpinLimit = 400000;
 
 __device__ __forceinline__ uint32_t smem_u32(const void* p) { return (uint32_t)__cvta_generic_to_shared(p); }
 
 __device__ __forceinline__ uint64_t tc_smem_desc(uint32_t addr) {
-  return (uint64_t)((addr & 0x3FFFF) >> 4) | ((uint64_t)(2048 >> 4) << 16) | ((uint64_t)(128 >> 4) << 32);
+  return (uint64_t)((addr & 0x3FFFF) >> 4) | ((uint64_t)((kTcBlk * 16) >> 4) << 16) | ((uint64_t)(128 >> 4) << 32);
 }
 
 __device__ __forceinline__ void wgmma_tf32_64x64x8(float (&d)[32], uint64_t adesc, uint64_t bdesc, int accumulate) {
@@ -79,10 +81,10 @@
   const int cloud = blockIdx.y;
   const int q = blockIdx.x * blockDim.x + threadIdx.x;
   const int n = n_vox[cloud];
-  const int NB = V >> 7;
-  if (q >= ((n + 127) & ~127)) return;
+  const int NB = V / kTcBlk;
+  if (q >= ((n + kTcM - 1) & ~(kTcM - 1))) return;
   const size_t base = (size_t)cloud * kDescK * V + (q < n ? perm[(size_t)cloud * V + q] : 0u);
-  const int blk = q >> 7, p = q & 127;
+  const int blk = q / kTcBlk, p = q % kTcBlk;
   float4* __restrict__ img = reinterpret_cast<float4*>(tiles + (size_t)(cloud * NB + blk) * kTcImages * kTileFloats) + p;
   const bool is_col = (cloud & 1) != 0;
   const float kLow = 1.0f - 0.5f * kTcC;
@@ -104,11 +106,11 @@
       hv[e] = __uint_as_float(__float_as_uint(xs) & 0xFFFFE000u);
       lv[e] = __uint_as_float(__float_as_uint(xs - hv[e]) & 0xFFFFE000u);
     }
-    img[0 * (kTileFloats / 4) + kc * 128] = make_float4(hv[0], hv[1], hv[2], hv[3]);
-    img[1 * (kTileFloats / 4) + kc * 128] = make_float4(lv[0], lv[1], lv[2], lv[3]);
-    if (kc < kDescK / 4 - 1) img[2 * (kTileFloats / 4) + kc * 128] = make_float4(xv[0], xv[1], xv[2], xv[3]);
+    img[0 * (kTileFloats / 4) + kc * kTcBlk] = make_float4(hv[0], hv[1], hv[2], hv[3]);
+    img[1 * (kTileFloats / 4) + kc * kTcBlk] = make_float4(lv[0], lv[1], lv[2], lv[3]);
+    if (kc < kDescK / 4 - 1) img[2 * (kTileFloats / 4) + kc * kTcBlk] = make_float4(xv[0], xv[1], xv[2], xv[3]);
   }
-  img[2 * (kTileFloats / 4) + (kDescK / 4 - 1) * 128] = make_float4(q < n ? kLow * acc : INFINITY, 0.0f, 0.0f, 0.0f);
+  img[2 * (kTileFloats / 4) + (kDescK / 4 - 1) * kTcBlk] = make_float4(q < n ? kLow * acc : INFINITY, 0.0f, 0.0f, 0.0f);
   if (q < n) norm[(size_t)cloud * V + q] = acc;
 }
 
@@ -209,18 +211,18 @@
 __device__ __forceinline__ float tc_fkey_inv(unsigned key) { return __uint_as_float((key & 0x80000000u) ? (key & 0x7FFFFFFFu) : ~key); }
 
 template <bool kDbg, bool kProf = false>
-__global__ void __launch_bounds__(kTcThreads, 1)
+__global__ void __launch_bounds__(kTcThreads, 2)
 tc_nn_kernel(const float* __restrict__ tiles, const float* __restrict__ norm, const int* __restrict__ n_vox, int V,
              const uint32_t* __restrict__ perm, unsigned long long* __restrict__ rowbest, unsigned long long* __restrict__ colbest_r,
              unsigned* __restrict__ tile_cmax, int* __restrict__ fallback, unsigned long long* __restrict__ stats,
              float* __restrict__ dbg_tile) {
   extern __shared__ __align__(128) unsigned char smem[];
-  __shared__ uint64_t s_fullx[kTcStages], s_sfree[kTcStages], s_fullhl[2], s_mma[kTcDone], s_afull;
+  __shared__ uint64_t s_fullx[kTcStages], s_sfree[kTcStages], s_fullhl, s_mma[kTcDone], s_afull;
   __shared__ unsigned long long s_rbest[kTcM];
-  __shared__ __align__(16) float s_wcj[kTcEpiWarps][64];
+  __shared__ __align__(16) float s_wcj[kTcEpiWarps][kTcN];
   __shared__ unsigned short s_queue[kTcEpiWarps][32];
   __shared__ int s_seq[8];
-  __shared__ float s_tlb[128];
+  __shared__ float s_tlb[kTcSmemTiles];
   __shared__ int s_dead, s_abort, s_evals, s_warm, s_npos;
   __shared__ int s_ndec;
 
@@ -231,14 +233,14 @@
   if (r0 >= nA || nB <= 0) return;
 
   const int warp = threadIdx.x >> 5, lane = threadIdx.x & 31;
-  const int NB = V >> 7;
+  const int NB = V / kTcBlk;
   auto tick = [&]() -> long long { return kProf ? clock64() : 0ll; };
   auto prof = [&](int slot, long long cyc) { if (kProf && lane == 0) atomicAdd(stats + slot, (unsigned long long)cyc); };
   const long long t_begin = tick();
-  constexpr uint32_t kABytes = kTcImages * kTcTileBytes;
+  constexpr uint32_t kABytes = (kTcM / kTcBlk) * kTcImages * kTcTileBytes;
   constexpr uint32_t kHLBytes = 2 * kTcTileBytes;
   constexpr uint32_t kXBytes = kTcTileBytes;
-  const uint32_t sA = smem_u32(smem), sHL0 = sA + kABytes, sX0 = sHL0 + 2 * kHLBytes;
+  const uint32_t sA = smem_u32(smem), sHL = sA + kABytes, sX0 = sHL + kHLBytes;
   const float* __restrict__ tA = tiles + (size_t)cloudA * NB * kTcImages * kTileFloats;
   const float* __restrict__ tB = tiles + (size_t)cloudB * NB * kTcImages * kTileFloats;
   const float* __restrict__ nrmA = norm + (size_t)cloudA * V;
@@ -246,13 +248,13 @@
   const uint32_t* __restrict__ permA = perm + (size_t)cloudA * V;
   const uint32_t* __restrict__ permB = perm + (size_t)cloudB * V;
   unsigned long long* __restrict__ cbg = colbest_r + (size_t)pair * V;
-  const uint32_t bar_fullx0 = smem_u32(&s_fullx[0]), bar_sfree0 = smem_u32(&s_sfree[0]), bar_fullhl0 = smem_u32(&s_fullhl[0]),
+  const uint32_t bar_fullx0 = smem_u32(&s_fullx[0]), bar_sfree0 = smem_u32(&s_sfree[0]), bar_fullhl = smem_u32(&s_fullhl),
                  bar_mma0 = smem_u32(&s_mma[0]), bar_a = smem_u32(&s_afull);
   const int n_tiles = (nB + kTcN - 1) / kTcN;
 
   if (threadIdx.x == 0) {
     for (int i = 0; i < kTcStages; ++i) { mbar_init(bar_fullx0 + 8 * i, 1); mbar_init(bar_sfree0 + 8 * i, kTcEpiWarps); }
-    for (int i = 0; i < 2; ++i) mbar_init(bar_fullhl0 + 8 * i, 1);
+    mbar_init(bar_fullhl, 1);
     for (int i = 0; i < kTcDone; ++i) mbar_init(bar_mma0 + 8 * i, kTcEpiWarps);
     mbar_init(bar_a, 1);
     s_dead = 0; s_abort = 0; s_evals = 0; s_warm = 0; s_npos = 0; s_ndec = 0;
@@ -279,30 +281,28 @@
     auto issue_hl = [&](int n) {
       const int t = v_seq[n & 7];
       if (lane != 0) return;
-      const uint32_t bar = bar_fullhl0 + 8 * (n & 1);
-      if (t < 0) { mbar_arrive(bar); return; }
-      mbar_expect_tx(bar, kHLBytes);
-      bulk_g2s(sHL0 + (n & 1) * kHLBytes, tB + (size_t)t * kTcImages * kTileFloats, kHLBytes, bar);
+      if (t < 0) { mbar_arrive(bar_fullhl); return; }
+      mbar_expect_tx(bar_fullhl, kHLBytes);
+      bulk_g2s(sHL, tB + (size_t)t * kTcImages * kTileFloats, kHLBytes, bar_fullhl);
     };
     if (lane == 0) {
       mbar_expect_tx(bar_a, kABytes);
-      bulk_g2s(sA, tA + (size_t)stripe * kTcImages * kTileFloats, kABytes, bar_a);
+      bulk_g2s(sA, tA + (size_t)stripe * (kTcM / kTcBlk) * kTcImages * kTileFloats, kABytes, bar_a);
     }
     bool ok = wait_decided(0);
-    if (ok) { issue_hl(0); ok = wait_decided(1); }
-    if (ok) issue_hl(1);
+    if (ok) issue_hl(0);
     long long p_wm = 0, p_wd = 0;
-    bool ended = !ok || v_seq[0] < 0 || v_seq[1] < 0;
+    bool ended = !ok || v_seq[0] < 0;
     for (int k = 0; ok && !ended; ++k) {
       const long long t0 = tick();
       ok = mbar_wait(bar_mma0 + 8 * (k & (kTcDone - 1)), (uint32_t)((k >> 2) & 1));
       const long long t1 = tick();
       p_wm += t1 - t0;
-      if (ok) ok = wait_decided(k + 2);
+      if (ok) ok = wait_decided(k + 1);
       p_wd += tick() - t1;
       if (!ok) break;
-      issue_hl(k + 2);
-      ended = v_seq[(k + 2) & 7] < 0;
+      issue_hl(k + 1);
+      ended = v_seq[(k + 1) & 7] < 0;
     }
     prof(12, p_wm); prof(28, p_wd);
     if (!ok) *v_dead = 1;
@@ -314,23 +314,20 @@
       if (!(amin <= amax && bmin <= bmax)) return 0.0f;
       return gap > 0.0f ? gap * gap * 0.9999f : 0.0f;
     };
-    const uint4* __restrict__ tcm4 = reinterpret_cast<const uint4*>(tile_cmax) + (size_t)pair * (V >> 7);
-    uint4 pq0, pq1, pq2, pq3;
+    constexpr int kPq = kTcSmemTiles / 32;
+    const uint2* __restrict__ tcm2 = reinterpret_cast<const uint2*>(tile_cmax) + (size_t)pair * (V / kTcN);
+    uint2 pq[kPq];
     auto fetch_tcm = [&]() {
-      pq0 = pq1 = pq2 = pq3 = make_uint4(0xFFFFFFFFu, 0xFFFFFFFFu, 0xFFFFFFFFu, 0xFFFFFFFFu);
-      if (lane < n_tiles) pq0 = __ldcg(tcm4 + lane);
-      if (lane + 32 < n_tiles) pq1 = __ldcg(tcm4 + lane + 32);
-      if (lane + 64 < n_tiles) pq2 = __ldcg(tcm4 + lane + 64);
-      if (lane + 96 < n_tiles) pq3 = __ldcg(tcm4 + lane + 96);
+#pragma unroll
+      for (int i = 0; i < kPq; ++i) pq[i] = lane + 32 * i < n_tiles ? __ldcg(tcm2 + lane + 32 * i) : make_uint2(0xFFFFFFFFu, 0xFFFFFFFFu);
     };
-    auto max4 = [](const uint4& q) -> unsigned { return max(max(q.x, q.y), max(q.z, q.w)); };
     fetch_tcm();
     int t0 = 0;
     {
       float best = INFINITY;
       for (int t = lane; t < n_tiles; t += 32) {
         const float g = tile_lb(t);
-        if (t < 128) s_tlb[t] = g;
+        if (t < kTcSmemTiles) s_tlb[t] = g;
         if (g < best) { best = g; t0 = t; }
       }
       const unsigned key = __reduce_min_sync(0xffffffffu, tc_fkey(best));
@@ -338,7 +335,7 @@
       t0 = __shfl_sync(0xffffffffu, t0, __ffs(who) - 1);
       __syncwarp();
     }
-    auto tlb = [&](int t) -> float { return t < 128 ? s_tlb[t] : tile_lb(t); };
+    auto tlb = [&](int t) -> float { return t < kTcSmemTiles ? s_tlb[t] : tile_lb(t); };
     int lo = t0 - 1, hi = t0 + 1;
     bool first = true, done = false;
     auto next_tile = [&]() -> int {
@@ -353,7 +350,9 @@
         }
       }
       const float rmaxf = __uint_as_float(__reduce_max_sync(0xffffffffu, rmax));
-      const unsigned tc0 = max4(pq0), tc1 = max4(pq1), tc2 = max4(pq2), tc3 = max4(pq3);
+      unsigned tcm[kPq];
+#pragma unroll
+      for (int i = 0; i < kPq; ++i) tcm[i] = max(pq[i].x, pq[i].y);
       if (*v_abort || *v_dead) return -1;
       const bool is_left = lane < 16;
       while (true) {
@@ -363,11 +362,14 @@
         const float lb = valid ? tlb(t) : INFINITY;
         unsigned cm = 0xFFFFFFFFu;
         {
-          const int src = t & 31, sl = (t >> 5) & 3;
-          const unsigned a0 = __shfl_sync(0xffffffffu, tc0, src), a1 = __shfl_sync(0xffffffffu, tc1, src);
-          const unsigned a2 = __shfl_sync(0xffffffffu, tc2, src), a3 = __shfl_sync(0xffffffffu, tc3, src);
-          if (valid && t < 128) cm = sl == 0 ? a0 : sl == 1 ? a1 : sl == 2 ? a2 : a3;
-          else if (valid) cm = max4(__ldcg(tcm4 + t));
+          const int src = t & 31, sl = (t >> 5) & (kPq - 1);
+#pragma unroll
+          for (int i = 0; i < kPq; ++i) {
+            const unsigned a = __shfl_sync(0xffffffffu, tcm[i], src);
+            if (sl == i) cm = a;
+          }
+          if (!valid) cm = 0xFFFFFFFFu;
+          else if (t >= kTcSmemTiles) { const uint2 q = __ldcg(tcm2 + t); cm = max(q.x, q.y); }
         }
         const bool visit = valid && (lb <= 0.0f || !(lb > rmaxf) || !(lb > __uint_as_float(cm)));
         const unsigned vb = __ballot_sync(0xffffffffu, visit);
@@ -401,12 +403,15 @@
     auto issue_x = [&](int n) {
       const int t = v_seq[n & 7];
       if (lane != 0) return;
-      const uint32_t bar = bar_fullx0 + 8 * (n & (kTcStages - 1));
+      const uint32_t bar = bar_fullx0 + 8 * (n % kTcStages);
       if (t < 0) { mbar_arrive(bar); return; }
       mbar_expect_tx(bar, kXBytes);
-      bulk_g2s(sX0 + (n & (kTcStages - 1)) * kXBytes, tB + ((size_t)t * kTcImages + 2) * kTileFloats, kXBytes, bar);
+      bulk_g2s(sX0 + (n % kTcStages) * kXBytes, tB + ((size_t)t * kTcImages + 2) * kTileFloats, kXBytes, bar);
     };
-    for (int n = 0; n < 3; ++n) { decide(n); issue_x(n); }
+    for (int n = 0; n < 3; ++n) {
+      decide(n);
+      if (n < kTcStages) issue_x(n);
+    }
     prof(11, tick() - t_setup);
     long long p_wm = 0, p_dec = 0, p_sf = 0;
     auto mbar_test = [&](uint32_t bar, uint32_t parity) -> bool {
@@ -420,16 +425,15 @@
           : "memory");
       return __all_sync(0xffffffffu, ready != 0);
     };
-    int nd = 3, nx = 3;
+    int nd = 3, nx = kTcStages;
     bool ok = true, end_decided = v_seq[0] < 0 || v_seq[1] < 0 || v_seq[2] < 0;
-    if (end_decided) nx = nd;
     int idle = 0;
     long long t_idle = 0;
     while (ok && !(end_decided && nx == nd)) {
-      const uint32_t bar_s = bar_sfree0 + 8 * (nx & (kTcStages - 1)), par_s = (uint32_t)(((nx - 4) >> 2) & 1);
+      const uint32_t bar_s = bar_sfree0 + 8 * (nx % kTcStages), par_s = (uint32_t)((nx / kTcStages - 1) & 1);
       const uint32_t bar_m = bar_mma0 + 8 * ((nd - 3) & (kTcDone - 1)), par_m = (uint32_t)(((nd - 3) >> 2) & 1);
       const bool can_x = nx < nd, can_d = !end_decided && nd < nx + 4;
-      if (can_x && (nx < 4 || mbar_test(bar_s, par_s))) {
+      if (can_x && mbar_test(bar_s, par_s)) {
         if (kProf && idle) { (can_d ? p_wm : p_sf) += tick() - t_idle; }
         idle = 0;
         issue_x(nx);
@@ -454,8 +458,7 @@
     if (lane == 0) s_npos = n_issued;
   } else {
     const int wg = warp >> 2;
-    const int rbase = (wg & 1) * 64 + 16 * (warp & 3);
-    const int cb = (wg >> 1) * 64;
+    const int rbase = wg * 64 + 16 * (warp & 3);
     const int cl = 2 * (lane & 3);
     const float kLow = 1.0f - 0.5f * kTcC;
     const float kW = kTcC / kLow;
@@ -471,8 +474,8 @@
       Ri_ub[h] = row_ok[h] ? INFINITY : -INFINITY;
     }
     const uint32_t row_bits = (row_ok[0] ? 0x33333333u : 0u) | (row_ok[1] ? 0xCCCCCCCCu : 0u);
-    const float4* __restrict__ aex = reinterpret_cast<const float4*>(smem + 2 * kTcTileBytes);
-    const uint32_t aH = sA + (uint32_t)((wg & 1) * 64 * 16), aL = aH + kTcTileBytes;
+    const float4* __restrict__ aex = reinterpret_cast<const float4*>(smem + (wg * kTcImages + 2) * kTcTileBytes);
+    const uint32_t aH = sA + (uint32_t)(wg * kTcImages * kTcTileBytes), aL = aH + kTcTileBytes;
     float* wcj = s_wcj[warp];
     unsigned short* wq = s_queue[warp];
     int evals_w = 0;
@@ -484,7 +487,7 @@
     int pf_tile = -1;
     unsigned long long pf_cb[2] = {~0ull, ~0ull};
     unsigned pf_ob[2] = {0u, 0u};
-    unsigned* __restrict__ tcmw = tile_cmax + ((size_t)pair * (V >> 7)) * 4 + (cb >> 5);
+    unsigned* __restrict__ tcmw = tile_cmax + ((size_t)pair * (V / kTcN)) * 2;
     int rr_tile = -1;
     unsigned rr_val[2] = {0u, 0u};
     auto rr_flush = [&]() {
@@ -492,14 +495,14 @@
 #pragma unroll
       for (int s = 0; s < 2; ++s) {
         const unsigned m = __reduce_max_sync(0xffffffffu, rr_val[s]);
-        if (lane == 0) atomicMin(tcmw + (size_t)rr_tile * 4 + s, m);
+        if (lane == 0) atomicMin(tcmw + (size_t)rr_tile * 2 + s, m);
       }
       rr_tile = -1;
     };
     for (int k = 0;; ++k) {
-      const int ts = k & (kTcDone - 1), st = k & (kTcStages - 1), hs = k & 1;
+      const int ts = k & (kTcDone - 1), st = k % kTcStages;
       const long long q0 = tick();
-      if (alive) alive = mbar_wait(bar_fullx0 + 8 * st, (uint32_t)((k >> 2) & 1));
+      if (alive) alive = mbar_wait(bar_fullx0 + 8 * st, (uint32_t)((k / kTcStages) & 1));
       const long long q1 = tick();
       p_wx += q1 - q0;
       alive = __all_sync(0xffffffffu, alive);
@@ -514,9 +517,9 @@
         } else {
 #pragma unroll
           for (int s = 0; s < 2; ++s)
-            if (c0 + cb + 32 * s + lane < nB) {
-              cb_cur[s] = __ldcg(cbg + c0 + cb + 32 * s + lane);
-              ob[s] = permB[c0 + cb + 32 * s + lane];
+            if (c0 + 32 * s + lane < nB) {
+              cb_cur[s] = __ldcg(cbg + c0 + 32 * s + lane);
+              ob[s] = permB[c0 + 32 * s + lane];
             }
         }
         pf_tile = -1;
@@ -527,16 +530,16 @@
 #pragma unroll
             for (int s = 0; s < 2; ++s) {
               pf_cb[s] = ~0ull; pf_ob[s] = 0u;
-              if (jn * kTcN + cb + 32 * s + lane < nB) {
-                pf_cb[s] = __ldcg(cbg + jn * kTcN + cb + 32 * s + lane);
-                pf_ob[s] = permB[jn * kTcN + cb + 32 * s + lane];
+              if (jn * kTcN + 32 * s + lane < nB) {
+                pf_cb[s] = __ldcg(cbg + jn * kTcN + 32 * s + lane);
+                pf_ob[s] = permB[jn * kTcN + 32 * s + lane];
               }
             }
           }
         }
       }
       const long long q2 = tick();
-      if (alive && jt >= 0) alive = mbar_wait(bar_fullhl0 + 8 * hs, (uint32_t)((k >> 1) & 1));
+      if (alive && jt >= 0) alive = mbar_wait(bar_fullhl, (uint32_t)(k & 1));
       alive = __all_sync(0xffffffffu, alive);
       if (!wg_all(alive && jt >= 0, wg)) {
         if (!alive) *v_dead = 1;
@@ -546,15 +549,16 @@
 #pragma unroll
       for (int i = 0; i < 32; ++i) d[i] = 0.0f;
       {
-        const uint32_t bH = sHL0 + hs * kHLBytes + (uint32_t)(cb * 16), bL = bH + kTcTileBytes;
+        constexpr uint32_t kKB = 2 * kTcBlk * 16;
+        const uint32_t bH = sHL, bL = bH + kTcTileBytes;
         asm volatile("wgmma.fence.sync.aligned;\n" ::: "memory");
 #pragma unroll
         for (int kb = 0; kb < kTcKB; ++kb) {
-          wgmma_tf32_64x64x8(d, tc_smem_desc(aH + kb * 4096), tc_smem_desc(bL + kb * 4096), kb > 0);
-          wgmma_tf32_64x64x8(d, tc_smem_desc(aL + kb * 4096), tc_smem_desc(bH + kb * 4096), 1);
-        }
-#pragma unroll
-        for (int kb = 0; kb < kTcKB; ++kb) wgmma_tf32_64x64x8(d, tc_smem_desc(aH + kb * 4096), tc_smem_desc(bH + kb * 4096), 1);
+          wgmma_tf32_64x64x8(d, tc_smem_desc(aH + kb * kKB), tc_smem_desc(bL + kb * kKB), kb > 0);
+          wgmma_tf32_64x64x8(d, tc_smem_desc(aL + kb * kKB), tc_smem_desc(bH + kb * kKB), 1);
+        }
+#pragma unroll
+        for (int kb = 0; kb < kTcKB; ++kb) wgmma_tf32_64x64x8(d, tc_smem_desc(aH + kb * kKB), tc_smem_desc(bH + kb * kKB), 1);
         asm volatile("wgmma.commit_group.sync.aligned;\n" ::: "memory");
         asm volatile("wgmma.wait_group.sync.aligned 0;\n" ::: "memory");
 #pragma unroll
@@ -570,12 +574,12 @@
       const long long q4 = tick();
       p_ld += q4 - q3;
       if (!skip) {
-        const float4* __restrict__ bex = reinterpret_cast<const float4*>(smem + kABytes + 2 * kHLBytes + st * kXBytes);
+        const float4* __restrict__ bex = reinterpret_cast<const float4*>(smem + kABytes + kHLBytes + st * kXBytes);
         float dbest[2];
         bool col_warm = false;
 #pragma unroll
         for (int s = 0; s < 2; ++s) {
-          const float nbm = bex[9 * 128 + cb + 32 * s + lane].x;
+          const float nbm = bex[9 * kTcBlk + 32 * s + lane].x;
           dbest[s] = cb_cur[s] == ~0ull ? INFINITY : __uint_as_float((unsigned)(cb_cur[s] >> 32));
           wcj[32 * s + lane] = nbm == INFINITY ? -INFINITY : dbest[s];
           col_warm |= cb_cur[s] == ~0ull && nbm != INFINITY;
@@ -597,7 +601,7 @@
 #pragma unroll
             for (int e = 0; e < 2; ++e) {
               const int c = 2 * i + cl + e;
-              const float nbc = bex[9 * 128 + cb + c].x;
+              const float nbc = bex[9 * kTcBlk + c].x;
               const float ub0 = fmaf(kW, nam[0] + nbc, d[i + e]), ub1 = fmaf(kW, nam[1] + nbc, d[i + 2 + e]);
               rowub[0] = fminf(rowub[0], ub0);
               rowub[1] = fminf(rowub[1], ub1);
@@ -618,7 +622,7 @@
         __syncwarp();
         const long long q5 = tick();
         p_prep += q5 - q4;
-        const int ncol = nB - c0 - cb;
+        const int ncol = nB - c0;
         uint32_t mask = 0, col_bits = 0;
 #pragma unroll
         for (int i = 0; i < 32; i += 4) {
@@ -636,8 +640,8 @@
             if (2 * i + cl + (e & 1) < ncol) col_bits |= 1u << (i + e);
             if (kDbg) {
               const int h = e >> 1, c = 2 * i + cl + (e & 1);
-              if (stripe == 0 && k == 0 && row_ok[h] && c < ncol)
-                dbg_tile[(size_t)oa[h] * kTcN + permB[c0 + cb + c]] = fmaf(0.5f * kW, nam[h] + bex[9 * 128 + cb + c].x, lbv);
+              if (stripe == 0 && row_ok[h] && c < ncol)
+                dbg_tile[(size_t)oa[h] * 128 + permB[c0 + c]] = fmaf(0.5f * kW, nam[h] + bex[9 * kTcBlk + c].x, lbv);
             }
           }
         }
@@ -660,11 +664,10 @@
           const int sl = q >> 5, i = q & 31, h = (i >> 1) & 1;
           const int rr = rbase + (sl >> 2) + 8 * h;
           const int c = 8 * (i >> 2) + 2 * (sl & 3) + (i & 1);
-          const int pcol = cb + c;
           float acc = 0.0f;
 #pragma unroll
           for (int kc = 0; kc < (kDescDim + 3) / 4; ++kc) {
-            const float4 a = aex[kc * 128 + rr], b = bex[kc * 128 + pcol];
+            const float4 a = aex[kc * kTcBlk + (rr & (kTcBlk - 1))], b = bex[kc * kTcBlk + c];
             float diff = a.x - b.x;
             acc = __fmaf_rn(diff, diff, acc);
             if (4 * kc + 1 < kDescDim) { diff = a.y - b.y; acc = __fmaf_rn(diff, diff, acc); }
@@ -680,14 +683,14 @@
           if (lane < nb && acc == acc) {
             const unsigned long long pr = tc_pack(acc, (int)oc);
             if (pr < v_rbest[rr]) atomicMin(&s_rbest[rr], pr);
-            if (acc <= dbc) atomicMin(cbg + c0 + pcol, tc_pack(acc, (int)orow));
+            if (acc <= dbc) atomicMin(cbg + c0 + c, tc_pack(acc, (int)orow));
           }
           __syncwarp();
           remaining = tot - nb;
         }
         if (lane == 0 && evals_w) {
           const int seen = atomicAdd(&s_evals, evals_w) + evals_w;
-          if (k >= 7 && seen > (k + 1) * (kTcM * kTcN / 2)) *v_abort = 1;
+          if ((k + 1) * (kTcM * kTcN) >= 8 * 128 * 128 && seen > (k + 1) * (kTcM * kTcN / 2)) *v_abort = 1;
         }
         evals_w = 0;
         p_ev += tick() - q6;
@@ -700,8 +703,8 @@
 #pragma unroll
         for (int s = 0; s < 2; ++s) {
           rr_val[s] = 0;
-          if (c0 + cb + 32 * s + lane < nB) {
-            const unsigned long long cbn = __ldcg(cbg + c0 + cb + 32 * s + lane);
+          if (c0 + 32 * s + lane < nB) {
+            const unsigned long long cbn = __ldcg(cbg + c0 + 32 * s + lane);
             rr_val[s] = cbn == ~0ull ? 0x7F800000u : (unsigned)(cbn >> 32);
           }
         }
@@ -726,7 +729,30 @@
   if (!aborted && threadIdx.x < kTcM && r0 + (int)threadIdx.x < nA) rowbest[(size_t)pair * V + r0 + threadIdx.x] = s_rbest[threadIdx.x];
 }
 
-static size_t tc_smem_bytes() { return (size_t)kTcImages * kTcTileBytes + 2 * 2 * (size_t)kTcTileBytes + (size_t)kTcStages * kTcTileBytes; }
+static size_t tc_smem_bytes() {
+  return ((size_t)(kTcM / kTcBlk) * kTcImages + 2 + kTcStages) * kTcTileBytes;
+}
+
+static int tc_prepare(qb200_handle* h, const void* kernel) {
+  if (int rc = ensure_dyn_smem(h, kernel, tc_smem_bytes())) return rc;
+  QB_CUDA_TRY(h, cudaFuncSetAttribute(kernel, cudaFuncAttributePreferredSharedMemoryCarveout, cudaSharedmemCarveoutMaxShared));
+  return QB200_OK;
+}
+
+int tc_footprint(qb200_handle* h, int* out5) {
+  const void* kernel = (const void*)tc_nn_kernel<false>;
+  if (int rc = tc_prepare(h, kernel)) return rc;
+  cudaFuncAttributes fa;
+  QB_CUDA_TRY(h, cudaFuncGetAttributes(&fa, kernel));
+  int ctas = 0;
+  QB_CUDA_TRY(h, cudaOccupancyMaxActiveBlocksPerMultiprocessor(&ctas, kernel, kTcThreads, tc_smem_bytes()));
+  out5[0] = kTcThreads;
+  out5[1] = (int)tc_smem_bytes();
+  out5[2] = (int)fa.sharedSizeBytes;
+  out5[3] = fa.numRegs;
+  out5[4] = ctas;
+  return QB200_OK;
+}
 
 static int sort_and_dedup(qb200_handle* h, int n_clouds, int dedup) {
   const int V = h->V;
@@ -749,7 +775,7 @@
 int launch_match_nn(qb200_handle* h, int n_pairs) {
   const int V = h->V;
   const size_t smem = tc_smem_bytes();
-  if (int rc = ensure_dyn_smem(h, (const void*)tc_nn_kernel<false>, smem)) return rc;
+  if (int rc = tc_prepare(h, (const void*)tc_nn_kernel<false>)) return rc;
   int rc = sort_and_dedup(h, 2 * n_pairs, 1);
   if (rc) return rc;
   const uint32_t* uperm = h->val_a;
@@ -768,7 +794,7 @@
   cudaEventRecord(h->kev[0], h->stream);
   static const int tc_prof = (getenv("QB200_TC_PROF") && getenv("QB200_TC_PROF")[0] == '1') ? 1 : 0;
   if (tc_prof) {
-    if (int rc2 = ensure_dyn_smem(h, (const void*)tc_nn_kernel<false, true>, smem)) return rc2;
+    if (int rc2 = tc_prepare(h, (const void*)tc_nn_kernel<false, true>)) return rc2;
     tc_nn_kernel<false, true><<<g, kTcThreads, smem, h->stream>>>(h->desc_tiles, h->desc_norm, n_unique, V, uperm, rowbest_u, colbest_u,
                                                                   tile_cmax, h->tc_fallback, h->tc_stats, nullptr);
   } else {
@@ -785,7 +811,7 @@
 
 int launch_tc_debug_tile(qb200_handle* h, float* d_out) {
   const size_t smem = tc_smem_bytes();
-  if (int rc0 = ensure_dyn_smem(h, (const void*)tc_nn_kernel<true>, smem)) return rc0;
+  if (int rc0 = tc_prepare(h, (const void*)tc_nn_kernel<true>)) return rc0;
   int rc = sort_and_dedup(h, 2, 0);
   if (rc) return rc;
   const uint32_t* uperm = h->val_a;
```

After: 12730, median of 6. +5.0%, better.
